# MasterVVK/qwen3-tts-axera-russian

Hardware: AMD Instinct MI355X
Metric: 12Hz codec-tokens/s (codec frames/s, 16 codes each) + RTF, Qwen3-TTS-0.6B (higher is better)
Workload: dtype f16 weights/KV, f32 accumulate (talker+CP); vocoder exact fp32 (f32 MFMA); 1 GPU; configs[2]/[3]: batch=32 mixed ru/en prompts per GPU, 64 frames/utterance/step (prefill + hipGraph decode loop), utterance-sharded DP over 1 GPU(s); batch_per_gpu=32

## Files before the change

### qwen3_tts_axera_russian_amd/csrc/q3_cp_api.hip

```cpp
#include "../../include/qwen3tts_cp.h"
#include "q3_cp.h"

namespace q3 {

static bool two_row_enabled() {
    static const bool on = !(getenv("Q3_CP_TWO_ROW") && atoi(getenv("Q3_CP_TWO_ROW")) == 0);
    return on;
}

int cp_seed_row0(const Work& w, int R, int row0, int R_total) {
    if (R_total <= 0) R_total = R;
    const int R16 = (R + 15) / 16 * 16;
    const bool two = two_row_enabled() && row0 == 0 && R_total == R && 2 * R16 <= w.max_rows;
    return two ? R16 : 0;
}

int cp_frame(hipStream_t s, const Model& m, Work& w, KVCache& kv, int R, const CpFrameIO& io, int row0, int R_total) {
    const ModelCfg& c = m.cfg;
    if (R_total <= 0) R_total = R;
    const int H = c.hidden, G = c.cp_groups;
    const int seed0 = cp_seed_row0(w, R, row0, R_total);
    RowMap rm;
    rm.slot_base = 0;
    rm.slot_stride = 1;
    rm.pos_stride = 0;
    if (seed0 > 0) {
        const int R16 = seed0;
        if (w.map_R16 != R16) {
            std::vector<int> slot(2 * R16), pos(2 * R16);
            for (int i = 0; i < 2 * R16; i++) {
                slot[i] = i % R16;
                pos[i] = i < R16 ? 1 : 0;
            }
            Q3_HIP(hipMemcpyAsync(w.map_slot, slot.data(), sizeof(int) * 2 * R16, hipMemcpyHostToDevice, s), -1);
            Q3_HIP(hipMemcpyAsync(w.map_pos, pos.data(), sizeof(int) * 2 * R16, hipMemcpyHostToDevice, s), -1);
            Q3_HIP(hipStreamSynchronize(s), -1);
            w.map_R16 = R16;
        }
        if (launch_gather_embed(s, m.talker_emb, c.talker_vocab, H, io.codes, 0, io.n_frames, io.frame_cap, 0, w.h, w.ssq, R,
                                row0, R_total, io.forced, w.xh, m.cp.L[0].in_ln))
            return -1;
        RowMap r2;
        r2.slot = w.map_slot;
        r2.pos = w.map_pos;
        r2.same_slot_rows = true;
        r2.valid_mod = R16;
        r2.valid_n = R;
        if (run_stack(s, m, m.cp, w, kv, R16 + R, r2, 256, 0)) return -1;
    } else {
        rm.pos_base = 0;
        if (run_stack(s, m, m.cp, w, kv, R, rm, 256, row0)) return -1;
        if (launch_gather_embed(s, m.talker_emb, c.talker_vocab, H, io.codes, 0, io.n_frames, io.frame_cap, 0, w.h, w.ssq, R,
                                row0, R_total, io.forced, w.xh, m.cp.L[0].in_ln))
            return -1;
        rm.pos_base = 1;
        if (run_stack(s, m, m.cp, w, kv, R, rm, 256, row0)) return -1;
    }
    const bool qkv_tab = m.cp_qkv_serves(R);
    for (int g = 0; g < G; g++) {
        if (g > 0) {
            rm.pos_base = g + 1;
            rm.skip_qkv0 = qkv_tab;
            if (run_stack(s, m, m.cp, w, kv, R, rm, 256, row0)) return -1;
        }
        LinArgs a;
        a.wp = m.cp_head[g].wp;
        a.N = c.cp_vocab;
        a.K = H;
        a.M = row0 + R;
        a.m_begin = row0;
        a.nt = 0;
        a.x16 = w.xh;
        a.ssq = w.ssq;
        a.ssq_parts = H / 16;
        a.eps = c.eps;
        a.y = w.logits;
        a.ldy = c.cp_vocab;
        if (launch_linear(s, a, PRO_NORM, EPI_STORE)) return -1;
        CpArgmaxArgs x;
        x.logits = w.logits;
        x.V = c.cp_vocab;
        x.R = R;
        x.row0 = row0;
        x.R_total = R_total;
        x.H = H;
        x.group = g;
        x.codes = io.codes;
        x.n_frames = io.n_frames;
        x.frame_cap = io.frame_cap;
        x.temperature = io.temperature;
        x.top_k = io.top_k;
        x.seed = io.seed;
        x.seed_ptr = io.seed_ptr;
        x.forced = io.forced;
        x.slots = io.slots;
        if (g + 1 < G) {
            x.next_table = m.cp_emb[g];
            x.h_out = w.h;
            x.ssq_out = w.ssq;
            x.xh_out = w.xh;
            x.gamma_next = m.cp.L[0].in_ln;
            if (qkv_tab) {
                x.next_qkv = m.cp_qkv_rows(g);
                x.qkv_out = w.qkv;
                x.qkv_ld = (c.n_heads + 2 * c.n_kv) * c.head_dim;
            }
        } else if (io.fb_h) {
            x.talker_emb = m.talker_emb;
            x.talker_vocab = c.talker_vocab;
            x.cp_tables = m.d_cp_emb_ptrs;
            x.pad_embed = io.pad_embed;
            x.n_groups = G;
            x.h_out = io.fb_h;
            x.ssq_out = io.fb_ssq;
            x.xh_out = io.fb_xh;
            x.gamma_next = io.fb_gamma;
        }
        if (launch_cp_argmax(s, x)) return -1;
    }
    return 0;
}

}

using namespace q3;

namespace {

struct CpHandle {
    Model* m = nullptr;
    int max_batch = 1;
    KVCache kv;
    Work w;
    hipStream_t s = nullptr;
    int *d_codes = nullptr, *d_nframes = nullptr;
    std::vector<int> h_codes;
    GraphExec graph;
    int graph_rows = 0;
    int step_next_pos = 0;
};

}

extern "C" {

void* cp_load(const char* weights, const char* embeddings_dir, int max_batch) {
    if (!weights) return nullptr;
    if (max_batch <= 0) max_batch = 1;
    Model* m = model_load(weights, false, true, embeddings_dir);
    if (!m) return nullptr;
    CpHandle* h = new CpHandle();
    h->m = m;
    h->max_batch = max_batch;
    const ModelCfg& c = m->cfg;
    bool ok = hipStreamCreate(&h->s) == hipSuccess;
    ok = ok && kv_alloc(h->kv, c.cp_layers, max_batch, c.n_kv, c.cp_groups + 1) == 0;
    ok = ok && work_alloc(h->w, c, 2 * ((max_batch + 15) / 16 * 16), c.cp_ffn, c.cp_vocab) == 0;
    ok = ok && hipMalloc((void**)&h->d_codes, sizeof(int) * 16 * max_batch) == hipSuccess;
    ok = ok && hipMalloc((void**)&h->d_nframes, sizeof(int) * max_batch) == hipSuccess;
    if (ok) {
        std::vector<int> ones(max_batch, 1);
        ok = hipMemcpy(h->d_nframes, ones.data(), sizeof(int) * max_batch, hipMemcpyHostToDevice) == hipSuccess;
    }
    if (!ok) {
        Q3_LOG("cp_load: allocation failed");
        cp_free(h);
        return nullptr;
    }
    h->h_codes.resize((size_t)16 * max_batch);
    return h;
}

void cp_free(void* hh) {
    CpHandle* h = (CpHandle*)hh;
    if (!h) return;
    if (h->s) hipStreamSynchronize(h->s);
    h->graph.reset();
    kv_free(h->kv);
    work_free(h->w);
    if (h->d_codes) hipFree(h->d_codes);
    if (h->d_nframes) hipFree(h->d_nframes);
    if (h->s) hipStreamDestroy(h->s);
    model_free(h->m);
    delete h;
}

int cp_hidden_size(void* hh) {
    CpHandle* h = (CpHandle*)hh;
    return h ? h->m->cfg.hidden : 0;
}

int cp_predict_batch(void* hh, const float* hidden, const int32_t* code_0, int n_rows, float temperature, int top_k,
                     uint64_t seed, int32_t* out_codes) {
    CpHandle* h = (CpHandle*)hh;
    if (!h || !hidden || !code_0 || !out_codes || n_rows <= 0 || n_rows > h->max_batch) return -1;
    const bool stochastic = temperature > 1e-6f;
    const Model& m = *h->m;
    const int H = m.cfg.hidden, G = m.cfg.cp_groups, R = n_rows;
    for (int r = 0; r < R; r++) {
        h->h_codes[(size_t)r * 16] = code_0[r];
        for (int j = 1; j < 16; j++) h->h_codes[(size_t)r * 16 + j] = -1;
    }
    Q3_HIP(hipMemcpyAsync(h->d_codes, h->h_codes.data(), sizeof(int) * 16 * R, hipMemcpyHostToDevice, h->s), -1);
    Q3_HIP(hipMemcpyAsync(h->w.rows_in, hidden, sizeof(float) * (size_t)R * H, hipMemcpyHostToDevice, h->s), -1);
    CpFrameIO io;
    io.codes = h->d_codes;
    io.n_frames = h->d_nframes;
    io.frame_cap = 1;
    io.temperature = temperature;
    io.top_k = top_k;
    io.seed = seed;
    auto body = [&]() -> int {
        if (launch_ssq_rows(h->s, h->w.rows_in, h->w.h, h->w.ssq, R, H, h->w.xh, m.cp.L[0].in_ln,
                            cp_seed_row0(h->w, R)))
            return -1;
        return cp_frame(h->s, m, h->w, h->kv, R, io);
    };
    if (stochastic) {
        if (body()) return -1;
    } else if (!h->graph.e || h->graph_rows != R) {
        if (body()) return -1;
        Q3_HIP(hipStreamSynchronize(h->s), -1);
        h->graph.reset();
        Q3_HIP(hipStreamBeginCapture(h->s, hipStreamCaptureModeThreadLocal), -1);
        int rc = body();
        hipError_t e = hipStreamEndCapture(h->s, &h->graph.g);
        if (rc || e != hipSuccess) {
            Q3_LOG("cp_predict: graph capture failed");
            return -1;
        }
        Q3_HIP(hipGraphInstantiate(&h->graph.e, h->graph.g, nullptr, nullptr, 0), -1);
        h->graph_rows = R;
    } else {
        Q3_HIP(hipGraphLaunch(h->graph.e, h->s), -1);
    }
    Q3_HIP(hipMemcpyAsync(h->h_codes.data(), h->d_codes, sizeof(int) * 16 * R, hipMemcpyDeviceToHost, h->s), -1);
    Q3_HIP(hipStreamSynchronize(h->s), -1);
    for (int r = 0; r < R; r++)
        for (int g = 0; g < G; g++) out_codes[(size_t)r * G + g] = h->h_codes[(size_t)r * 16 + 1 + g];
    return 0;
}

int cp_predict(void* hh, const float* hidden, int32_t code_0, float temperature, int top_k, uint64_t seed,
               int32_t* out_codes) {
    return cp_predict_batch(hh, hidden, &code_0, 1, temperature, top_k, seed, out_codes);
// ... 53 lines not shown
```

### qwen3_tts_axera_russian_amd/csrc/q3_engine.hip

```cpp
#include "../../include/qwen3tts_engine.h"
#include "q3_cp.h"

#include <algorithm>
#include <chrono>
#include <cmath>

using namespace q3;

namespace {

struct Engine {
    Model* m = nullptr;
    int max_batch = 0, n_ctx = 0, max_frames = 0;
    hipStream_t s = nullptr;
    KVCache kv_t, kv_c;
    Work wt, wc;
    int prefill_rows = 0;
    int *d_slot = nullptr, *d_pos = nullptr;
    int* d_tiles = nullptr;
    int *d_iota = nullptr;
    int *d_past = nullptr, *d_npast = nullptr, *d_ntext = nullptr, *d_done = nullptr, *d_nframes = nullptr;
    int *d_pos0 = nullptr, *d_posdec = nullptr, *d_lastrow = nullptr;
    int* d_codes = nullptr;
    int* d_forced = nullptr;
    bool forced_on = false;
    unsigned long long* d_seed = nullptr;
    unsigned long long n_requests = 0, req_seed = 0, n_refills = 0;
    float* d_pad = nullptr;
    int B = 0, ignore_eos = 0, cap_frames = 0, frames_run = 0;
    int frames_hi = 0;
    GraphExec graph[8];
    int graph_B = 0, graph_ignore = -1, graph_cap = -1, graph_chains = 0;
    hipEvent_t ev0 = nullptr, ev1 = nullptr;
    float last_run_ms = 0.f, last_prefill_ms = 0.f, last_host_launch_ms = 0.f;
    int* h_done = nullptr;
    float t_temp = 0.f, t_top_p = 0.95f, c_temp = 0.f;
    int t_top_k = 50, c_top_k = 50;
    unsigned long long seed = 0;
    int n_chains = 1;
    hipStream_t cs[8] = {nullptr};
    hipEvent_t ev_fork = nullptr, ev_join[8] = {nullptr};
    bool slot_mode = false;
    int graph_slots = -1;
    SlotParams* d_slots = nullptr;
    std::vector<int> h_budget, h_age;
    std::vector<char> h_live;
};

unsigned long long mix_seed(unsigned long long seed, unsigned long long k, unsigned long long golden) {
    unsigned long long z = seed + golden * k;
    z = (z ^ (z >> 30)) * 0xBF58476D1CE4E5B9ull;
    z = (z ^ (z >> 27)) * 0x94D049BB133111EBull;
    return z ^ (z >> 31);
}

int talker_tail(Engine* e, hipStream_t st, int row0, int R) {
    const Model& m = *e->m;
    const int H = m.cfg.hidden;
    FinalNormArgs f;
    f.h = e->wt.h;
    f.ssq = e->wt.ssq;
    f.ssq_parts = H / 16;
    f.gamma = m.talker.final_norm;
    f.eps = m.cfg.eps;
    f.R = R;
    f.row0 = row0;
    f.H = H;
    f.out_f32 = e->wt.hidden_f32;
    f.out_f16 = e->wt.hidden_f16;
    f.out_copy = e->wc.h;
    f.out_copy_ssq = e->wc.ssq;
    f.out_copy_xh = e->wc.xh;
    f.out_copy_gamma = m.cp.L[0].in_ln;
    f.out_copy_row_off = cp_seed_row0(e->wc, R, row0, e->B);
    if (launch_final_norm(st, f)) return -1;
    LinArgs a;
    a.wp = m.talker_head.wp;
    a.N = m.cfg.talker_vocab;
    a.K = H;
    a.M = row0 + R;
    a.m_begin = row0;
    a.nt = 1;
    a.x16 = e->wt.hidden_f16;
    a.y = e->wt.logits;
    a.ldy = m.cfg.talker_vocab;
    return launch_linear(st, a, PRO_F16, EPI_STORE);
}

int frame_chain(Engine* e, hipStream_t st, int row0, int R) {
    const Model& m = *e->m;
    TalkerSampleArgs sa;
    sa.logits = e->wt.logits;
    sa.V = m.cfg.talker_vocab;
    sa.R = R;
    sa.row0 = row0;
    sa.R_total = e->B;
    sa.audio_vocab = m.cfg.cp_vocab;
    sa.eos = m.cfg.codec_eos;
    sa.past = e->d_past;
    sa.n_past = e->d_npast;
    sa.n_text = e->d_ntext;
    sa.done = e->d_done;
    sa.codes = e->d_codes;
    sa.n_frames = e->d_nframes;
    sa.frame_cap = e->max_frames;
    sa.pos0 = e->d_pos0;
    sa.pos = e->d_posdec;
    sa.ignore_eos = e->ignore_eos;
    sa.max_frames = e->cap_frames;
    sa.temperature = e->t_temp;
    sa.top_k = e->t_top_k;
    sa.top_p = e->t_top_p;
    sa.seed = e->seed;
    sa.seed_ptr = e->d_seed;
    sa.forced = e->forced_on ? e->d_forced : nullptr;
    sa.slots = e->slot_mode ? e->d_slots : nullptr;
    if (launch_talker_sample(st, sa)) return -1;
    CpFrameIO io;
    io.codes = e->d_codes;
    io.n_frames = e->d_nframes;
    io.frame_cap = e->max_frames;
    io.fb_h = e->wt.h;
    io.fb_ssq = e->wt.ssq;
    io.fb_xh = e->wt.xh;
    io.fb_gamma = m.talker.L[0].in_ln;
    io.pad_embed = e->d_pad;
    io.temperature = e->c_temp;
    io.top_k = e->c_top_k;
    io.seed = e->seed ^ 0x5851F42D4C957F2Dull;
    io.seed_ptr = e->d_seed;
    io.forced = e->forced_on ? e->d_forced : nullptr;
    io.slots = e->slot_mode ? e->d_slots : nullptr;
    if (cp_frame(st, m, e->wc, e->kv_c, R, io, row0, e->B)) return -1;
    RowMap rm;
    rm.slot_base = 0;
    rm.slot_stride = 1;
    rm.pos = e->d_posdec;
    if (run_stack(st, m, m.talker, e->wt, e->kv_t, R, rm, 1024, row0)) return -1;
    return talker_tail(e, st, row0, R);
}

int n_chains_eff(const Engine* e) {
    const int nc = e->n_chains < 1 ? 1 : e->n_chains;
    return (nc > 1 && e->B % (16 * nc) == 0) ? nc : 1;
}

void chain_rows(const Engine* e, int c, int& row0, int& R) {
    const int nc = n_chains_eff(e);
    row0 = 0;
    for (int i = 0; i < c; i++) row0 += e->B / nc + (i < e->B % nc ? 1 : 0);
    R = e->B / nc + (c < e->B % nc ? 1 : 0);
}

int frame_eager(Engine* e) {
    const int nc = n_chains_eff(e);
    for (int c = 0; c < nc; c++) {
        int row0, R;
        chain_rows(e, c, row0, R);
        if (frame_chain(e, e->cs[c], row0, R)) return -1;
    }
    return 0;
}

int fork_chains(Engine* e) {
    Q3_HIP(hipEventRecord(e->ev_fork, e->s), -1);
    for (int c = 0; c < n_chains_eff(e); c++) Q3_HIP(hipStreamWaitEvent(e->cs[c], e->ev_fork, 0), -1);
    return 0;
}
int join_chains(Engine* e) {
    for (int c = 0; c < n_chains_eff(e); c++) {
        Q3_HIP(hipEventRecord(e->ev_join[c], e->cs[c]), -1);
        Q3_HIP(hipStreamWaitEvent(e->s, e->ev_join[c], 0), -1);
    }
    return 0;
}

}

extern "C" {

void q3e_free(void* ee) {
    Engine* e = (Engine*)ee;
    if (!e) return;
    if (e->s) hipStreamSynchronize(e->s);
    for (auto& g : e->graph) g.reset();
    kv_free(e->kv_t);
    kv_free(e->kv_c);
    work_free(e->wt);
    work_free(e->wc);
    void* ps[] = {e->d_tiles, e->d_slot, e->d_pos,  e->d_iota,   e->d_past,    e->d_npast, e->d_ntext, e->d_done,
                  e->d_nframes, e->d_pos0, e->d_posdec, e->d_lastrow, e->d_codes, e->d_pad, e->d_forced, e->d_seed, e->d_slots};
    for (void* p : ps)
        if (p) hipFree(p);
    if (e->h_done) hipHostFree(e->h_done);
    for (int c = 0; c < 8; c++) {
        if (e->cs[c]) hipStreamDestroy(e->cs[c]);
        if (e->ev_join[c]) hipEventDestroy(e->ev_join[c]);
    }
    if (e->ev_fork) hipEventDestroy(e->ev_fork);
    if (e->ev0) hipEventDestroy(e->ev0);
    if (e->ev1) hipEventDestroy(e->ev1);
    if (e->s) hipStreamDestroy(e->s);
    if (e->m) model_free(e->m);
    delete e;
}

void* q3e_create(const char* weights, int max_batch, int n_ctx, int max_frames) {
    if (!weights || max_batch <= 0 || n_ctx <= 0 || max_frames <= 0) return nullptr;
    Model* m = model_load(weights, true, true);
    if (!m) return nullptr;
    if (n_ctx > m->max_pos) {
        Q3_LOG("q3e_create: n_ctx=%d exceeds the RoPE table (%d)", n_ctx, m->max_pos);
        model_free(m);
        return nullptr;
    }
    Engine* e = new Engine();
    e->m = m;
    e->max_batch = max_batch;
    e->n_ctx = n_ctx;
    e->max_frames = max_frames;
    const ModelCfg& c = m->cfg;
    e->prefill_rows = max_batch > 2048 ? max_batch : 2048;
    int prio_lo = 0, prio_hi = 0;
    const bool use_prio = !(getenv("Q3_STREAM_PRIO") && atoi(getenv("Q3_STREAM_PRIO")) == 0) &&
                          hipDeviceGetStreamPriorityRange(&prio_lo, &prio_hi) == hipSuccess && prio_lo != prio_hi;
    auto mkstream = [&](hipStream_t* st) {
        return (use_prio ? hipStreamCreateWithPriority(st, hipStreamNonBlocking, prio_hi)
                         : hipStreamCreateWithFlags(st, hipStreamNonBlocking)) == hipSuccess;
    };
    bool ok = mkstream(&e->s);
    ok = ok && hipEventCreate(&e->ev0) == hipSuccess && hipEventCreate(&e->ev1) == hipSuccess;
    ok = ok && hipEventCreateWithFlags(&e->ev_fork, hipEventDisableTiming) == hipSuccess;
    for (int c = 0; c < 8 && ok; c++)
        ok = mkstream(&e->cs[c]) &&
             hipEventCreateWithFlags(&e->ev_join[c], hipEventDisableTiming) == hipSuccess;
    if (const char* nc = getenv("Q3_CHAINS")) e->n_chains = atoi(nc) < 1 ? 1 : atoi(nc) > 8 ? 8 : atoi(nc);
    else e->n_chains = 1;
    ok = ok && kv_alloc(e->kv_t, c.talker_layers, max_batch, c.n_kv, n_ctx) == 0;
    ok = ok && kv_alloc(e->kv_c, c.cp_layers, max_batch, c.n_kv, c.cp_groups + 1) == 0;
    ok = ok && work_alloc(e->wt, c, e->prefill_rows, c.talker_ffn, c.talker_vocab) == 0;
    ok = ok && work_alloc(e->wc, c, 2 * ((max_batch + 15) / 16 * 16), c.cp_ffn, c.cp_vocab) == 0;
    auto ialloc = [&](int** p, size_t n) { return hipMalloc((void**)p, sizeof(int) * n) == hipSuccess; };
    ok = ok && ialloc(&e->d_slot, e->prefill_rows) && ialloc(&e->d_pos, e->prefill_rows);
    ok = ok && ialloc(&e->d_tiles, (size_t)4 * e->prefill_rows);
    ok = ok && ialloc(&e->d_iota, max_batch) && ialloc(&e->d_past, (size_t)max_batch * 32);
    ok = ok && ialloc(&e->d_npast, max_batch) && ialloc(&e->d_ntext, max_batch) && ialloc(&e->d_done, max_batch);
    ok = ok && ialloc(&e->d_nframes, max_batch) && ialloc(&e->d_pos0, max_batch) && ialloc(&e->d_posdec, max_batch);
    ok = ok && ialloc(&e->d_lastrow, max_batch);
    ok = ok && ialloc(&e->d_codes, (size_t)max_frames * max_batch * 16);
    ok = ok && hipMalloc((void**)&e->d_pad, sizeof(float) * c.hidden) == hipSuccess;
    ok = ok && hipMalloc((void**)&e->d_seed, sizeof(unsigned long long) * max_batch) == hipSuccess;
    ok = ok && hipMemset(e->d_seed, 0, sizeof(unsigned long long) * max_batch) == hipSuccess;
    ok = ok && hipHostMalloc((void**)&e->h_done, sizeof(int) * max_batch, 0) == hipSuccess;
    if (ok) {
        std::vector<int> iota(max_batch);
        for (int i = 0; i < max_batch; i++) iota[i] = i;
        ok = hipMemcpy(e->d_iota, iota.data(), sizeof(int) * max_batch, hipMemcpyHostToDevice) == hipSuccess;
        ok = ok && hipMemset(e->d_pad, 0, sizeof(float) * c.hidden) == hipSuccess;
    }
    if (!ok) {
        Q3_LOG("q3e_create: allocation failed");
        q3e_free(e);
        return nullptr;
    }
    return e;
}

int q3e_set_sampling(void* ee, float talker_temperature, int talker_top_k, float talker_top_p, float cp_temperature,
                     int cp_top_k, uint64_t seed) {
    Engine* e = (Engine*)ee;
    if (!e) return -1;
    e->t_temp = talker_temperature;
    e->t_top_k = talker_top_k;
    e->t_top_p = talker_top_p;
    e->c_temp = cp_temperature;
    e->c_top_k = cp_top_k;
    e->seed = seed;
    e->n_requests = 0;
    for (auto& g : e->graph) g.reset();
    return 0;
}

int q3e_set_forced_codes(void* ee, const int32_t* forced, int n_frames) {
    Engine* e = (Engine*)ee;
    if (!e) return -1;
    const bool on = forced != nullptr && n_frames > 0;
    if (on && e->slot_mode) {
        Q3_LOG("q3e_set_forced_codes: not for a per-slot batch (q3e_open)");
        return -1;
    }
    if (on) {
        if (e->B <= 0 || n_frames > e->max_frames) return -1;
        const size_t total = (size_t)e->max_frames * e->max_batch * 16;
        if (!e->d_forced) Q3_HIP(hipMalloc((void**)&e->d_forced, sizeof(int) * total), -1);
        Q3_HIP(hipMemset(e->d_forced, 0xff, sizeof(int) * total), -1);
        Q3_HIP(hipMemcpy(e->d_forced, forced, sizeof(int) * 16 * (size_t)e->B * n_frames, hipMemcpyHostToDevice), -1);
    }
    if (on != e->forced_on) {
        e->forced_on = on;
        for (auto& g : e->graph) g.reset();
    }
    return 0;
}

int q3e_set_chains(void* ee, int n) {
    Engine* e = (Engine*)ee;
    if (!e || n < 1 || n > 8) return -1;
    if (n != e->n_chains) {
        e->n_chains = n;
        for (auto& g : e->graph) g.reset();
    }
    return 0;
}

int q3e_set_pad_embed(void* ee, const float* pad) {
    Engine* e = (Engine*)ee;
    if (!e || !pad) return -1;
    Q3_HIP(hipMemcpy(e->d_pad, pad, sizeof(float) * e->m->cfg.hidden, hipMemcpyHostToDevice), -1);
    return 0;
}

static int prefill_ids(Engine* e, int n, const int* ids, const float* prefix, const int32_t* n_rows, int B_total) {
    const Model& m = *e->m;
    const int H = m.cfg.hidden;
    size_t row_off = 0;
    int u0 = 0;
    std::vector<int> slot, pos, tiles, last(n);
    while (u0 < n) {
        int u1 = u0, rows = 0;
        while (u1 < n && rows + n_rows[u1] <= e->prefill_rows) rows += n_rows[u1++];
        slot.resize(rows);
        pos.resize(rows);
        int r = 0;
        tiles.clear();
        bool contiguous = true;
        for (int u = u0; u < u1; u++) {
            const int b = ids[u];
            if (u > u0 && b != ids[u - 1] + 1) contiguous = false;
            for (int i = 0; i < n_rows[u]; i += 16) {
                const int nn = n_rows[u] - i < 16 ? n_rows[u] - i : 16;
                const int t4[4] = {r + i, nn, b, i};
                tiles.insert(tiles.end(), t4, t4 + 4);
            }
            for (int i = 0; i < n_rows[u]; i++, r++) {
                slot[r] = b;
                pos[r] = i;
            }
            last[u] = r - 1;
        }
        Q3_HIP(hipMemcpyAsync(e->wt.rows_in, prefix + row_off * H, sizeof(float) * (size_t)rows * H, hipMemcpyHostToDevice, e->s), -1);
        Q3_HIP(hipMemcpyAsync(e->d_slot, slot.data(), sizeof(int) * rows, hipMemcpyHostToDevice, e->s), -1);
        Q3_HIP(hipMemcpyAsync(e->d_pos, pos.data(), sizeof(int) * rows, hipMemcpyHostToDevice, e->s), -1);
        Q3_HIP(hipMemcpyAsync(e->d_tiles, tiles.data(), sizeof(int) * tiles.size(), hipMemcpyHostToDevice, e->s), -1);
        if (contiguous) {
            Q3_HIP(hipMemcpyAsync(e->d_lastrow + ids[u0], last.data() + u0, sizeof(int) * (u1 - u0), hipMemcpyHostToDevice, e->s), -1);
        } else {
            for (int u = u0; u < u1; u++)
                Q3_HIP(hipMemcpyAsync(e->d_lastrow + ids[u], last.data() + u, sizeof(int), hipMemcpyHostToDevice, e->s), -1);
        }
        if (launch_ssq_rows(e->s, e->wt.rows_in, e->wt.h, e->wt.ssq, rows, H, e->wt.xh, m.talker.L[0].in_ln)) return -1;
        RowMap rm;
        rm.slot = e->d_slot;
        rm.pos = e->d_pos;
        rm.same_slot_rows = true;
        rm.tiles = e->d_tiles;
        rm.n_tiles = (int)(tiles.size() / 4);
        if (run_stack(e->s, m, m.talker, e->wt, e->kv_t, rows, rm, 1024)) return -1;
        for (int u = u0; u < u1; u += contiguous ? (u1 - u0) : 1) {
            FinalNormArgs f;
            f.h = e->wt.h;
            f.ssq = e->wt.ssq;
            f.ssq_parts = H / 16;
            f.gamma = m.talker.final_norm;
            f.eps = m.cfg.eps;
            f.R = contiguous ? u1 - u0 : 1;
            f.row0 = ids[u];
            f.H = H;
            f.row_map = e->d_lastrow;
            f.out_f32 = e->wt.hidden_f32;
            f.out_f16 = e->wt.hidden_f16;
            f.out_copy = e->wc.h;
            f.out_copy_ssq = e->wc.ssq;
            f.out_copy_xh = e->wc.xh;
            f.out_copy_gamma = m.cp.L[0].in_ln;
            f.out_copy_row_off = n_chains_eff(e) == 1 ? cp_seed_row0(e->wc, B_total, 0, B_total) : 0;
            if (launch_final_norm(e->s, f)) return -1;
        }
        Q3_HIP(hipStreamSynchronize(e->s), -1);
        row_off += rows;
        u0 = u1;
    }
    return 0;
}

static int clear_slot(Engine* e, int b, const int32_t* n_rows, const int32_t* n_text) {
    Q3_HIP(hipMemsetAsync(e->d_npast + b, 0, sizeof(int), e->s), -1);
    Q3_HIP(hipMemsetAsync(e->d_done + b, 0, sizeof(int), e->s), -1);
    Q3_HIP(hipMemsetAsync(e->d_nframes + b, 0, sizeof(int), e->s), -1);
    Q3_HIP(hipMemsetAsync(e->d_past + 32 * b, 0, sizeof(int) * 32, e->s), -1);
    Q3_HIP(hipMemset2DAsync(e->d_codes + 16 * (size_t)b, sizeof(int) * 16 * (size_t)e->B, 0xff, sizeof(int) * 16, e->max_frames, e->s), -1);
    Q3_HIP(hipMemcpyAsync(e->d_ntext + b, n_text, sizeof(int), hipMemcpyHostToDevice, e->s), -1);
    Q3_HIP(hipMemcpyAsync(e->d_pos0 + b, n_rows, sizeof(int), hipMemcpyHostToDevice, e->s), -1);
    Q3_HIP(hipMemcpyAsync(e->d_posdec + b, n_rows, sizeof(int), hipMemcpyHostToDevice, e->s), -1);
    return 0;
}

static int head_all_rows(Engine* e) {
    const Model& m = *e->m;
    LinArgs a;
    a.wp = m.talker_head.wp;
    a.N = m.cfg.talker_vocab;
    a.K = m.cfg.hidden;
    a.M = e->B;
    a.nt = 1;
    a.x16 = e->wt.hidden_f16;
    a.y = e->wt.logits;
    a.ldy = m.cfg.talker_vocab;
    return launch_linear(e->s, a, PRO_F16, EPI_STORE);
}

int q3e_start(void* ee, int B, const float* prefix, const int32_t* n_rows, const int32_t* n_text, int ignore_eos,
              int max_frames) {
    Engine* e = (Engine*)ee;
    if (!e || !prefix || !n_rows || !n_text || B <= 0 || B > e->max_batch) return -1;
    const Model& m = *e->m;
    const int H = m.cfg.hidden;
    if (max_frames <= 0 || max_frames > e->max_frames) max_frames = e->max_frames;
    std::vector<int> pos0(B);
    for (int b = 0; b < B; b++) {
        if (n_rows[b] <= 0 || n_rows[b] > e->prefill_rows || n_rows[b] + max_frames > e->n_ctx) {
            Q3_LOG("q3e_start: utterance %d: %d prefix rows + %d frames do not fit n_ctx=%d", b, n_rows[b], max_frames,
                   e->n_ctx);
            return -1;
        }
        pos0[b] = n_rows[b];
    }
    e->B = B;
    e->ignore_eos = ignore_eos ? 1 : 0;
    e->cap_frames = max_frames;
    e->frames_run = 0;
    e->frames_hi = 0;
    e->slot_mode = false;
    Q3_HIP(hipMemsetAsync(e->d_npast, 0, sizeof(int) * B, e->s), -1);
    Q3_HIP(hipMemsetAsync(e->d_done, 0, sizeof(int) * B, e->s), -1);
    Q3_HIP(hipMemsetAsync(e->d_nframes, 0, sizeof(int) * B, e->s), -1);
    Q3_HIP(hipMemsetAsync(e->d_past, 0, sizeof(int) * 32 * B, e->s), -1);
    Q3_HIP(hipMemsetAsync(e->d_codes, 0xff, sizeof(int) * 16 * (size_t)B * e->max_frames, e->s), -1);
    {
        unsigned long long z = e->seed + 0x9E3779B97F4A7C15ull * e->n_requests++;
        z = (z ^ (z >> 30)) * 0xBF58476D1CE4E5B9ull;
        z = (z ^ (z >> 27)) * 0x94D049BB133111EBull;
        e->req_seed = e->n_requests == 1 ? e->seed : (z ^ (z >> 31));
        e->n_refills = 0;
        std::vector<unsigned long long> seeds(B, e->req_seed);
        Q3_HIP(hipMemcpy(e->d_seed, seeds.data(), sizeof(unsigned long long) * B, hipMemcpyHostToDevice), -1);
    }
    if (e->forced_on) {
        e->forced_on = false;
        for (auto& g : e->graph) g.reset();
    }
    Q3_HIP(hipMemcpyAsync(e->d_ntext, n_text, sizeof(int) * B, hipMemcpyHostToDevice, e->s), -1);
    Q3_HIP(hipMemcpyAsync(e->d_pos0, pos0.data(), sizeof(int) * B, hipMemcpyHostToDevice, e->s), -1);
    Q3_HIP(hipMemcpyAsync(e->d_posdec, pos0.data(), sizeof(int) * B, hipMemcpyHostToDevice, e->s), -1);
    Q3_HIP(hipStreamSynchronize(e->s), -1);
    Q3_HIP(hipEventRecord(e->ev0, e->s), -1);
    {
        std::vector<int> ids(B);
        for (int b = 0; b < B; b++) ids[b] = b;
        if (prefill_ids(e, B, ids.data(), prefix, n_rows, B)) return -1;
    }
    if (head_all_rows(e)) return -1;
    Q3_HIP(hipEventRecord(e->ev1, e->s), -1);
    Q3_HIP(hipStreamSynchronize(e->s), -1);
    hipEventElapsedTime(&e->last_prefill_ms, e->ev0, e->ev1);
    return 0;
}

int q3e_run(void* ee, int n_frames) {
    Engine* e = (Engine*)ee;
    if (!e || e->B <= 0 || n_frames <= 0) return -1;
    int room = (e->cap_frames < e->max_frames ? e->cap_frames : e->max_frames) - e->frames_run;
    if (e->slot_mode) {
        room = 0;
        for (int b = 0; b < e->B; b++)
            if (e->h_live[b]) room = std::max(room, e->h_budget[b] - e->h_age[b]);
    }
    if (room <= 0) return 0;
    if (n_frames > room) n_frames = room;
    int done_frames = 0;
    const int nc = n_chains_eff(e);
    Q3_HIP(hipEventRecord(e->ev0, e->s), -1);
    if (fork_chains(e)) return -1;
    static const bool no_graph = getenv("Q3_NO_GRAPH") && atoi(getenv("Q3_NO_GRAPH")) != 0;
    const bool need_capture = !e->graph[0].e || e->graph_B != e->B || e->graph_ignore != e->ignore_eos ||
                              e->graph_cap != e->cap_frames || e->graph_chains != nc ||
                              e->graph_slots != (int)e->slot_mode;
    if (no_graph) {
        for (; done_frames < n_frames; done_frames++)
            if (frame_eager(e)) return -1;
    } else if (need_capture) {
        if (frame_eager(e)) return -1;
        done_frames++;
        for (int c = 0; c < nc; c++) Q3_HIP(hipStreamSynchronize(e->cs[c]), -1);
        for (int c = 0; c < nc; c++) {
            int row0, R;
            chain_rows(e, c, row0, R);
            e->graph[c].reset();
            Q3_HIP(hipStreamBeginCapture(e->cs[c], hipStreamCaptureModeRelaxed), -1);
            int rc = frame_chain(e, e->cs[c], row0, R);
            hipError_t er = hipStreamEndCapture(e->cs[c], &e->graph[c].g);
            if (rc || er != hipSuccess) {
                Q3_LOG("q3e_run: graph capture failed");
                return -1;
            }
            Q3_HIP(hipGraphInstantiate(&e->graph[c].e, e->graph[c].g, nullptr, nullptr, 0), -1);
        }
        e->graph_B = e->B;
        e->graph_ignore = e->ignore_eos;
        e->graph_cap = e->cap_frames;
        e->graph_chains = nc;
        e->graph_slots = (int)e->slot_mode;
    }
    const int check_every = 16;
    const auto th0 = std::chrono::steady_clock::now();
    while (!no_graph && done_frames < n_frames) {
        int chunk = n_frames - done_frames;
        if (!e->ignore_eos && chunk > check_every) chunk = check_every;
        for (int i = 0; i < chunk; i++)
            for (int c = 0; c < nc; c++) Q3_HIP(hipGraphLaunch(e->graph[c].e, e->cs[c]), -1);
        done_frames += chunk;
        if (!e->ignore_eos && done_frames < n_frames) {
            if (join_chains(e)) return -1;
            Q3_HIP(hipMemcpyAsync(e->h_done, e->d_done, sizeof(int) * e->B, hipMemcpyDeviceToHost, e->s), -1);
            Q3_HIP(hipStreamSynchronize(e->s), -1);
            bool all = true;
            for (int b = 0; b < e->B; b++) all = all && e->h_done[b];
            if (all) break;
            if (fork_chains(e)) return -1;
        }
    }
    e->last_host_launch_ms = (float)std::chrono::duration<double, std::milli>(std::chrono::steady_clock::now() - th0).count();
    if (join_chains(e)) return -1;
    Q3_HIP(hipEventRecord(e->ev1, e->s), -1);
    Q3_HIP(hipStreamSynchronize(e->s), -1);
    hipEventElapsedTime(&e->last_run_ms, e->ev0, e->ev1);
    if (e->slot_mode) {
        for (int b = 0; b < e->B; b++)
            if (e->h_age[b] >= 0) e->h_age[b] = std::min(e->h_age[b] + done_frames, e->max_frames);
        return done_frames;
    }
    e->frames_run += done_frames;
    e->frames_hi += done_frames;
    return done_frames;
}

float q3e_last_run_ms(void* ee) { return ee ? ((Engine*)ee)->last_run_ms : -1.f; }
float q3e_last_host_launch_ms(void* ee) { return ee ? ((Engine*)ee)->last_host_launch_ms : -1.f; }
float q3e_last_prefill_ms(void* ee) { return ee ? ((Engine*)ee)->last_prefill_ms : -1.f; }

int q3e_get_codes(void* ee, int32_t* out, int max_out_frames, int32_t* n_frames_per_utt) {
    Engine* e = (Engine*)ee;
    if (!e || !out || e->B <= 0) return -1;
    int nf = e->frames_hi < e->max_frames ? e->frames_hi : e->max_frames;
    if (e->slot_mode) {
        int hi = 0;
        for (int b = 0; b < e->B; b++)
            hi = std::max(hi, e->h_age[b]);
        nf = std::min(hi, e->max_frames);
    }
    if (nf > max_out_frames) nf = max_out_frames;
    Q3_HIP(hipMemcpy(out, e->d_codes, sizeof(int) * 16 * (size_t)e->B * nf, hipMemcpyDeviceToHost), -1);
    if (n_frames_per_utt) {
        Q3_HIP(hipMemcpy(n_frames_per_utt, e->d_npast, sizeof(int) * e->B, hipMemcpyDeviceToHost), -1);
    }
    return nf;
}

int q3e_get_done(void* ee, int32_t* done, int32_t* frames) {
    Engine* e = (Engine*)ee;
    if (!e || !done || e->B <= 0) return -1;
    Q3_HIP(hipMemcpy(done, e->d_done, sizeof(int) * e->B, hipMemcpyDeviceToHost), -1);
    std::vector<int> np(e->B);
    Q3_HIP(hipMemcpy(np.data(), e->d_npast, sizeof(int) * e->B, hipMemcpyDeviceToHost), -1);
    for (int b = 0; b < e->B; b++)
        if (np[b] >= (e->slot_mode ? e->h_budget[b] : e->cap_frames)) done[b] = 1;
    if (e->slot_mode)
        for (int b = 0; b < e->B; b++)
            if (done[b]) e->h_live[b] = 0;
    if (frames) memcpy(frames, np.data(), sizeof(int) * e->B);
    return 0;
}

int q3e_refill(void* ee, int n, const int32_t* slots, const float* prefix, const int32_t* n_rows, const int32_t* n_text) {
    Engine* e = (Engine*)ee;
    if (!e || e->B <= 0 || n <= 0 || n > e->B || !slots || !prefix || !n_rows || !n_text) return -1;
    if (e->forced_on) {
        Q3_LOG("q3e_refill: a teacher-forced batch cannot be refilled");
        return -1;
    }
    if (e->slot_mode) {
        Q3_LOG("q3e_refill: a per-slot batch (q3e_open) takes new utterances with q3e_admit");
        return -1;
    }
    std::vector<int> ids(slots, slots + n), seen(e->B, 0);
    for (int u = 0; u < n; u++) {
        const int b = ids[u];
        if (b < 0 || b >= e->B || seen[b]++) {
            Q3_LOG("q3e_refill: slot %d is out of range or listed twice (batch of %d)", b, e->B);
            return -1;
        }
        if (n_rows[u] <= 0 || n_rows[u] > e->prefill_rows || n_rows[u] + e->cap_frames > e->n_ctx) {
            Q3_LOG("q3e_refill: utterance %d: %d prefix rows + %d frames do not fit n_ctx=%d", u, n_rows[u], e->cap_frames, e->n_ctx);
            return -1;
        }
    }
    Q3_HIP(hipStreamSynchronize(e->s), -1);
    Q3_HIP(hipEventRecord(e->ev0, e->s), -1);
    for (int u = 0; u < n; u++) {
        const int b = ids[u];
        if (clear_slot(e, b, n_rows + u, n_text + u)) return -1;
        unsigned long long z = e->req_seed + 0xD1B54A32D192ED03ull * ++e->n_refills;
        z = (z ^ (z >> 30)) * 0xBF58476D1CE4E5B9ull;
        z = (z ^ (z >> 27)) * 0x94D049BB133111EBull;
        z ^= z >> 31;
        Q3_HIP(hipMemcpyAsync(e->d_seed + b, &z, sizeof(z), hipMemcpyHostToDevice, e->s), -1);
        Q3_HIP(hipStreamSynchronize(e->s), -1);
    }
    Q3_HIP(hipStreamSynchronize(e->s), -1);
    if (prefill_ids(e, n, ids.data(), prefix, n_rows, e->B)) return -1;
    if (head_all_rows(e)) return -1;
    Q3_HIP(hipEventRecord(e->ev1, e->s), -1);
    Q3_HIP(hipStreamSynchronize(e->s), -1);
    hipEventElapsedTime(&e->last_prefill_ms, e->ev0, e->ev1);
    e->frames_run = 0;
    return 0;
}

int q3e_open(void* ee, int B, int ignore_eos) {
    Engine* e = (Engine*)ee;
    if (!e || B <= 0 || B > e->max_batch) return -1;
    const Model& m = *e->m;
    const ModelCfg& c = m.cfg;
    if (c.talker_vocab > 4096 || c.cp_vocab > 4096) {
        Q3_LOG("q3e_open: vocabularies of %d / %d are beyond the per-slot sampler", c.talker_vocab, c.cp_vocab);
        return -1;
    }
    Q3_HIP(hipStreamSynchronize(e->s), -1);
    if (!e->d_slots) Q3_HIP(hipMalloc((void**)&e->d_slots, sizeof(SlotParams) * e->max_batch), -1);
    e->B = B;
    e->ignore_eos = ignore_eos ? 1 : 0;
    e->cap_frames = e->max_frames;
    e->frames_run = 0;
    e->frames_hi = 0;
    e->slot_mode = true;
    e->h_budget.assign(B, 0);
    e->h_age.assign(B, -1);
    e->h_live.assign(B, 0);
    if (e->forced_on) {
        e->forced_on = false;
        for (auto& g : e->graph) g.reset();
    }
    Q3_HIP(hipMemsetAsync(e->d_npast, 0, sizeof(int) * B, e->s), -1);
    Q3_HIP(hipMemsetD32Async((hipDeviceptr_t)e->d_done, 1, B, e->s), -1);
    Q3_HIP(hipMemsetD32Async((hipDeviceptr_t)e->d_nframes, e->max_frames, B, e->s), -1);
    Q3_HIP(hipMemsetAsync(e->d_past, 0, sizeof(int) * 32 * B, e->s), -1);
    Q3_HIP(hipMemsetAsync(e->d_ntext, 0, sizeof(int) * B, e->s), -1);
// ... 10 lines not shown

int q3e_admit(void* ee, int n, const int32_t* slots, const float* prefix, const int32_t* n_rows, const int32_t* n_text,
              const q3e_slot_params* params) {
    Engine* e = (Engine*)ee;
    if (!e || !e->slot_mode || n <= 0 || n > e->B || !slots || !prefix || !n_rows || !n_text || !params) {
        if (e && !e->slot_mode) Q3_LOG("q3e_admit: the batch was not opened with q3e_open");
        return -1;
    }
    std::vector<int> ids(slots, slots + n), seen(e->B, 0);
    std::vector<SlotParams> sp(n);
    for (int u = 0; u < n; u++) {
        const int b = ids[u];
        const q3e_slot_params& p = params[u];
        if (b < 0 || b >= e->B || seen[b]++) {
            Q3_LOG("q3e_admit: slot %d is out of range or listed twice (batch of %d)", b, e->B);
            return -1;
        }
        if (p.max_frames <= 0 || p.max_frames > e->max_frames) {
            Q3_LOG("q3e_admit: utterance %d: a budget of %d frames is outside 1..%d", u, p.max_frames, e->max_frames);
            return -1;
        }
        if (n_rows[u] <= 0 || n_rows[u] > e->prefill_rows || n_rows[u] + p.max_frames > e->n_ctx) {
            Q3_LOG("q3e_admit: utterance %d: %d prefix rows + %d frames do not fit n_ctx=%d", u, n_rows[u], p.max_frames, e->n_ctx);
            return -1;
        }
        if (!(std::isfinite(p.temperature) && p.temperature >= 0.f) || !(std::isfinite(p.cp_temperature) && p.cp_temperature >= 0.f) ||
            !(p.top_p > 0.f && p.top_p <= 1.f)) {
            Q3_LOG("q3e_admit: utterance %d: temperatures must be finite and >= 0, top_p in (0, 1]", u);
            return -1;
        }
        sp[u].max_frames = p.max_frames;
        sp[u].t_temp = p.temperature;
        sp[u].t_top_k = p.top_k;
        sp[u].t_top_p = p.top_p;
        sp[u].c_temp = p.cp_temperature;
        sp[u].c_top_k = p.cp_top_k;
        sp[u].seed = mix_seed(p.seed, (unsigned long long)(uint32_t)p.utt + 1ull, 0x9E3779B97F4A7C15ull);
        sp[u].no_row = 1;
    }
    Q3_HIP(hipStreamSynchronize(e->s), -1);
    Q3_HIP(hipEventRecord(e->ev0, e->s), -1);
    for (int u = 0; u < n; u++) {
        if (clear_slot(e, ids[u], n_rows + u, n_text + u)) return -1;
        Q3_HIP(hipMemcpyAsync(e->d_slots + ids[u], &sp[u], sizeof(SlotParams), hipMemcpyHostToDevice, e->s), -1);
    }
    Q3_HIP(hipStreamSynchronize(e->s), -1);
    const int H = e->m->cfg.hidden;
    size_t row_off = 0;
    for (int u = 0; u < n; u++) {
        if (prefill_ids(e, 1, &ids[u], prefix + row_off * H, n_rows + u, e->B)) return -1;
        row_off += n_rows[u];
    }
    if (head_all_rows(e)) return -1;
    Q3_HIP(hipEventRecord(e->ev1, e->s), -1);
    Q3_HIP(hipStreamSynchronize(e->s), -1);
    hipEventElapsedTime(&e->last_prefill_ms, e->ev0, e->ev1);
    for (int u = 0; u < n; u++) {
        e->h_budget[ids[u]] = sp[u].max_frames;
        e->h_age[ids[u]] = 0;
        e->h_live[ids[u]] = 1;
    }
    return 0;
}

int q3e_release(void* ee, int n, const int32_t* slots) {
    Engine* e = (Engine*)ee;
    if (!e || !e->slot_mode || n < 0 || (n > 0 && !slots)) return -1;
    for (int u = 0; u < n; u++)
        if (slots[u] < 0 || slots[u] >= e->B) {
            Q3_LOG("q3e_release: slot %d is out of range (batch of %d)", slots[u], e->B);
            return -1;
        }
    for (int u = 0; u < n; u++) {
        Q3_HIP(hipMemsetD32Async((hipDeviceptr_t)(e->d_done + slots[u]), 1, 1, e->s), -1);
        e->h_live[slots[u]] = 0;
    }
    Q3_HIP(hipStreamSynchronize(e->s), -1);
    return 0;
}

int q3e_get_hidden(void* ee, float* out) {
    Engine* e = (Engine*)ee;
    if (!e || !out || e->B <= 0) return -1;
    Q3_HIP(hipMemcpy(out, e->wt.hidden_f32, sizeof(float) * (size_t)e->B * e->m->cfg.hidden, hipMemcpyDeviceToHost), -1);
    return 0;
}

double q3e_step_weight_bytes(void* ee) {
    Engine* e = (Engine*)ee;
    if (!e) return 0.0;
    const ModelCfg& c = e->m->cfg;
    const double head = 2.0 * c.hidden;
    double bytes = (double)e->m->talker.weight_bytes + head * c.talker_vocab +
                   (double)(c.cp_groups + 1) * (double)e->m->cp.weight_bytes + head * c.cp_vocab * c.cp_groups;
    int row0 = 0, R = e->B;
    if (e->B > 0) chain_rows(e, 0, row0, R);
    if (R > 0 && e->m->cp_qkv_serves(R)) {
        const double qkv_ld = (double)(c.n_heads + 2 * c.n_kv) * c.head_dim;
        bytes -= (double)(c.cp_groups - 1) * (qkv_ld * c.hidden * 2.0 - 4.0 * qkv_ld * e->B);
    }
    return bytes;
}

}
```

### qwen3_tts_axera_russian_amd/csrc/q3_model.h

```cpp
#pragma once
#include "q3_kernels.h"

namespace q3 {

struct DevLinear {
    half_t* wp = nullptr;
    int N = 0, K = 0;
};

struct DevLayer {
    DevLinear qkv, o, gu, down;
    float *in_ln = nullptr, *post_ln = nullptr, *q_norm = nullptr, *k_norm = nullptr;
};

struct DevStack {
    std::vector<DevLayer> L;
    float* final_norm = nullptr;
    const float* tail_gamma = nullptr;
    int ffn = 0;
    int nt = 0;
    size_t weight_bytes = 0;
};

struct Model {
    ModelCfg cfg;
    int device = 0;
    bool has_talker = false, has_cp = false;
    DevStack talker, cp;
    float* talker_emb = nullptr;
    DevLinear talker_head;
    std::vector<float*> cp_emb;
    std::vector<DevLinear> cp_head;
    const float** d_cp_emb_ptrs = nullptr;
    float* cp_qkv_tab = nullptr;
    int cp_qkv_kbw = 0;
    const float* cp_qkv_rows(int group) const {
        return cp_qkv_tab + (size_t)group * cfg.cp_vocab * ((cfg.n_heads + 2 * cfg.n_kv) * cfg.head_dim);
    }
    bool cp_qkv_serves(int rows) const {
        return cp_qkv_tab && linear_decode_kbw(cfg.hidden, (cfg.n_heads + 2 * cfg.n_kv) * cfg.head_dim, rows) == cp_qkv_kbw;
    }
    float *rope_cos = nullptr, *rope_sin = nullptr;
    int max_pos = 0;
    std::vector<void*> allocs;
    size_t device_bytes = 0;
};

Model* model_load(const char* path, bool want_talker, bool want_cp, const char* aux_dir = nullptr);
void model_free(Model* m);

struct KVCache {
    half_t *k = nullptr, *v = nullptr;
    int n_layers = 0, n_slots = 0, n_kv = 0, n_ctx = 0, head_dim = 128;
    size_t layer_stride() const { return (size_t)n_slots * n_kv * n_ctx * head_dim; }
    size_t bytes() const { return layer_stride() * n_layers * sizeof(half_t) * 2; }
};
int kv_alloc(KVCache& kv, int n_layers, int n_slots, int n_kv, int n_ctx);
void kv_free(KVCache& kv);
int kv_zero(hipStream_t s, KVCache& kv);

inline size_t frag_idx_host(int m, int k, int K) {
    return ((((size_t)(m >> 4) * (K >> 5) + (k >> 5)) * 64 + (m & 15) + 16 * ((k >> 3) & 3)) << 3) + (k & 7);
}

struct Work {
    int max_rows = 0, hidden = 0;
    float* rows_in = nullptr;
    float *h = nullptr, *ssq = nullptr, *qkv = nullptr;
    half_t* xh = nullptr;
    half_t *attn = nullptr, *act = nullptr;
    float* hidden_f32 = nullptr;
    half_t* hidden_f16 = nullptr;
    float* logits = nullptr;
    int *map_slot = nullptr, *map_pos = nullptr;
    int map_R16 = 0;
};
int work_alloc(Work& w, const ModelCfg& c, int max_rows, int ffn, int max_vocab);
void work_free(Work& w);
int work_zero(hipStream_t s, Work& w, const ModelCfg& c, int ffn, int max_vocab);

struct RowMap {
    const int* slot = nullptr;
    const int* pos = nullptr;
    int slot_base = 0, slot_stride = 0, pos_base = 0, pos_stride = 0;
    bool same_slot_rows = false;
    int valid_mod = 0, valid_n = 0;
    const int* tiles = nullptr;
    int n_tiles = 0;
    bool skip_qkv0 = false;
};

int run_stack(hipStream_t s, const Model& m, const DevStack& st, Work& w, KVCache& kv, int R,
              const RowMap& rm, int attn_threads, int row0 = 0);

struct GraphExec {
    hipGraph_t g = nullptr;
    hipGraphExec_t e = nullptr;
    void reset();
};

}
```

### qwen3_tts_axera_russian_amd/csrc/q3_model.hip

```cpp
#include "q3_model.h"

#include <cmath>

namespace q3 {

namespace {

struct Loader {
    Model* m;
    const Pack& p;
    hipStream_t s = nullptr;
    half_t* stage = nullptr;
    size_t stage_elems = 0;
    std::vector<uint16_t> host16;
    bool ok = true;

    void* dalloc(size_t bytes) {
        void* d = nullptr;
        if (hipMalloc(&d, bytes) != hipSuccess) {
            Q3_LOG("hipMalloc(%zu) failed", bytes);
            ok = false;
            return nullptr;
        }
        m->allocs.push_back(d);
        m->device_bytes += bytes;
        return d;
    }
    const PackTensor* need(const std::string& n, uint32_t ndim, uint64_t d0, uint64_t d1 = 0) {
        const PackTensor* t = p.find(n);
        if (!t) {
            Q3_LOG("weight file lacks tensor %s", n.c_str());
            ok = false;
            return nullptr;
        }
        if (t->ndim != ndim || t->shape[0] != d0 || (ndim > 1 && t->shape[1] != d1) ||
            (t->dtype != F32 && t->dtype != F16 && t->dtype != BF16)) {
            Q3_LOG("tensor %s: unexpected shape/dtype", n.c_str());
            ok = false;
            return nullptr;
        }
        return t;
    }
    float* up_f32(const std::string& n, uint32_t ndim, uint64_t d0, uint64_t d1 = 0) {
        const PackTensor* t = need(n, ndim, d0, d1);
        if (!t) return nullptr;
        size_t ne = t->numel();
        float* d = (float*)dalloc(ne * 4);
        if (!d) return nullptr;
        if (t->dtype == F32) {
            if (hipMemcpy(d, t->data, ne * 4, hipMemcpyHostToDevice) != hipSuccess) ok = false;
        } else {
            std::vector<float> tmp(ne);
            const uint16_t* src = (const uint16_t*)t->data;
            if (t->dtype == BF16)
                for (size_t i = 0; i < ne; i++) tmp[i] = bf16_to_f32(src[i]);
            else
                for (size_t i = 0; i < ne; i++) tmp[i] = h2f(src[i]);
            if (hipMemcpy(d, tmp.data(), ne * 4, hipMemcpyHostToDevice) != hipSuccess) ok = false;
        }
        return d;
    }
    bool pack_into(const std::string& n, int N, int K, half_t* dst, int tile_off, int tile_stride) {
        const PackTensor* t = need(n, 2, (uint64_t)N, (uint64_t)K);
        if (!t) return false;
        size_t ne = (size_t)N * K;
        if (ne > stage_elems) {
            if (stage) hipFree(stage);
            stage = nullptr;
            if (hipMalloc((void**)&stage, ne * 2) != hipSuccess) {
                ok = false;
                return false;
            }
            stage_elems = ne;
        }
        const void* src = t->data;
        if (t->dtype == F32) {
            host16.resize(ne);
            const float* f = (const float*)t->data;
            for (size_t i = 0; i < ne; i++) host16[i] = f2h_sat(f[i]);
            src = host16.data();
        } else if (t->dtype == BF16) {
            host16.resize(ne);
            const uint16_t* b = (const uint16_t*)t->data;
            for (size_t i = 0; i < ne; i++) host16[i] = f2h_sat(bf16_to_f32(b[i]));
            src = host16.data();
        }
        if (hipMemcpy(stage, src, ne * 2, hipMemcpyHostToDevice) != hipSuccess) {
            ok = false;
            return false;
        }
        if (launch_pack_linear(s, stage, N, K, dst, tile_off, tile_stride) != 0) {
            ok = false;
            return false;
        }
        if (hipStreamSynchronize(s) != hipSuccess) {
            ok = false;
            return false;
        }
        return true;
    }
    DevLinear lin_alloc(int N, int K) {
        DevLinear l;
        l.N = N;
        l.K = K;
        l.wp = (half_t*)dalloc((size_t)N * K * 2);
        return l;
    }
    bool load_stack(DevStack& st, const char* prefix, int n_layers, int ffn) {
        const ModelCfg& c = m->cfg;
        const int H = c.hidden, D = c.head_dim, NQ = c.n_heads * D, NKV = c.n_kv * D;
        st.ffn = ffn;
        st.L.resize(n_layers);
        for (int i = 0; i < n_layers && ok; i++) {
            DevLayer& L = st.L[i];
            std::string b = std::string(prefix) + ".layers." + std::to_string(i) + ".";
            L.in_ln = up_f32(b + "input_ln", 1, H);
            L.post_ln = up_f32(b + "post_ln", 1, H);
            L.q_norm = up_f32(b + "q_norm", 1, D);
            L.k_norm = up_f32(b + "k_norm", 1, D);
            L.qkv = lin_alloc(NQ + 2 * NKV, H);
            L.o = lin_alloc(H, NQ);
            L.gu = lin_alloc(2 * ffn, H);
            L.down = lin_alloc(H, ffn);
            if (!ok) break;
            pack_into(b + "q_proj", NQ, H, L.qkv.wp, 0, 1);
            pack_into(b + "k_proj", NKV, H, L.qkv.wp, NQ / 16, 1);
            pack_into(b + "v_proj", NKV, H, L.qkv.wp, (NQ + NKV) / 16, 1);
            pack_into(b + "o_proj", H, NQ, L.o.wp, 0, 1);
            pack_into(b + "gate_proj", ffn, H, L.gu.wp, 0, 2);
            pack_into(b + "up_proj", ffn, H, L.gu.wp, 1, 2);
            pack_into(b + "down_proj", H, ffn, L.down.wp, 0, 1);
            st.weight_bytes += ((size_t)(NQ + 2 * NKV) * H + (size_t)H * NQ + (size_t)3 * ffn * H) * 2;
        }
        st.final_norm = up_f32(std::string(prefix) + ".norm", 1, H);
        return ok;
    }
    bool build_cp_qkv_table() {
        static const bool on = !(getenv("Q3_CP_QKV_TABLE") && atoi(getenv("Q3_CP_QKV_TABLE")) == 0);
        const ModelCfg& c = m->cfg;
        const int H = c.hidden, V = c.cp_vocab, G = c.cp_groups, ld = (c.n_heads + 2 * c.n_kv) * c.head_dim;
        if (!on || G < 2) return true;
        int pass = 64;
        while (pass >= 16 && !linear_decode_kbw(H, ld, pass)) pass /= 2;
        if (pass < 16) {
            Q3_LOG("code predictor: no q|k|v table (launch_linear has no weight-streaming kernel for K=%d)", H);
            return true;
        }
        const size_t Vp = ((size_t)V + 63) / 64 * 64, bytes = (size_t)(G - 1) * V * ld * sizeof(float);
        float* tab = (float*)dalloc(bytes);
        int* ids = nullptr;
        float *h = nullptr, *ssq = nullptr;
        half_t* xh = nullptr;
        bool good = tab && hipMalloc((void**)&ids, Vp * 4) == hipSuccess && hipMalloc((void**)&h, Vp * H * 4) == hipSuccess &&
                    hipMalloc((void**)&ssq, Vp * (H / 16) * 4) == hipSuccess && hipMalloc((void**)&xh, Vp * H * 2) == hipSuccess;
        if (good) {
            std::vector<int> iota(Vp, -1);
            for (int t = 0; t < V; t++) iota[t] = t;
            good = hipMemcpy(ids, iota.data(), Vp * 4, hipMemcpyHostToDevice) == hipSuccess;
        }
        for (int g = 0; g + 1 < G && good; g++) {
            good = launch_gather_embed(s, m->cp_emb[g], V, H, ids, 1, nullptr, 0, 0, h, ssq, (int)Vp, 0, 0, nullptr, xh,
                                       m->cp.L[0].in_ln) == 0;
            for (int r0 = 0; r0 < V && good; r0 += pass) {
                LinArgs a;
                a.wp = m->cp.L[0].qkv.wp;
                a.N = m->cp.L[0].qkv.N;
                a.K = H;
                a.M = r0 + pass < V ? r0 + pass : V;
                a.m_begin = r0;
                a.nt = m->cp.nt;
                a.x16 = xh;
                a.ssq = ssq;
                a.ssq_parts = H / 16;
                a.eps = c.eps;
                a.y = tab + (size_t)g * V * ld;
                a.ldy = ld;
                good = launch_linear(s, a, PRO_NORM, EPI_STORE) == 0;
            }
        }
        good = good && hipStreamSynchronize(s) == hipSuccess;
        for (void* d : {(void*)ids, (void*)h, (void*)ssq, (void*)xh})
            if (d) hipFree(d);
        if (!good) {
            Q3_LOG("code predictor: building the q|k|v table failed");
            ok = false;
            return false;
        }
        m->cp_qkv_tab = tab;
        m->cp_qkv_kbw = linear_decode_kbw(H, ld, pass);
        Q3_LOG("code predictor: layer-0 q|k|v table, %d groups x %d tokens x %d columns f32 = %zu bytes", G - 1, V, ld, bytes);
        return true;
    }
};

}

Model* model_load(const char* path, bool want_talker, bool want_cp, const char* aux_dir) {
    int ndev = 0;
    if (hipGetDeviceCount(&ndev) != hipSuccess || ndev <= 0) {
        Q3_LOG("no HIP device available -- this library has no CPU path");
        return nullptr;
    }
    Pack p;
    if (!p.open_auto(path, aux_dir)) return nullptr;
    Model* m = new Model();
    m->cfg.from_pack(p);
    const ModelCfg& c = m->cfg;
    if (c.head_dim != 128 || c.hidden != 1024 || c.n_heads != 2 * c.n_kv) {
        Q3_LOG("unsupported geometry: hidden=%d head_dim=%d heads=%d/%d (kernels are built for 1024/128, GQA 2)",
               c.hidden, c.head_dim, c.n_heads, c.n_kv);
        delete m;
        return nullptr;
    }
    hipGetDevice(&m->device);
    Loader L{m, p};
    if (hipStreamCreate(&L.s) != hipSuccess) {
        delete m;
        return nullptr;
    }
    const int H = c.hidden;
    if (p.find("talker.codec_embedding")) m->talker_emb = L.up_f32("talker.codec_embedding", 2, c.talker_vocab, H);
    if (want_talker) {
        m->talker.nt = 1;
        L.load_stack(m->talker, "talker", c.talker_layers, c.talker_ffn);
        m->talker_head = L.lin_alloc(c.talker_vocab, H);
        if (L.ok) L.pack_into("talker.codec_head", c.talker_vocab, H, m->talker_head.wp, 0, 1);
        if (!m->talker_emb) {
            Q3_LOG("weight file lacks talker.codec_embedding");
            L.ok = false;
        }
        m->has_talker = L.ok;
    }
    if (want_cp && L.ok) {
        m->cp.nt = 0;
        L.load_stack(m->cp, "cp", c.cp_layers, c.cp_ffn);
        m->cp.tail_gamma = m->cp.final_norm;
        m->cp_emb.resize(c.cp_groups);
        m->cp_head.resize(c.cp_groups);
        for (int g = 0; g < c.cp_groups && L.ok; g++) {
            m->cp_emb[g] = L.up_f32("cp.codec_emb." + std::to_string(g), 2, c.cp_vocab, H);
            m->cp_head[g] = L.lin_alloc(c.cp_vocab, H);
            if (L.ok) L.pack_into("cp.lm_head." + std::to_string(g), c.cp_vocab, H, m->cp_head[g].wp, 0, 1);
        }
        if (L.ok) {
            m->d_cp_emb_ptrs = (const float**)L.dalloc(sizeof(float*) * c.cp_groups);
            if (m->d_cp_emb_ptrs &&
                hipMemcpy((void*)m->d_cp_emb_ptrs, m->cp_emb.data(), sizeof(float*) * c.cp_groups,
                          hipMemcpyHostToDevice) != hipSuccess)
                L.ok = false;
        }
        if (!m->talker_emb) {
            Q3_LOG("weight file lacks talker.codec_embedding (code_0 embedding of the code predictor)");
            L.ok = false;
        }
        if (L.ok) L.build_cp_qkv_table();
        m->has_cp = L.ok;
    }
    if (L.ok) {
        m->max_pos = 8192;
        const int half = c.head_dim / 2;
        std::vector<float> cs((size_t)m->max_pos * half), sn((size_t)m->max_pos * half);
        for (int i = 0; i < half; i++) {
            const float inv_freq = 1.0f / powf((float)c.rope_theta, (float)(2 * i) / (float)c.head_dim);
            for (int pos = 0; pos < m->max_pos; pos++) {
                const float ang = (float)pos * inv_freq;
                cs[(size_t)pos * half + i] = cosf(ang);
                sn[(size_t)pos * half + i] = sinf(ang);
            }
        }
        m->rope_cos = (float*)L.dalloc(cs.size() * 4);
        m->rope_sin = (float*)L.dalloc(sn.size() * 4);
        if (L.ok) {
            if (hipMemcpy(m->rope_cos, cs.data(), cs.size() * 4, hipMemcpyHostToDevice) != hipSuccess) L.ok = false;
            if (hipMemcpy(m->rope_sin, sn.data(), sn.size() * 4, hipMemcpyHostToDevice) != hipSuccess) L.ok = false;
        }
    }
    if (L.stage) hipFree(L.stage);
    hipStreamDestroy(L.s);
    if (!L.ok) {
        model_free(m);
        return nullptr;
    }
    return m;
}

void model_free(Model* m) {
    if (!m) return;
    for (void* d : m->allocs) hipFree(d);
    delete m;
}

int kv_alloc(KVCache& kv, int n_layers, int n_slots, int n_kv, int n_ctx) {
    kv.n_layers = n_layers;
    kv.n_slots = n_slots;
    kv.n_kv = n_kv;
    kv.n_ctx = n_ctx;
    const size_t bytes = kv.layer_stride() * n_layers * sizeof(half_t);
    Q3_HIP(hipMalloc((void**)&kv.k, bytes), -1);
    Q3_HIP(hipMalloc((void**)&kv.v, bytes), -1);
    Q3_HIP(hipMemset(kv.k, 0, bytes), -1);
    Q3_HIP(hipMemset(kv.v, 0, bytes), -1);
    return 0;
}
void kv_free(KVCache& kv) {
    if (kv.k) hipFree(kv.k);
    if (kv.v) hipFree(kv.v);
    kv.k = kv.v = nullptr;
}

int kv_zero(hipStream_t s, KVCache& kv) {
    const size_t bytes = kv.layer_stride() * kv.n_layers * sizeof(half_t);
    Q3_HIP(hipMemsetAsync(kv.k, 0, bytes, s), -1);
    Q3_HIP(hipMemsetAsync(kv.v, 0, bytes, s), -1);
    return 0;
}

int work_zero(hipStream_t s, Work& w, const ModelCfg& c, int ffn, int max_vocab) {
    const size_t R = (size_t)w.max_rows;
    const int qkv_ld = (c.n_heads + 2 * c.n_kv) * c.head_dim;
    Q3_HIP(hipMemsetAsync(w.rows_in, 0, R * c.hidden * 4, s), -1);
    Q3_HIP(hipMemsetAsync(w.h, 0, R * c.hidden * 4, s), -1);
    Q3_HIP(hipMemsetAsync(w.ssq, 0, R * (c.hidden / 16) * 4, s), -1);
    Q3_HIP(hipMemsetAsync(w.xh, 0, R * c.hidden * 2, s), -1);
    Q3_HIP(hipMemsetAsync(w.qkv, 0, R * qkv_ld * 4, s), -1);
    Q3_HIP(hipMemsetAsync(w.attn, 0, R * c.n_heads * c.head_dim * 2, s), -1);
    Q3_HIP(hipMemsetAsync(w.act, 0, R * ffn * 2, s), -1);
    Q3_HIP(hipMemsetAsync(w.hidden_f32, 0, R * c.hidden * 4, s), -1);
    Q3_HIP(hipMemsetAsync(w.hidden_f16, 0, R * c.hidden * 2, s), -1);
    Q3_HIP(hipMemsetAsync(w.logits, 0, R * max_vocab * 4, s), -1);
    return 0;
}

int work_alloc(Work& w, const ModelCfg& c, int max_rows, int ffn, int max_vocab) {
    max_rows = (max_rows + 127) / 128 * 128;
    w.max_rows = max_rows;
    w.hidden = c.hidden;
    const size_t R = (size_t)max_rows;
    const int qkv_ld = (c.n_heads + 2 * c.n_kv) * c.head_dim;
    Q3_HIP(hipMalloc((void**)&w.rows_in, R * c.hidden * 4), -1);
    Q3_HIP(hipMalloc((void**)&w.h, R * c.hidden * 4), -1);
    Q3_HIP(hipMemset(w.h, 0, R * c.hidden * 4), -1);
    Q3_HIP(hipMalloc((void**)&w.ssq, R * (c.hidden / 16) * 4), -1);
    Q3_HIP(hipMalloc((void**)&w.xh, R * c.hidden * 2), -1);
    Q3_HIP(hipMemset(w.xh, 0, R * c.hidden * 2), -1);
    Q3_HIP(hipMalloc((void**)&w.qkv, R * qkv_ld * 4), -1);
    Q3_HIP(hipMalloc((void**)&w.attn, R * c.n_heads * c.head_dim * 2), -1);
    Q3_HIP(hipMemset(w.attn, 0, R * c.n_heads * c.head_dim * 2), -1);
    Q3_HIP(hipMalloc((void**)&w.act, R * ffn * 2), -1);
    Q3_HIP(hipMemset(w.act, 0, R * ffn * 2), -1);
    Q3_HIP(hipMalloc((void**)&w.hidden_f32, R * c.hidden * 4), -1);
    Q3_HIP(hipMalloc((void**)&w.hidden_f16, R * c.hidden * 2), -1);
    Q3_HIP(hipMemset(w.hidden_f16, 0, R * c.hidden * 2), -1);
    Q3_HIP(hipMalloc((void**)&w.logits, R * max_vocab * 4), -1);
    Q3_HIP(hipMalloc((void**)&w.map_slot, R * 4), -1);
    Q3_HIP(hipMalloc((void**)&w.map_pos, R * 4), -1);
    w.map_R16 = 0;
    return 0;
}
void work_free(Work& w) {
    void* ps[] = {w.rows_in, w.h, w.ssq, w.xh, w.qkv, w.attn, w.act, w.hidden_f32, w.hidden_f16, w.logits, w.map_slot, w.map_pos};
    for (void* p : ps)
        if (p) hipFree(p);
    w = Work();
}

int run_stack(hipStream_t s, const Model& m, const DevStack& st, Work& w, KVCache& kv, int R, const RowMap& rm,
              int attn_threads, int row0) {
    const ModelCfg& c = m.cfg;
    const int H = c.hidden, D = c.head_dim;
    const int qkv_ld = (c.n_heads + 2 * c.n_kv) * D;
    if (row0 % 16) {
        Q3_LOG("run_stack: row0=%d must be a multiple of 16 (fragment-ordered activations)", row0);
        return -1;
    }
    if (row0 + R > w.max_rows) {
        Q3_LOG("run_stack: %d rows > workspace %d", R, w.max_rows);
        return -1;
    }
    for (size_t li = 0; li < st.L.size(); li++) {
        const DevLayer& L = st.L[li];
        LinArgs a;
        a = LinArgs();
        a.wp = L.qkv.wp;
        a.N = L.qkv.N;
        a.K = H;
        a.M = row0 + R;
        a.m_begin = row0;
        a.nt = st.nt;
        a.x16 = w.xh;
        a.ssq = w.ssq;
        a.ssq_parts = H / 16;
        a.eps = c.eps;
        a.y = w.qkv;
        a.ldy = qkv_ld;
        if (!(li == 0 && rm.skip_qkv0) && launch_linear(s, a, PRO_NORM, EPI_STORE)) return -1;
        AttnArgs t;
        t.qkv = w.qkv;
        t.ld = qkv_ld;
        t.R = R;
        t.row0 = row0;
        t.q_norm = L.q_norm;
        t.k_norm = L.k_norm;
        t.eps = c.eps;
        t.rope_cos = m.rope_cos;
        t.rope_sin = m.rope_sin;
        t.slot = rm.slot;
        t.pos = rm.pos;
        t.slot_base = rm.slot_base;
        t.slot_stride = rm.slot_stride;
        t.pos_base = rm.pos_base;
        t.pos_stride = rm.pos_stride;
        t.kc = kv.k + li * kv.layer_stride();
        t.vc = kv.v + li * kv.layer_stride();
        t.n_ctx = kv.n_ctx;
        t.n_kv = c.n_kv;
        t.n_heads = c.n_heads;
        t.out = w.attn;
        t.scale = 1.0f / sqrtf((float)D);
        t.threads = attn_threads;
        t.valid_mod = rm.valid_mod;
        t.valid_n = rm.valid_n;
        if (rm.same_slot_rows && R > 1) {
            if (launch_attn(s, t, ATTN_PREP)) return -1;
            if (rm.tiles && rm.n_tiles > 0) {
                t.tiles = rm.tiles;
                t.n_tiles = rm.n_tiles;
            } else if (!rm.slot && !rm.pos && rm.slot_stride == 0 && rm.pos_stride == 1 && rm.valid_mod == 0) {
                t.tiles = nullptr;
                t.n_tiles = (R + 15) / 16;
            }
            if (launch_attn(s, t, ATTN_ATTEND)) return -1;
        } else {
            if (launch_attn(s, t, ATTN_FUSED)) return -1;
        }
        a = LinArgs();
        a.wp = L.o.wp;
        a.N = H;
        a.K = L.o.K;
        a.M = row0 + R;
        a.m_begin = row0;
        a.nt = st.nt;
        a.x16 = w.attn;
        a.h_out = w.h;
        a.ssq_out = w.ssq;
        a.xh_out = w.xh;
        a.gamma = L.post_ln;
        if (launch_linear(s, a, PRO_F16, EPI_RESID)) return -1;
        a = LinArgs();
        a.wp = L.gu.wp;
        a.N = L.gu.N;
        a.K = H;
        a.M = row0 + R;
        a.m_begin = row0;
        a.nt = st.nt;
        a.x16 = w.xh;
        a.ssq = w.ssq;
        a.ssq_parts = H / 16;
        a.eps = c.eps;
        a.act = w.act;
        if (launch_linear(s, a, PRO_NORM, EPI_SWIGLU)) return -1;
        a = LinArgs();
        a.wp = L.down.wp;
        a.N = H;
        a.K = L.down.K;
        a.M = row0 + R;
        a.m_begin = row0;
        a.nt = st.nt;
        a.x16 = w.act;
        a.h_out = w.h;
        a.ssq_out = w.ssq;
        a.gamma = li + 1 < st.L.size() ? st.L[li + 1].in_ln : st.tail_gamma;
        a.xh_out = a.gamma ? w.xh : nullptr;
        if (launch_linear(s, a, PRO_F16, EPI_RESID)) return -1;
    }
    return 0;
}

void GraphExec::reset() {
    if (e) hipGraphExecDestroy(e);
    if (g) hipGraphDestroy(g);
    e = nullptr;
    g = nullptr;
}

}
```

### qwen3_tts_axera_russian_amd/csrc/q3_talker_api.hip

```cpp
#include "../../include/qwen3tts_talker.h"
#include "q3_model.h"

using namespace q3;

namespace {

struct TalkerModel {
    Model* m = nullptr;
};

struct TalkerCtx {
    TalkerModel* tm = nullptr;
    int n_ctx = 0, n_batch = 0, n_slots = 1;
    KVCache kv;
    Work w;
    hipStream_t s = nullptr;
    int *d_slot = nullptr, *d_pos = nullptr;
    std::vector<int> n_used;
    GraphExec g1;
    int g1_rows = 0;
    float* h_pinned = nullptr;
    int* i_pinned = nullptr;
};

const int kStateMagic = 0x564b3351;

int attn_threads_for(int n_ctx) { return n_ctx <= 64 ? 256 : 1024; }

int forward_rows(TalkerCtx* c, int R, const RowMap& rm) {
    const Model& m = *c->tm->m;
    if (launch_ssq_rows(c->s, c->w.rows_in, c->w.h, c->w.ssq, R, m.cfg.hidden, c->w.xh, m.talker.L[0].in_ln)) return -1;
    if (run_stack(c->s, m, m.talker, c->w, c->kv, R, rm, attn_threads_for(c->n_ctx))) return -1;
    return 0;
}

int final_hidden(TalkerCtx* c, int first_row, int R) {
    const Model& m = *c->tm->m;
    const int H = m.cfg.hidden;
    FinalNormArgs f;
    f.h = c->w.h;
    f.ssq = c->w.ssq;
    f.src_off = first_row;
    f.ssq_parts = H / 16;
    f.gamma = m.talker.final_norm;
    f.eps = m.cfg.eps;
    f.R = R;
    f.H = H;
    f.out_f32 = c->w.hidden_f32;
    f.out_f16 = c->w.hidden_f16;
    return launch_final_norm(c->s, f);
}

}

extern "C" {

void wrapper_backend_init(void) {
    int n = 0;
    if (hipGetDeviceCount(&n) != hipSuccess || n <= 0)
        Q3_LOG("wrapper_backend_init: no HIP device visible; model loading will fail (no CPU path)");
}

void wrapper_backend_free(void) {}

void* wrapper_load_model(const char* path, int n_gpu_layers) {
    (void)n_gpu_layers;
    if (!path) return nullptr;
    Model* m = model_load(path, true, false);
    if (!m) return nullptr;
    TalkerModel* tm = new TalkerModel();
    tm->m = m;
    return tm;
}

void wrapper_free_model(void* model) {
    TalkerModel* tm = (TalkerModel*)model;
    if (!tm) return;
    model_free(tm->m);
    delete tm;
}

int wrapper_model_n_embd(const void* model) {
    const TalkerModel* tm = (const TalkerModel*)model;
    return tm && tm->m ? tm->m->cfg.hidden : 0;
}

void* wrapper_create_context_slots(void* model, int n_ctx, int n_batch, int n_slots) {
    TalkerModel* tm = (TalkerModel*)model;
    if (!tm || !tm->m || n_ctx <= 0 || n_slots <= 0) return nullptr;
    if (n_batch <= 0) n_batch = n_ctx;
    if (n_ctx > tm->m->max_pos) {
        Q3_LOG("wrapper_create_context: n_ctx=%d exceeds the RoPE table (%d)", n_ctx, tm->m->max_pos);
        return nullptr;
    }
    TalkerCtx* c = new TalkerCtx();
    c->tm = tm;
    c->n_ctx = n_ctx;
    c->n_batch = n_batch > n_slots ? n_batch : n_slots;
    c->n_slots = n_slots;
    c->n_used.assign(n_slots, 0);
    const ModelCfg& cfg = tm->m->cfg;
    bool ok = hipStreamCreate(&c->s) == hipSuccess;
    ok = ok && kv_alloc(c->kv, cfg.talker_layers, n_slots, cfg.n_kv, n_ctx) == 0;
    ok = ok && work_alloc(c->w, cfg, c->n_batch, cfg.talker_ffn, cfg.talker_vocab) == 0;
    ok = ok && hipMalloc((void**)&c->d_slot, sizeof(int) * c->n_batch) == hipSuccess;
    ok = ok && hipMalloc((void**)&c->d_pos, sizeof(int) * c->n_batch) == hipSuccess;
    ok = ok && hipHostMalloc((void**)&c->h_pinned, sizeof(float) * cfg.hidden * 2, 0) == hipSuccess;
    ok = ok && hipHostMalloc((void**)&c->i_pinned, sizeof(int) * 2, 0) == hipSuccess;
    if (!ok) {
        Q3_LOG("wrapper_create_context: allocation failed");
        wrapper_free_context(c);
        return nullptr;
    }
    return c;
}

void* wrapper_create_context(void* model, int n_ctx, int n_batch, int n_threads, int embeddings) {
    (void)n_threads;
    if (!embeddings) {
        Q3_LOG("wrapper_create_context: only embeddings mode exists in this library");
        return nullptr;
    }
    return wrapper_create_context_slots(model, n_ctx, n_batch, 1);
}

void wrapper_free_context(void* ctx) {
    TalkerCtx* c = (TalkerCtx*)ctx;
    if (!c) return;
    if (c->s) hipStreamSynchronize(c->s);
    c->g1.reset();
    kv_free(c->kv);
    work_free(c->w);
    if (c->d_slot) hipFree(c->d_slot);
    if (c->d_pos) hipFree(c->d_pos);
    if (c->h_pinned) hipHostFree(c->h_pinned);
    if (c->i_pinned) hipHostFree(c->i_pinned);
    if (c->s) hipStreamDestroy(c->s);
    delete c;
}

int wrapper_ctx_n_slots(void* ctx) {
    TalkerCtx* c = (TalkerCtx*)ctx;
    return c ? c->n_slots : 0;
}

void wrapper_kv_clear(void* ctx) {
    TalkerCtx* c = (TalkerCtx*)ctx;
    if (!c) return;
    c->n_used.assign(c->n_slots, 0);
}

int wrapper_decode_embd_slot(void* ctx, int slot, const float* embd, int n_tokens, int n_embd, int pos_start,
                             float* out_hidden) {
    TalkerCtx* c = (TalkerCtx*)ctx;
    if (!c || !embd || !out_hidden) return -1;
    const Model& m = *c->tm->m;
    const int H = m.cfg.hidden;
    if (n_embd != H || n_tokens <= 0 || n_tokens > c->n_batch || slot < 0 || slot >= c->n_slots || pos_start < 0 ||
        pos_start + n_tokens > c->n_ctx) {
        Q3_LOG("wrapper_decode_embd: bad arguments (n_tokens=%d n_embd=%d pos_start=%d slot=%d; n_ctx=%d n_batch=%d)",
               n_tokens, n_embd, pos_start, slot, c->n_ctx, c->n_batch);
        return -1;
    }
    Q3_HIP(hipMemcpyAsync(c->w.rows_in, embd, sizeof(float) * (size_t)n_tokens * H, hipMemcpyHostToDevice, c->s), -1);
    if (n_tokens == 1) {
        c->i_pinned[0] = slot;
        c->i_pinned[1] = pos_start;
        Q3_HIP(hipMemcpyAsync(c->d_slot, &c->i_pinned[0], sizeof(int), hipMemcpyHostToDevice, c->s), -1);
        Q3_HIP(hipMemcpyAsync(c->d_pos, &c->i_pinned[1], sizeof(int), hipMemcpyHostToDevice, c->s), -1);
        RowMap rm;
        rm.slot = c->d_slot;
        rm.pos = c->d_pos;
        if (!c->g1.e || c->g1_rows != 1) {
            if (forward_rows(c, 1, rm) || final_hidden(c, 0, 1)) return -1;
            Q3_HIP(hipStreamSynchronize(c->s), -1);
            c->g1.reset();
            Q3_HIP(hipStreamBeginCapture(c->s, hipStreamCaptureModeThreadLocal), -1);
            int rc = forward_rows(c, 1, rm) || final_hidden(c, 0, 1);
            hipError_t e = hipStreamEndCapture(c->s, &c->g1.g);
            if (rc || e != hipSuccess) {
                Q3_LOG("wrapper_decode_embd: graph capture failed");
                return -1;
            }
            Q3_HIP(hipGraphInstantiate(&c->g1.e, c->g1.g, nullptr, nullptr, 0), -1);
            c->g1_rows = 1;
        } else {
            Q3_HIP(hipGraphLaunch(c->g1.e, c->s), -1);
// ... 16 lines not shown
}

int wrapper_decode_embd(void* ctx, const float* embd, int n_tokens, int n_embd, int pos_start, float* out_hidden) {
    return wrapper_decode_embd_slot(ctx, 0, embd, n_tokens, n_embd, pos_start, out_hidden);
}

int wrapper_decode_embd_batch(void* ctx, const float* embd, int n_rows, int n_embd, const int32_t* slot_ids,
                              const int32_t* pos, float* out_hidden) {
    TalkerCtx* c = (TalkerCtx*)ctx;
    if (!c || !embd || !out_hidden || !slot_ids || !pos) return -1;
    const Model& m = *c->tm->m;
    const int H = m.cfg.hidden;
    if (n_embd != H || n_rows <= 0 || n_rows > c->n_batch || n_rows > c->n_slots) return -1;
    for (int r = 0; r < n_rows; r++) {
        if (slot_ids[r] < 0 || slot_ids[r] >= c->n_slots || pos[r] < 0 || pos[r] >= c->n_ctx) return -1;
        for (int q = 0; q < r; q++)
            if (slot_ids[q] == slot_ids[r]) return -1;
    }
    Q3_HIP(hipMemcpyAsync(c->w.rows_in, embd, sizeof(float) * (size_t)n_rows * H, hipMemcpyHostToDevice, c->s), -1);
    Q3_HIP(hipMemcpyAsync(c->d_slot, slot_ids, sizeof(int) * n_rows, hipMemcpyHostToDevice, c->s), -1);
    Q3_HIP(hipMemcpyAsync(c->d_pos, pos, sizeof(int) * n_rows, hipMemcpyHostToDevice, c->s), -1);
    RowMap rm;
    rm.slot = c->d_slot;
    rm.pos = c->d_pos;
    if (forward_rows(c, n_rows, rm) || final_hidden(c, 0, n_rows)) return -1;
    Q3_HIP(hipMemcpyAsync(out_hidden, c->w.hidden_f32, sizeof(float) * (size_t)n_rows * H, hipMemcpyDeviceToHost, c->s),
           -1);
    Q3_HIP(hipStreamSynchronize(c->s), -1);
    for (int r = 0; r < n_rows; r++)
        if (pos[r] + 1 > c->n_used[slot_ids[r]]) c->n_used[slot_ids[r]] = pos[r] + 1;
    return 0;
}

int wrapper_codec_head(void* ctx, const float* hidden, int n_rows, float* logits_out) {
    TalkerCtx* c = (TalkerCtx*)ctx;
    if (!c || !hidden || !logits_out || n_rows <= 0 || n_rows > c->n_batch) return -1;
    const Model& m = *c->tm->m;
    const int H = m.cfg.hidden, V = m.cfg.talker_vocab;
    std::vector<uint16_t> h16((size_t)((n_rows + 15) / 16 * 16) * H, 0);
    for (int r = 0; r < n_rows; r++)
        for (int k = 0; k < H; k++) h16[frag_idx_host(r, k, H)] = f2h_sat(hidden[(size_t)r * H + k]);
    Q3_HIP(hipMemcpyAsync(c->w.hidden_f16, h16.data(), h16.size() * 2, hipMemcpyHostToDevice, c->s), -1);
    LinArgs a;
    a.wp = m.talker_head.wp;
    a.N = V;
    a.K = H;
    a.M = n_rows;
    a.nt = 1;
    a.x16 = c->w.hidden_f16;
    a.y = c->w.logits;
    a.ldy = V;
    if (launch_linear(c->s, a, PRO_F16, EPI_STORE)) return -1;
    Q3_HIP(hipMemcpyAsync(logits_out, c->w.logits, sizeof(float) * (size_t)n_rows * V, hipMemcpyDeviceToHost, c->s), -1);
    Q3_HIP(hipStreamSynchronize(c->s), -1);
    return V;
}

size_t wrapper_state_get_size(void* ctx) {
    TalkerCtx* c = (TalkerCtx*)ctx;
    if (!c) return 0;
    const size_t per = (size_t)c->kv.n_kv * c->n_used[0] * c->kv.head_dim * sizeof(half_t);
    return 6 * sizeof(int32_t) + 2 * per * c->kv.n_layers;
}

int wrapper_state_save_file(void* ctx, const char* path) {
    TalkerCtx* c = (TalkerCtx*)ctx;
    if (!c || !path) return -1;
    FILE* f = fopen(path, "wb");
    if (!f) {
        Q3_LOG("wrapper_state_save_file: failed to save to %s", path);
        return -1;
    }
    const int n_pos = c->n_used[0], D = c->kv.head_dim;
    int32_t hdr[6] = {kStateMagic, 1, c->kv.n_layers, c->kv.n_kv, D, n_pos};
    bool ok = fwrite(hdr, sizeof(hdr), 1, f) == 1;
    std::vector<uint16_t> buf((size_t)n_pos * D);
    hipStreamSynchronize(c->s);
    for (int l = 0; l < c->kv.n_layers && ok; l++)
        for (int kvsel = 0; kvsel < 2 && ok; kvsel++)
            for (int g = 0; g < c->kv.n_kv && ok; g++) {
                const half_t* base = (kvsel ? c->kv.v : c->kv.k) + l * c->kv.layer_stride() +
                                     ((size_t)0 * c->kv.n_kv + g) * (size_t)c->kv.n_ctx * D;
                if (n_pos > 0) {
                    ok = hipMemcpy(buf.data(), base, buf.size() * 2, hipMemcpyDeviceToHost) == hipSuccess;
                    ok = ok && fwrite(buf.data(), 2, buf.size(), f) == buf.size();
                }
            }
    ok = (fclose(f) == 0) && ok;
    if (!ok) {
        Q3_LOG("wrapper_state_save_file: failed to save to %s", path);
        return -1;
    }
    return 0;
}

int wrapper_state_load_file(void* ctx, const char* path) {
    TalkerCtx* c = (TalkerCtx*)ctx;
    if (!c || !path) return -1;
    FILE* f = fopen(path, "rb");
    if (!f) {
        Q3_LOG("wrapper_state_load_file: failed to load from %s", path);
        return -1;
    }
    int32_t hdr[6];
    bool ok = fread(hdr, sizeof(hdr), 1, f) == 1;
    const int D = c->kv.head_dim;
    ok = ok && hdr[0] == kStateMagic && hdr[1] == 1 && hdr[2] == c->kv.n_layers && hdr[3] == c->kv.n_kv &&
         hdr[4] == D && hdr[5] >= 0 && hdr[5] <= c->n_ctx;
    if (!ok) {
        fclose(f);
        Q3_LOG("wrapper_state_load_file: %s does not match this context", path);
        return -1;
    }
    const int n_pos = hdr[5];
    std::vector<uint16_t> buf((size_t)n_pos * D);
    hipStreamSynchronize(c->s);
    for (int l = 0; l < c->kv.n_layers && ok; l++)
        for (int kvsel = 0; kvsel < 2 && ok; kvsel++)
            for (int g = 0; g < c->kv.n_kv && ok; g++) {
                half_t* base = (kvsel ? c->kv.v : c->kv.k) + l * c->kv.layer_stride() +
                               ((size_t)0 * c->kv.n_kv + g) * (size_t)c->kv.n_ctx * D;
                if (n_pos > 0) {
                    ok = fread(buf.data(), 2, buf.size(), f) == buf.size();
                    ok = ok && hipMemcpy(base, buf.data(), buf.size() * 2, hipMemcpyHostToDevice) == hipSuccess;
                }
            }
    fclose(f);
    if (!ok) {
        Q3_LOG("wrapper_state_load_file: failed to load from %s", path);
        return -1;
    }
    c->n_used[0] = n_pos;
    fprintf(stderr, "wrapper_state_load_file: loaded from %s, n_tokens=%d\n", path, n_pos);
    return 0;
}

}
```

### qwen3_tts_axera_russian_amd/csrc/q3_text_api.hip

```cpp
#include "../../include/qwen3tts_text.h"
#include "q3_model.h"

using namespace q3;

namespace {

typedef _Float16 h8v __attribute__((ext_vector_type(8)));

__device__ __forceinline__ size_t fidx(int m, int k, int K) {
    return ((((size_t)(m >> 4) * (K >> 5) + (k >> 5)) * 64 + (m & 15) + 16 * ((k >> 3) & 3)) << 3) + (k & 7);
}

__global__ void __launch_bounds__(256) text_gather_kernel(const half_t* __restrict__ table, int V, int TD,
                                                          const int* __restrict__ ids, half_t* __restrict__ x16) {
    const int r = blockIdx.x, t = ids[r];
    for (int k8 = threadIdx.x; k8 < TD / 8; k8 += 256) {
        h8v v = {0, 0, 0, 0, 0, 0, 0, 0};
        if (t >= 0 && t < V) v = *(const h8v*)(table + (size_t)t * TD + k8 * 8);
        *(h8v*)(x16 + fidx(r, k8 * 8, TD)) = v;
    }
}
__global__ void __launch_bounds__(256) bias_rows_kernel(const float* __restrict__ bias, int N, float* __restrict__ h) {
    const int r = blockIdx.x;
    for (int n4 = threadIdx.x; n4 < N / 4; n4 += 256) *(float4*)(h + fidx(r, n4 * 4, N)) = *(const float4*)(bias + n4 * 4);
}
__global__ void __launch_bounds__(256) silu_f16_kernel(const float* __restrict__ h, half_t* __restrict__ x16, size_t n) {
    const size_t i = (size_t)blockIdx.x * 256 + threadIdx.x;
    if (i < n) {
        const float v = h[i];
        const float s = v * (1.0f / (1.0f + __expf(-v)));
        x16[i] = (half_t)fminf(fmaxf(s, -65504.f), 65504.f);
    }
}
__global__ void __launch_bounds__(256) prefix_rows_kernel(const float* __restrict__ proj, int H, const int* __restrict__ src,
                                                          const int* __restrict__ cod, const float* __restrict__ codec,
                                                          int codec_vocab, float* __restrict__ out) {
    const int j = blockIdx.x, s = src[j], c = cod[j];
    for (int k4 = threadIdx.x; k4 < H / 4; k4 += 256) {
        float4 v = *(const float4*)(proj + fidx(s, k4 * 4, H));
        if (c >= 0 && c < codec_vocab) {
            const float4 e = *(const float4*)(codec + (size_t)c * H + k4 * 4);
            v.x += e.x;
            v.y += e.y;
            v.z += e.z;
            v.w += e.w;
        }
        *(float4*)(out + (size_t)j * H + k4 * 4) = v;
    }
}

struct TextFE {
    int V = 0, TD = 0, H = 0, codec_vocab = 0, max_rows = 0;
    int special[12] = {151644, 77091, 198, 151671, 151672, 151673, 2148, 2149, 2155, 2156, 2157, 0};
    half_t* table = nullptr;
    DevLinear fc1, fc2;
    float *b1 = nullptr, *b2 = nullptr, *codec = nullptr;
    half_t *x16 = nullptr, *a16 = nullptr;
    float *h1 = nullptr, *h2 = nullptr, *ssq = nullptr, *out = nullptr;
    int *d_ids = nullptr, *d_src = nullptr, *d_cod = nullptr;
    hipStream_t s = nullptr;
    std::vector<void*> allocs;
};

void* dal(TextFE* t, size_t bytes) {
    void* p = nullptr;
    if (hipMalloc(&p, bytes ? bytes : 16) != hipSuccess) return nullptr;
    hipMemset(p, 0, bytes ? bytes : 16);
    t->allocs.push_back(p);
    return p;
}

half_t* upload_f16(TextFE* t, const PackTensor* pt) {
    const size_t ne = pt->numel();
    half_t* d = (half_t*)dal(t, ne * 2);
    if (!d) return nullptr;
    const size_t slice = (size_t)8 << 20;
    std::vector<uint16_t> buf;
    for (size_t o = 0; o < ne; o += slice) {
        const size_t n = ne - o < slice ? ne - o : slice;
        const void* src = nullptr;
        if (pt->dtype == F16) src = (const uint16_t*)pt->data + o;
        else {
            buf.resize(n);
            if (pt->dtype == F32) {
                const float* f = (const float*)pt->data + o;
                for (size_t i = 0; i < n; i++) buf[i] = f2h_sat(f[i]);
            } else if (pt->dtype == BF16) {
                const uint16_t* b = (const uint16_t*)pt->data + o;
                for (size_t i = 0; i < n; i++) buf[i] = f2h_sat(bf16_to_f32(b[i]));
            } else return nullptr;
            src = buf.data();
        }
        if (hipMemcpy(d + o, src, n * 2, hipMemcpyHostToDevice) != hipSuccess) return nullptr;
    }
    return d;
}
float* upload_f32(TextFE* t, const PackTensor* pt) {
    const size_t ne = pt->numel();
    float* d = (float*)dal(t, ne * 4);
    if (!d) return nullptr;
    std::vector<float> tmp;
    const void* src = pt->data;
    if (pt->dtype != F32) {
        tmp.resize(ne);
        const uint16_t* u = (const uint16_t*)pt->data;
        for (size_t i = 0; i < ne; i++) tmp[i] = pt->dtype == BF16 ? bf16_to_f32(u[i]) : h2f(u[i]);
        src = tmp.data();
    }
    return hipMemcpy(d, src, ne * 4, hipMemcpyHostToDevice) == hipSuccess ? d : nullptr;
}
bool pack_linear(TextFE* t, const PackTensor* pt, DevLinear& L) {
    L.N = (int)pt->shape[0];
    L.K = (int)pt->shape[1];
    half_t* rowmajor = upload_f16(t, pt);
    L.wp = (half_t*)dal(t, (size_t)L.N * L.K * 2);
    if (!rowmajor || !L.wp) return false;
    if (launch_pack_linear(t->s, rowmajor, L.N, L.K, L.wp, 0, 1)) return false;
    return hipStreamSynchronize(t->s) == hipSuccess;
}

int project(TextFE* t, int R) {
    hipLaunchKernelGGL(text_gather_kernel, dim3(R), dim3(256), 0, t->s, t->table, t->V, t->TD, t->d_ids, t->x16);
    hipLaunchKernelGGL(bias_rows_kernel, dim3(R), dim3(256), 0, t->s, t->b1, t->fc1.N, t->h1);
    LinArgs a;
    a.wp = t->fc1.wp;
    a.N = t->fc1.N;
    a.K = t->fc1.K;
    a.M = R;
    a.x16 = t->x16;
    a.h_out = t->h1;
    a.ssq_out = t->ssq;
    if (launch_linear(t->s, a, PRO_F16, EPI_RESID)) return -1;
    const int Rp = (R + 15) / 16 * 16;
    const size_t n1 = (size_t)Rp * t->fc1.N;
    hipLaunchKernelGGL(silu_f16_kernel, dim3((unsigned)((n1 + 255) / 256)), dim3(256), 0, t->s, t->h1, t->a16, n1);
    hipLaunchKernelGGL(bias_rows_kernel, dim3(R), dim3(256), 0, t->s, t->b2, t->fc2.N, t->h2);
    a = LinArgs();
    a.wp = t->fc2.wp;
    a.N = t->fc2.N;
    a.K = t->fc2.K;
    a.M = R;
    a.x16 = t->a16;
    a.h_out = t->h2;
    a.ssq_out = t->ssq;
    if (launch_linear(t->s, a, PRO_F16, EPI_RESID)) return -1;
    Q3_HIP(hipGetLastError(), -1);
    return 0;
}

int emit(TextFE* t, const std::vector<int>& ids, const std::vector<int>& src, const std::vector<int>& cod, float* out) {
    const int R = (int)ids.size(), J = (int)src.size();
    if (R > t->max_rows || J > t->max_rows) return -1;
    for (int id : ids)
        if (id < 0 || id >= t->V) {
            Q3_LOG("text front-end: token id %d outside the table of %d rows", id, t->V);
            return -1;
        }
    Q3_HIP(hipMemcpyAsync(t->d_ids, ids.data(), sizeof(int) * R, hipMemcpyHostToDevice, t->s), -1);
    Q3_HIP(hipMemcpyAsync(t->d_src, src.data(), sizeof(int) * J, hipMemcpyHostToDevice, t->s), -1);
    Q3_HIP(hipMemcpyAsync(t->d_cod, cod.data(), sizeof(int) * J, hipMemcpyHostToDevice, t->s), -1);
    if (project(t, R)) return -1;
    hipLaunchKernelGGL(prefix_rows_kernel, dim3(J), dim3(256), 0, t->s, t->h2, t->H, t->d_src, t->d_cod, t->codec, t->codec_vocab,
                       t->out);
    Q3_HIP(hipGetLastError(), -1);
    Q3_HIP(hipMemcpyAsync(out, t->out, sizeof(float) * (size_t)J * t->H, hipMemcpyDeviceToHost, t->s), -1);
    Q3_HIP(hipStreamSynchronize(t->s), -1);
    return J;
}

}

extern "C" {

void tfe_free(void* hh) {
    TextFE* t = (TextFE*)hh;
    if (!t) return;
    if (t->s) hipStreamSynchronize(t->s);
    for (void* p : t->allocs) hipFree(p);
    if (t->s) hipStreamDestroy(t->s);
    delete t;
}

void* tfe_load(const char* weights, const char* embeddings_dir, int max_tokens) {
    int ndev = 0;
    if (hipGetDeviceCount(&ndev) != hipSuccess || ndev <= 0) {
        Q3_LOG("no HIP device available -- this library has no CPU path");
        return nullptr;
    }
    if (!weights && !embeddings_dir) return nullptr;
    Pack p;
    if (!p.open_auto(weights ? weights : embeddings_dir, embeddings_dir)) return nullptr;
    const PackTensor *te = p.find("text.embedding"), *w1 = p.find("text.fc1.weight"), *c1 = p.find("text.fc1.bias"),
                     *w2 = p.find("text.fc2.weight"), *c2 = p.find("text.fc2.bias"), *ce = p.find("talker.codec_embedding");
    if (!te || !w1 || !c1 || !w2 || !c2 || !ce) {
        Q3_LOG("tfe_load: %s lacks text.embedding / text.fc{1,2}.{weight,bias} / talker.codec_embedding", weights ? weights : embeddings_dir);
        return nullptr;
    }
    TextFE* t = new TextFE();
    t->V = (int)te->shape[0];
    t->TD = (int)te->shape[1];
    t->H = (int)w2->shape[0];
    t->codec_vocab = (int)ce->shape[0];
    const int mid = (int)w1->shape[0];
    if (te->ndim != 2 || (int)w1->shape[1] != t->TD || (int)w2->shape[1] != mid || (int)ce->shape[1] != t->H ||
        (t->TD != 1024 && t->TD != 2048 && t->TD != 3072) || (mid != 1024 && mid != 2048 && mid != 3072) || t->H % 128 || mid % 128) {
        Q3_LOG("tfe_load: unsupported geometry table [%d][%d] -> %d -> %d (the GEMM kernels take K in {1024, 2048, 3072}, N %% 128 == 0)",
               t->V, t->TD, mid, t->H);
        delete t;
        return nullptr;
    }
    static const char* keys[12] = {"im_start", "assistant", "newline", "tts_pad", "tts_bos", "tts_eos", "codec_pad", "codec_bos",
                                   "codec_nothink", "codec_think_bos", "codec_think_eos", ""};
    for (int i = 0; i < 11; i++) t->special[i] = (int)p.get(keys[i], (double)t->special[i]);
    t->max_rows = (max_tokens > 0 ? max_tokens : 512) + 16;
    const size_t Rp = ((size_t)t->max_rows + 127) / 128 * 128;
    bool ok = hipStreamCreate(&t->s) == hipSuccess;
    ok = ok && (t->table = upload_f16(t, te)) && pack_linear(t, w1, t->fc1) && pack_linear(t, w2, t->fc2);
    ok = ok && (t->b1 = upload_f32(t, c1)) && (t->b2 = upload_f32(t, c2)) && (t->codec = upload_f32(t, ce));
    ok = ok && (t->x16 = (half_t*)dal(t, Rp * t->TD * 2)) && (t->a16 = (half_t*)dal(t, Rp * mid * 2));
    ok = ok && (t->h1 = (float*)dal(t, Rp * mid * 4)) && (t->h2 = (float*)dal(t, Rp * t->H * 4));
    ok = ok && (t->ssq = (float*)dal(t, Rp * (mid / 16) * 4)) && (t->out = (float*)dal(t, Rp * t->H * 4));
    ok = ok && (t->d_ids = (int*)dal(t, Rp * 4)) && (t->d_src = (int*)dal(t, Rp * 4)) && (t->d_cod = (int*)dal(t, Rp * 4));
    if (!ok) {
        Q3_LOG("tfe_load: upload failed");
        tfe_free(t);
        return nullptr;
    }
    return t;
}

int tfe_hidden_size(void* h) { return h ? ((TextFE*)h)->H : 0; }
int tfe_text_vocab(void* h) { return h ? ((TextFE*)h)->V : 0; }

int tfe_embed_text(void* hh, const int32_t* token_ids, int n, float* out) {
    TextFE* t = (TextFE*)hh;
    if (!t || !token_ids || !out || n <= 0) return -1;
    std::vector<int> ids(token_ids, token_ids + n), src(n), cod(n, -1);
    for (int i = 0; i < n; i++) src[i] = i;
    return emit(t, ids, src, cod, out) == n ? 0 : -1;
}

int tfe_build_prefix(void* hh, const int32_t* text_token_ids, int n, const int32_t* special, float* out) {
    TextFE* t = (TextFE*)hh;
    if (!t || !out || n < 0 || (n > 0 && !text_token_ids)) return -1;
    const int* sp = special ? special : t->special;
    std::vector<int> ids = {sp[0], sp[1], sp[2], sp[3], sp[4], sp[5]};
    ids.insert(ids.end(), text_token_ids, text_token_ids + n);
    std::vector<int> src, cod;
    auto row = [&](int s_, int c_) {
        src.push_back(s_);
        cod.push_back(c_);
    };
    for (int i = 0; i < 3; i++) row(i, -1);
    row(3, sp[8]);
    row(3, sp[9]);
    row(3, sp[10]);
    row(4, sp[6]);
    for (int i = 0; i < n; i++) row(6 + i, sp[6]);
    row(5, sp[6]);
    row(3, sp[7]);
    return emit(t, ids, src, cod, out);
}

int tfe_tts_pad_embed(void* hh, float* out) {
    TextFE* t = (TextFE*)hh;
    if (!t || !out) return -1;
    const int32_t id = t->special[3];
    return tfe_embed_text(t, &id, 1, out);
}

}
```

### qwen3_tts_axera_russian_amd/csrc/q3_voc.hip

```cpp
#include "../../include/qwen3tts_voc.h"
#include "q3_common.h"
#include "q3_voc_ops.h"

#include <algorithm>
#include <cmath>
#include <utility>

namespace q3 {

typedef float f16v __attribute__((ext_vector_type(16)));

enum { VOP_RVQ = 1, VOP_CONV = 2, VOP_CONVT = 3, VOP_DWCONV = 4, VOP_NORM = 5, VOP_ATTN = 6, VOP_GLU = 7, VOP_EMBMEAN = 8 };
enum { VF_SNAKE = 1, VF_RES_ADD = 2, VF_RES_SAVE = 4, VF_CLAMP = 8, VF_GELU = 16 };

__device__ __forceinline__ float gelu_erf(float x) { return 0.5f * x * (1.0f + erff(x * 0.70710678118654752f)); }
__device__ __forceinline__ float elu1(float x) { return x > 0.f ? x : expm1f(x); }


static int g_voc_split = 1;
static int g_voc_max_wgs = 0;
constexpr int VKC = 8;
constexpr int VTN = 128;
#ifndef Q3_VOC_XPAD
#define Q3_VOC_XPAD 1
// ... 1171 lines not shown
    };
    const int t0 = pos - window + 1 > 0 ? pos - window + 1 : 0;
    float q0, q1;
    rope(x + ((size_t)b * 3 * HD + h * D) * x_ld, x_ld, skip + i, pos - t0, q0, q1);
    const float* kb = kv + ((size_t)b * 2 * HD + h * D) * kv_ld;
    const float* vb = kb + (size_t)HD * kv_ld;
    const float scale = 1.0f / sqrtf((float)D);
    float m = -INFINITY, lsum = 0.f, o0 = 0.f, o1 = 0.f;
    for (int t = t0; t <= pos; t++) {
        const int col = Hk + (t - p0);
        float k0, k1;
        rope(kb, kv_ld, col, t - t0, k0, k1);
        float sc = q0 * k0 + q1 * k1;
#pragma unroll
        for (int o = 32; o > 0; o >>= 1) sc += __shfl_xor(sc, o, 64);
        sc *= scale;
        const float mn = fmaxf(m, sc), corr = __expf(m - mn), p = __expf(sc - mn);
        float v0 = 0.f, v1 = 0.f;
        if (on) {
            v0 = vb[(size_t)j * kv_ld + col];
            v1 = vb[(size_t)(j + half) * kv_ld + col];
        }
        lsum = lsum * corr + p;
        o0 = o0 * corr + p * v0;
        o1 = o1 * corr + p * v1;
        m = mn;
    }
    if (on) {
        float* yb = y + ((size_t)b * HD + h * D) * x_ld + skip + i;
        yb[(size_t)j * x_ld] = o0 / lsum;
        yb[(size_t)(j + half) * x_ld] = o1 / lsum;
    }
}

template <typename T>
__global__ void __launch_bounds__(256) voc_incr_emit_kernel(const float* __restrict__ y, int ld, int skip, int n,
                                                            const long long* __restrict__ out_off, T* __restrict__ out) {
    const int b = blockIdx.y;
    const long long o = out_off[b];
    for (int i = blockIdx.x * 256 + threadIdx.x; i < n; i += gridDim.x * 256) voc_store(out, o + i, y[(size_t)b * ld + skip + i]);
}

struct VocOp {
    int op = 0, cin = 0, cout = 0, k = 0, p0 = 0, flags = 0, nq = 0, cb = 0;
    float *w = nullptr, *bias = nullptr, *alpha = nullptr, *inv_beta = nullptr;
    int kind = 0, heads = 0, head_dim = 0, window = 0;
    float eps = 0.f, theta = 10000.f;
    _Float16 *w_hi = nullptr, *w_lo = nullptr;
    int Mp128 = 0;
    float *p_sem = nullptr, *p_ac = nullptr;
    float* w1p = nullptr;
    int lt = 0, rt = 0;
};

static inline long pitch4(long L) { return (L + 31) & ~31L; }
static inline long convt_out(const VocOp& op, long L) { return (L - 1) * op.p0 + op.k - op.lt - op.rt; }
static inline long convt_cols(const VocOp& op, long L) {
    const long lc = (convt_out(op, L) + op.lt + op.p0 - 1) / op.p0;
    return lc < L ? L : lc;
}

struct Voc {
    int device = 0;
    int chunk = 64, max_batch = 1, upsample = 1;
    long chunk_samples = 0;
    std::vector<VocOp> ops;
    std::vector<void*> allocs;
    hipStream_t s = nullptr;
    hipEvent_t e0 = nullptr, e1 = nullptr;
    int64_t* d_codes = nullptr;
    int* d_ovf = nullptr;
    bool warned_ovf = false;
    float *buf[3] = {nullptr, nullptr, nullptr};
    _Float16 *plane[4] = {nullptr, nullptr, nullptr, nullptr};
    size_t buf_elems = 0;
    float last_ms = 0.f;
    double flops_per_chunk = 0.0;
    float* d_wave = nullptr;
    int16_t* d_wave16 = nullptr;
    size_t wave_cap = 0, wave16_cap = 0;
    ChunkPlace* d_place = nullptr;
    float batch_ms = 0.f;
    int batch_chunks = 0;
};

static float* voc_up(Voc* v, const PackTensor* t) {
    size_t ne = t->numel();
    std::vector<float> tmp;
    const float* src = (const float*)t->data;
    if (t->dtype == F16) {
        tmp.resize(ne);
        for (size_t i = 0; i < ne; i++) tmp[i] = h2f(((const uint16_t*)t->data)[i]);
        src = tmp.data();
    } else if (t->dtype != F32) {
        return nullptr;
    }
    float* d = nullptr;
    if (hipMalloc((void**)&d, ne * 4) != hipSuccess) return nullptr;
    v->allocs.push_back(d);
    if (hipMemcpy(d, src, ne * 4, hipMemcpyHostToDevice) != hipSuccess) return nullptr;
    return d;
}

static float* voc_up_host(Voc* v, const std::vector<float>& h) {
    float* d = nullptr;
    if (hipMalloc((void**)&d, h.size() * 4) != hipSuccess) return nullptr;
    v->allocs.push_back(d);
    if (hipMemcpy(d, h.data(), h.size() * 4, hipMemcpyHostToDevice) != hipSuccess) return nullptr;
    return d;
}

static void voc_destroy(Voc* v) {
    if (!v) return;
    if (v->s) hipStreamSynchronize(v->s);
    for (void* p : v->allocs) hipFree(p);
    for (float* b : v->buf)
        if (b) hipFree(b);
    for (_Float16* b : v->plane)
        if (b) hipFree(b);
    if (v->d_codes) hipFree(v->d_codes);
    if (v->d_wave) hipFree(v->d_wave);
    if (v->d_wave16) hipFree(v->d_wave16);
    if (v->d_place) hipFree(v->d_place);
    if (v->d_ovf) hipFree(v->d_ovf);
    if (v->e0) hipEventDestroy(v->e0);
    if (v->e1) hipEventDestroy(v->e1);
    if (v->s) hipStreamDestroy(v->s);
    delete v;
}

}

using namespace q3;

static inline void voc_bind(const Voc* v) {
    int d = -1;
    if (v && (hipGetDevice(&d) != hipSuccess || d != v->device)) hipSetDevice(v->device);
}

extern "C" {

void voc_free(void* vv) {
    voc_bind((Voc*)vv);
    voc_destroy((Voc*)vv);
}

void* voc_load(const char* weights, int chunk_tokens, int max_batch) {
    int ndev = 0;
    if (hipGetDeviceCount(&ndev) != hipSuccess || ndev <= 0) {
        Q3_LOG("no HIP device available -- this library has no CPU path");
        return nullptr;
    }
    if (!weights) return nullptr;
    Pack p;
    if (!p.open(weights)) return nullptr;
    const PackTensor* prog = p.find("voc.program");
    if (!prog || prog->dtype != I32 || prog->ndim != 2 || prog->shape[1] != 8) {
        Q3_LOG("%s holds no vocoder program (tensor voc.program int32 [n][8])", weights);
        return nullptr;
    }
    if (const char* ex = getenv("Q3_VOC_EXACT")) g_voc_split = atoi(ex) ? 0 : 1;
    Voc* v = new Voc();
    hipGetDevice(&v->device);
    v->chunk = chunk_tokens > 0 ? chunk_tokens : 64;
    v->max_batch = max_batch > 0 ? max_batch : 1;
    bool ok = true;
    {
        int lo = 0, hi = 0;
        const bool prio = !(getenv("Q3_STREAM_PRIO") && atoi(getenv("Q3_STREAM_PRIO")) == 0);
        if (prio && hipDeviceGetStreamPriorityRange(&lo, &hi) == hipSuccess && lo != hi)
            ok = hipStreamCreateWithPriority(&v->s, hipStreamNonBlocking, lo) == hipSuccess;
        else
            ok = hipStreamCreateWithFlags(&v->s, hipStreamNonBlocking) == hipSuccess;
    }
    ok = ok && hipEventCreate(&v->e0) == hipSuccess && hipEventCreate(&v->e1) == hipSuccess;
    const int32_t* pr = (const int32_t*)prog->data;
    const int n_ops = (int)prog->shape[0];
    int C = 0;
    long L = v->chunk;
    size_t max_elems = 0;
    double flops = 0.0;
    for (int i = 0; i < n_ops && ok; i++) {
        const int32_t* r = pr + i * 8;
        VocOp op;
        op.op = r[0];
        const std::string base = "voc.op" + std::to_string(i) + ".";
        auto need = [&](const char* n) -> const PackTensor* {
            const PackTensor* t = p.find(base + n);
            if (!t) {
                Q3_LOG("vocoder program op %d needs tensor %s%s", i, base.c_str(), n);
                ok = false;
            }
            return t;
        };
        if (op.op == VOP_EMBMEAN) {
            op.nq = r[1];
            op.cb = r[2];
            op.cout = r[3];
            const PackTensor* tb = need("embedding");
            if (!ok) break;
            if (op.nq < 1 || op.nq > 16 || tb->numel() != (uint64_t)op.nq * op.cb * op.cout) {
                Q3_LOG("vocoder op %d: embedding table size does not match the program (1..16 quantisers)", i);
                ok = false;
                break;
            }
            op.w = voc_up(v, tb);
            ok = op.w != nullptr;
            C = op.cout;
        } else if (op.op == VOP_RVQ) {
            op.nq = r[1];
            op.cb = r[2];
            op.cin = r[3];
            op.cout = r[4];
            const PackTensor *cb = need("codebook"), *ps = need("proj_sem"), *pa = need("proj_ac");
            if (!ok) break;
            if (op.nq < 1 || op.nq > 16) {
                Q3_LOG("vocoder op %d: %d quantisers (a request carries 16 ids per frame)", i, op.nq);
                ok = false;
                break;
            }
            if (cb->numel() != (uint64_t)op.nq * op.cb * op.cin || ps->numel() != (uint64_t)op.cout * op.cin ||
                pa->numel() != (uint64_t)op.cout * op.cin) {
                Q3_LOG("vocoder op %d: RVQ tensor sizes do not match the program", i);
                ok = false;
                break;
            }
            op.w = voc_up(v, cb);
            op.p_sem = voc_up(v, ps);
            op.p_ac = voc_up(v, pa);
            ok = op.w && op.p_sem && op.p_ac;
            C = op.cout;
            flops += 2.0 * 2 * op.cin * op.cout * L;
        } else if (op.op == VOP_CONV || op.op == VOP_CONVT) {
            op.cin = r[1];
            op.cout = r[2];
            op.k = r[3];
            op.p0 = r[4];
            op.flags = r[5];
            if (op.op == VOP_CONVT) {
                op.lt = r[6];
                op.rt = r[7];
                if (op.lt < 0 || op.rt < 0 || op.p0 <= 0 || op.lt + op.rt > op.k || convt_out(op, L) <= 0) {
                    Q3_LOG("vocoder op %d: transposed conv k=%d s=%d cannot be trimmed by %d + %d", i, op.k, op.p0, op.lt, op.rt);
                    ok = false;
                    break;
                }
            }
            if (op.cin != C) {
                Q3_LOG("vocoder op %d: expects %d input channels, previous op produced %d", i, op.cin, C);
                ok = false;
                break;
            }
            const PackTensor *wt = need("weight"), *bs = p.find(base + "bias");
            if (!ok) break;
            if (wt->numel() != (uint64_t)op.cin * op.cout * op.k || wt->dtype != F32) {
                Q3_LOG("vocoder op %d: weight size/dtype does not match the program", i);
                ok = false;
                break;
            }
            const float* src = (const float*)wt->data;
            std::vector<float> wk;
            if (op.op == VOP_CONV) {
                wk.resize((size_t)op.k * op.cout * op.cin);
                for (int co = 0; co < op.cout; co++)
                    for (int ci = 0; ci < op.cin; ci++)
                        for (int k = 0; k < op.k; k++)
                            wk[((size_t)k * op.cout + co) * op.cin + ci] = src[((size_t)co * op.cin + ci) * op.k + k];
            } else {
                const int s = op.p0;
                const int J = s > 0 ? op.k / s : 0;
                if (s <= 0 || J < 1 || op.k != J * s) {
                    Q3_LOG("vocoder op %d: transposed conv needs kernel = J*stride (got k=%d s=%d)", i, op.k, s);
                    ok = false;
                    break;
                }
                wk.resize((size_t)J * op.cout * s * op.cin);
                for (int j = 0; j < J; j++)
                    for (int co = 0; co < op.cout; co++)
                        for (int ph = 0; ph < s; ph++)
                            for (int ci = 0; ci < op.cin; ci++)
                                wk[((size_t)(J - 1 - j) * op.cout * s + (size_t)co * s + ph) * op.cin + ci] =
                                    src[((size_t)ci * op.cout + co) * op.k + ph + j * s];
            }
            if (op.cin % 16 == 0) {
                const int KTAPS = op.op == VOP_CONV ? op.k : op.k / op.p0;
                const int Mrows = op.op == VOP_CONV ? op.cout : op.cout * op.p0;
                const int Mp = Mrows % 96 == 0 ? Mrows : (Mrows + 127) / 128 * 128;
                std::vector<uint16_t> hi((size_t)(op.cin / 16) * KTAPS * Mp * 16, 0), lo(hi.size(), 0);
                bool in_range = true;
                for (int k = 0; k < KTAPS; k++)
                    for (int m = 0; m < Mrows; m++)
                        for (int ci = 0; ci < op.cin; ci++) {
                            const float wv = wk[((size_t)k * Mrows + m) * op.cin + ci];
                            in_range = in_range && fabsf(wv) <= 65504.f;
                            const uint16_t h = f2h_sat(wv);
                            const size_t d = ((((size_t)(ci >> 4) * KTAPS + k) * Mp) + m) * 16 + (ci & 15);
                            hi[d] = h;
                            lo[d] = f2h_sat((wv - h2f(h)) * 2048.0f);
                        }
                void *dh = nullptr, *dl = nullptr;
                if (in_range) {
                    if (hipMalloc(&dh, hi.size() * 2) != hipSuccess || hipMalloc(&dl, lo.size() * 2) != hipSuccess) {
                        ok = false;
                        break;
                    }
                    v->allocs.push_back(dh);
                    v->allocs.push_back(dl);
                    ok = hipMemcpy(dh, hi.data(), hi.size() * 2, hipMemcpyHostToDevice) == hipSuccess &&
                         hipMemcpy(dl, lo.data(), lo.size() * 2, hipMemcpyHostToDevice) == hipSuccess;
                    op.w_hi = (_Float16*)dh;
                    op.w_lo = (_Float16*)dl;
                    op.Mp128 = Mp;
                    if (!ok) break;
                }
            }
            if (op.op == VOP_CONV && op.k == 1 && op.cin == op.cout && resunit_channels(op.cin) &&
                (op.flags & VF_RES_ADD) && (op.flags & VF_SNAKE)) {
                const int Cc = op.cin;
                std::vector<float> w1((size_t)Cc * Cc);
                for (int t2 = 0; t2 < Cc / 32; t2++)
                    for (int t = 0; t < Cc / 2; t++)
                        for (int ln = 0; ln < 64; ln++) {
                            const int mt = t / 16, q = t % 16, h = ln >> 5, m = ln & 31;
                            const int c = 32 * mt + (q & 3) + 8 * (q >> 2) + 4 * h;
                            w1[((size_t)t2 * (Cc / 2) + t) * 64 + ln] = wk[(size_t)(32 * t2 + m) * Cc + c];
                        }
                op.w1p = voc_up_host(v, w1);
                if (!op.w1p) {
                    ok = false;
                    break;
                }
            }
            {
                const int KTAPS = op.op == VOP_CONV ? op.k : op.k / op.p0;
                const int Mrows = op.op == VOP_CONV ? op.cout : op.cout * op.p0;
                const int Mp = (Mrows + 3) / 4 * 4;
                std::vector<float> wp((size_t)(op.cin / 8) * KTAPS * 8 * Mp, 0.f);
                for (int k = 0; k < KTAPS; k++)
                    for (int m = 0; m < Mrows; m++)
                        for (int ci = 0; ci < op.cin; ci++)
                            wp[((((size_t)(ci >> 3) * KTAPS + k) * 8 + (ci & 7)) * Mp) + m] =
                                wk[((size_t)k * Mrows + m) * op.cin + ci];
                wk.swap(wp);
            }
            op.w = voc_up_host(v, wk);
            op.bias = bs ? voc_up(v, bs) : nullptr;
            if (op.flags & VF_SNAKE) {
                const PackTensor *al = need("alpha"), *be = need("beta");
                if (!ok) break;
                std::vector<float> ha(op.cin), hb(op.cin);
                for (int c = 0; c < op.cin; c++) {
                    const float av = al->dtype == F32 ? ((const float*)al->data)[c] : h2f(((const uint16_t*)al->data)[c]);
                    const float bv = be->dtype == F32 ? ((const float*)be->data)[c] : h2f(((const uint16_t*)be->data)[c]);
                    ha[c] = expf(av);
                    hb[c] = 1.0f / (expf(bv) + 1e-9f);
                }
                op.alpha = voc_up_host(v, ha);
                op.inv_beta = voc_up_host(v, hb);
            }
            if (op.cin % 8) {
                Q3_LOG("vocoder op %d: Cin=%d is not a multiple of 8", i, op.cin);
                ok = false;
                break;
            }
            ok = ok && op.w;
            flops += 2.0 * op.cin * op.cout * op.k * L;
            C = op.cout;
            if (op.op == VOP_CONVT) L = convt_out(op, L);
        } else if (op.op == VOP_DWCONV || op.op == VOP_NORM || op.op == VOP_ATTN || op.op == VOP_GLU) {
            op.cin = r[1];
            op.cout = r[2];
            op.flags = r[5];
            if (op.cin != C) {
                Q3_LOG("vocoder op %d: expects %d input channels, previous op produced %d", i, op.cin, C);
                ok = false;
                break;
            }
            auto vec = [&](const char* n, uint64_t ne, bool required) -> float* {
                const PackTensor* t = p.find(base + n);
                if (!t) {
                    if (required) {
                        Q3_LOG("vocoder program op %d needs tensor %s%s", i, base.c_str(), n);
                        ok = false;
                    }
                    return nullptr;
                }
                if (t->numel() != ne) {
                    Q3_LOG("vocoder op %d: tensor %s has %llu elements, the program needs %llu", i, n,
                           (unsigned long long)t->numel(), (unsigned long long)ne);
                    ok = false;
                    return nullptr;
                }
                float* d = voc_up(v, t);
                if (!d) ok = false;
                return d;
            };
            if (op.op == VOP_DWCONV) {
                op.k = r[3];
                if (op.cout != op.cin || op.k < 1 || op.k > 64) ok = false;
                op.w = vec("weight", (uint64_t)op.cin * op.k, true);
                op.bias = vec("bias", (uint64_t)op.cin, false);
                flops += 2.0 * op.cin * op.k * L;
            } else if (op.op == VOP_NORM) {
                op.kind = r[3];
                op.eps = (float)((double)r[4] * 1e-9);
                if (op.cout != op.cin || (op.kind != 0 && op.kind != 1)) ok = false;
                op.w = vec("weight", (uint64_t)op.cin, true);
                op.bias = vec("bias", (uint64_t)op.cin, false);
            } else if (op.op == VOP_ATTN) {
                op.heads = r[3];
                op.head_dim = r[4];
                op.window = r[6];
                op.theta = (float)r[7];
                if (op.heads <= 0 || op.head_dim <= 0 || op.head_dim > 128 || (op.head_dim & 1) || op.window <= 0 ||
                    op.cin != 3 * op.heads * op.head_dim || op.cout != op.heads * op.head_dim)
                    ok = false;
                flops += 4.0 * op.heads * op.head_dim * (double)(op.window < L ? op.window : L) * L;
            } else {
                op.kind = r[3];
                if (op.cin != 2 * op.cout || (op.kind != 0 && op.kind != 1)) ok = false;
            }
            if (!ok) {
                Q3_LOG("vocoder op %d: malformed program row / tensors", i);
                break;
            }
            C = op.cout;
            if ((size_t)op.cin * pitch4(L) > max_elems) max_elems = (size_t)op.cin * pitch4(L);
        } else {
            Q3_LOG("vocoder program op %d: unknown opcode %d", i, op.op);
            ok = false;
            break;
        }
        if ((size_t)C * pitch4(L) > max_elems) max_elems = (size_t)C * pitch4(L);
        v->ops.push_back(op);
    }
    if (ok && C != 1) {
        Q3_LOG("vocoder program must end with 1 channel (got %d)", C);
        ok = false;
    }
    if (ok) {
        long up = 1;
        for (const VocOp& o : v->ops)
            if (o.op == VOP_CONVT) up *= o.p0;
        v->upsample = (int)up;
        v->chunk_samples = L;
        if (L > (long)v->chunk * up) {
            Q3_LOG("vocoder program yields %ld samples for %d frames, more than %ld per frame", L, v->chunk, up);
            ok = false;
        }
    }
    if (ok) {
        v->flops_per_chunk = flops;
        v->buf_elems = max_elems * v->max_batch;
        for (int i = 0; i < 3 && ok; i++)
            ok = hipMalloc((void**)&v->buf[i], v->buf_elems * 4) == hipSuccess && hipMemset(v->buf[i], 0, v->buf_elems * 4) == hipSuccess;
        for (int i = 0; i < 4 && ok; i++) ok = hipMalloc((void**)&v->plane[i], v->buf_elems * 2) == hipSuccess;
        ok = ok && hipMalloc((void**)&v->d_codes, sizeof(int64_t) * 16 * v->chunk * v->max_batch) == hipSuccess;
        ok = ok && hipMalloc((void**)&v->d_ovf, 16) == hipSuccess && hipMemset(v->d_ovf, 0, 16) == hipSuccess;
        ok = ok && hipMalloc((void**)&v->d_place, sizeof(ChunkPlace) * v->max_batch) == hipSuccess;
    }
    if (!ok) {
        Q3_LOG("voc_load failed");
        voc_destroy(v);
        return nullptr;
    }
    return v;
}

int voc_set_exact_fp32(int on) {
    g_voc_split = on ? 0 : 1;
    return 0;
}

int voc_set_narrow_k1(int on) {
    g_voc_narrow_k1 = on ? 1 : 0;
    return 0;
}

int voc_set_fused_units(int on) {
    g_voc_fuse = on ? 1 : 0;
    return 0;
}

int voc_set_max_workgroups(int n) {
    if (n < 0) {
        int dev = 0;
        hipDeviceProp_t p;
        n = (hipGetDevice(&dev) == hipSuccess && hipGetDeviceProperties(&p, dev) == hipSuccess) ? p.multiProcessorCount : 0;
    }
    g_voc_max_wgs = n;
    return n;
}

int voc_chunk_tokens(void* vv) { return vv ? ((Voc*)vv)->chunk : 0; }
int voc_samples_per_token(void* vv) { return vv ? ((Voc*)vv)->upsample : 0; }
int voc_chunk_samples(void* vv) { return vv ? (int)((Voc*)vv)->chunk_samples : 0; }
float voc_last_decode_ms(void* vv) { return vv ? ((Voc*)vv)->last_ms : -1.f; }
double voc_decode_flops(void* vv, int B) { return vv ? ((Voc*)vv)->flops_per_chunk * B : 0.0; }

struct SplitState {
    int f32_idx = 0;
    bool f32_cur = true;
    int planes = -1;
    float* res = nullptr;
};

static bool split_capable(const VocOp& op) { return (op.op == VOP_CONV || op.op == VOP_CONVT) && op.w_hi != nullptr; }

static int voc_conv_split(Voc* v, const VocOp& op, const VocOp* next, bool last, int B, int C, long L, SplitState& st) {
    const int KT = op.op == VOP_CONV ? op.k : op.k / op.p0;
    int in_set = st.planes;
    if (in_set < 0) {
        if (!st.f32_cur) return -1;
        in_set = 0;
        hipLaunchKernelGGL(snake_split_kernel, dim3((unsigned)((L + 255) / 256), op.cin / 8, B), dim3(256), 0, v->s,
                           v->buf[st.f32_idx], op.alpha, op.inv_beta, v->plane[0], v->plane[1], op.cin, (int)L, (int)pitch4(L),
                           (op.flags & VF_GELU) ? 1 : 0, v->d_ovf);
        Q3_HIP(hipGetLastError(), -1);
    }
    if (op.flags & VF_RES_SAVE) {
        if (!st.f32_cur) return -1;
        st.res = v->buf[st.f32_idx];
    }
    const bool want_planes = next && split_capable(*next) && op.op == VOP_CONV && op.cout % 16 == 0 && !(next->flags & VF_GELU);
    const bool want_f32 = !want_planes || last || (next->flags & VF_RES_SAVE);
    SplitArgs sa;
    sa.xh = v->plane[2 * in_set];
    sa.xl = v->plane[2 * in_set + 1];
    sa.w_hi = op.w_hi;
    sa.w_lo = op.w_lo;
    sa.bias = op.bias;
    sa.ovf = v->d_ovf;
    sa.res = (op.flags & VF_RES_ADD) ? st.res : nullptr;
    sa.Cin = op.cin;
    sa.Cout = op.cout;
    sa.Mp = op.Mp128;
    sa.Lin = (int)L;
    sa.clamp = (op.flags & VF_CLAMP) ? 1 : 0;
    if (op.op == VOP_CONV) {
        sa.dil = op.p0;
        sa.stride = 1;
        sa.M = op.cout;
// ... 125 lines not shown
            st.f32_idx = cur;
            st.f32_cur = true;
            st.planes = -1;
            if (op_ms) {
                hipEventRecord(v->e1, v->s);
                hipStreamSynchronize(v->s);
                hipEventElapsedTime(&op_ms[i], v->e0, v->e1);
                op_ms[i + 1] = 0.f;
            }
            i++;
            continue;
        } else {
            if (!st.f32_cur) return -1;
            cur = st.f32_idx;
            in = v->buf[cur];
            out = v->buf[cur ^ 1];
            ConvArgs a;
            a.x = in;
            a.y = out;
            a.wk = op.w;
            a.bias = op.bias;
            a.alpha = op.alpha;
            a.inv_beta = op.inv_beta;
            a.Cin = op.cin;
            a.Cout = op.cout;
            a.Lin = (int)L;
            a.clamp = (op.flags & VF_CLAMP) ? 1 : 0;
            a.gelu = (op.flags & VF_GELU) ? 1 : 0;
            a.ldx = ld;
            if (op.op == VOP_CONV) {
                a.K = op.k;
                a.dil = op.p0;
                a.stride = 1;
                a.M = op.cout;
                a.Lout = a.Lc = (int)L;
                a.Lrule = (int)Lf;
            } else {
                a.K = op.k / op.p0;
                a.dil = 1;
                a.stride = op.p0;
                a.M = op.cout * op.p0;
                a.lt = op.lt;
                a.Lout = (int)convt_out(op, L);
                a.Lc = (int)convt_cols(op, L);
                a.Lrule = (int)convt_cols(op, Lf);
            }
            a.ldy = (int)pitch4(a.Lout);
            if (op.flags & VF_RES_SAVE) {
                std::swap(v->buf[2], v->buf[cur]);
                res = st.res = v->buf[2];
                a.x = res;
            }
            if (op.flags & VF_RES_ADD) a.res = res ? res : st.res;
            if (launch_conv(v->s, a, B)) return -1;
            C = op.cout;
            if (op.op == VOP_CONVT) L = convt_out(op, L), Lf = convt_out(op, Lf);
            cur ^= 1;
            st.f32_idx = cur;
            st.f32_cur = true;
            st.planes = -1;
        }
        if (op_ms) {
            hipEventRecord(v->e1, v->s);
            hipStreamSynchronize(v->s);
            hipEventElapsedTime(&op_ms[i], v->e0, v->e1);
        }
    }
    if (!st.f32_cur) return -1;
    *out_dev = v->buf[st.f32_idx];
    if (outC) *outC = C;
    if (outL) *outL = L;
    return 0;
}

int voc_decode(void* vv, const int64_t* codes, int B, float* out) {
    Voc* v = (Voc*)vv;
    voc_bind(v);
    if (!v || !codes || !out || B <= 0 || B > v->max_batch) return -1;
    Q3_HIP(hipMemcpyAsync(v->d_codes, codes, sizeof(int64_t) * 16 * (size_t)v->chunk * B, hipMemcpyHostToDevice, v->s), -1);
    Q3_HIP(hipEventRecord(v->e0, v->s), -1);
    float* res = nullptr;
    if (voc_run(v, B, &res)) return -1;
    Q3_HIP(hipEventRecord(v->e1, v->s), -1);
    int ovf = 0;
    if (g_voc_split) Q3_HIP(hipMemcpyAsync(&ovf, v->d_ovf, sizeof(int), hipMemcpyDeviceToHost, v->s), -1);
    const size_t row = sizeof(float) * (size_t)v->chunk_samples, dpitch = sizeof(float) * (size_t)pitch4(v->chunk_samples);
    Q3_HIP(hipMemcpy2DAsync(out, row, res, dpitch, row, (size_t)B, hipMemcpyDeviceToHost, v->s), -1);
    Q3_HIP(hipStreamSynchronize(v->s), -1);
    if (ovf) {
        if (!v->warned_ovf) Q3_LOG("vocoder: activation outside the fp16 range, decoding this call with the exact-fp32 path");
        v->warned_ovf = true;
        Q3_HIP(hipMemsetAsync(v->d_ovf, 0, sizeof(int), v->s), -1);
        Q3_HIP(hipEventRecord(v->e0, v->s), -1);
        if (voc_run(v, B, &res, -1, nullptr, nullptr, nullptr, true)) return -1;
        Q3_HIP(hipEventRecord(v->e1, v->s), -1);
        Q3_HIP(hipMemcpy2DAsync(out, row, res, dpitch, row, (size_t)B, hipMemcpyDeviceToHost, v->s), -1);
        Q3_HIP(hipStreamSynchronize(v->s), -1);
    }
    hipEventElapsedTime(&v->last_ms, v->e0, v->e1);
    return 0;
}

int voc_debug_profile(void* vv, int B, float* op_ms, int max_ops) {
    Voc* v = (Voc*)vv;
    voc_bind(v);
    if (!v || B <= 0 || B > v->max_batch || (int)v->ops.size() > max_ops) return -1;
    float* res = nullptr;
    if (voc_run(v, B, &res, -1, nullptr, nullptr, op_ms)) return -1;
    return (int)v->ops.size();
}

int voc_debug_run(void* vv, const int64_t* codes, int B, int n_ops, float* out, int* C, int* L) {
    Voc* v = (Voc*)vv;
    voc_bind(v);
    if (!v || B <= 0 || B > v->max_batch) return -1;
    Q3_HIP(hipMemcpyAsync(v->d_codes, codes, sizeof(int64_t) * 16 * (size_t)v->chunk * B, hipMemcpyHostToDevice, v->s), -1);
    float* res = nullptr;
    long LL = 0;
    if (voc_run(v, B, &res, n_ops, C, &LL)) return -1;
    *L = (int)LL;
    Q3_HIP(hipMemcpy2DAsync(out, sizeof(float) * (size_t)LL, res, sizeof(float) * (size_t)pitch4(LL), sizeof(float) * (size_t)LL,
                            (size_t)B * (*C), hipMemcpyDeviceToHost, v->s), -1);
    Q3_HIP(hipStreamSynchronize(v->s), -1);
    return 0;
}

static int voc_decode_frames(const Voc* v, int len) {
    static const int full = getenv("Q3_VOC_FULL_CHUNKS") ? atoi(getenv("Q3_VOC_FULL_CHUNKS")) : 0;
    static const int rnd = getenv("Q3_VOC_FRAME_ROUND") ? atoi(getenv("Q3_VOC_FRAME_ROUND")) : 8;
    if (full || g_voc_split || len >= v->chunk) return v->chunk;
    const int r = rnd > 0 ? rnd : 1;
    const int t = (len + 1 + r - 1) / r * r;
    return t < v->chunk ? t : v->chunk;
}

int voc_synthesize_max_samples(void* vv, int n) {
    Voc* v = (Voc*)vv;
    if (!v || n <= 0) return 0;
    return (n + v->chunk) * v->upsample;
}

namespace {
struct WalkChunk { int utt, start, len; size_t cl; int head; long long dst; };

long long plan_walk(const Voc* v, int u, int n, long long base, std::vector<WalkChunk>& out) {
    const int CH = v->chunk, SPT = v->upsample;
    const size_t CS = (size_t)v->chunk_samples, OV = (size_t)16 * SPT;
    if (n > CH && CH <= 32) {
        Q3_LOG("vocoder chunk walk: chunk_tokens=%d is too short for the 16-frame overlap walk (need > 32)", CH);
        return -1;
    }
    auto sliced = [&](int len) -> size_t { return (size_t)len * SPT < CS ? (size_t)len * SPT : CS; };
    if (n <= CH) {
        out.push_back({u, 0, n, sliced(n), 0, base});
        return (long long)sliced(n);
    }
    size_t have = 0;
    for (int start = 0; start < n; start += CH - 16) {
        const int len = (start + CH <= n) ? CH : n - start;
        const size_t cl = sliced(len);
        if (start == 0) {
            out.push_back({u, start, len, cl, 0, base});
            have = cl;
        } else if (have >= OV && cl >= OV) {
            out.push_back({u, start, len, cl, (int)OV, base + (long long)(have - OV)});
            have += cl - OV;
        } else {
            out.push_back({u, start, len, cl, 0, base + (long long)have});
            have += cl;
        }
    }
    return (long long)have;
}

extern "C++" {
template <class ChunkCodes, class Restore>
int decode_walk(Voc* v, const std::vector<WalkChunk>& walk, ChunkCodes chunk_codes, float* wave, Restore restore, int* n_calls) {
    const int CH = v->chunk, OV = 16 * v->upsample;
    std::vector<int> order(walk.size()), frames(walk.size());
    for (size_t i = 0; i < walk.size(); i++) order[i] = (int)i, frames[i] = voc_decode_frames(v, walk[i].len);
    std::stable_sort(order.begin(), order.end(), [&](int x, int y) { return frames[x] > frames[y]; });
    std::vector<int64_t> padded((size_t)v->max_batch * CH * 16);
    std::vector<ChunkPlace> place(v->max_batch);
    bool redo_exact = false;
    for (int attempt = 0; attempt < 2; attempt++) {
        Q3_HIP(hipEventRecord(v->e0, v->s), -1);
        if (restore()) return -1;
        int calls = 0;
        for (size_t c0 = 0; c0 < walk.size();) {
            const int T = frames[order[c0]];
            int B = 0;
            while (c0 + B < walk.size() && B < v->max_batch && frames[order[c0 + B]] == T) B++;
            std::fill(padded.begin(), padded.begin() + (size_t)B * T * 16, 0);
            for (int b = 0; b < B; b++) {
                const WalkChunk& w = walk[order[c0 + b]];
                memcpy(padded.data() + (size_t)b * T * 16, chunk_codes(order[c0 + b]), sizeof(int64_t) * 16 * w.len);
                place[b] = {b, (int)w.cl, w.head, w.dst};
            }
            Q3_HIP(hipMemcpyAsync(v->d_codes, padded.data(), sizeof(int64_t) * 16 * (size_t)T * B, hipMemcpyHostToDevice, v->s), -1);
            Q3_HIP(hipMemcpyAsync(v->d_place, place.data(), sizeof(ChunkPlace) * B, hipMemcpyHostToDevice, v->s), -1);
            float* res = nullptr;
            long LL = 0;
            if (voc_run(v, B, &res, -1, nullptr, &LL, nullptr, redo_exact, T)) return -1;
            for (int b = 0; b < B; b++)
                if ((long)place[b].len > LL) {
                    Q3_LOG("vocoder chunk walk: a decode of %d frames yields %ld samples, fewer than the %d kept", T, LL, place[b].len);
                    return -1;
                }
            const int pitch = (int)pitch4(LL);
            hipLaunchKernelGGL(voc_place_copy_kernel, dim3(64, B), dim3(256), 0, v->s, res, pitch, v->d_place, wave);
            hipLaunchKernelGGL(voc_place_blend_kernel, dim3(32, B), dim3(256), 0, v->s, res, pitch, v->d_place, wave, OV);
            Q3_HIP(hipGetLastError(), -1);
            Q3_HIP(hipStreamSynchronize(v->s), -1);
            c0 += B;
            calls++;
        }
        Q3_HIP(hipEventRecord(v->e1, v->s), -1);
        int ovf = 0;
        if (g_voc_split && !redo_exact) Q3_HIP(hipMemcpyAsync(&ovf, v->d_ovf, sizeof(int), hipMemcpyDeviceToHost, v->s), -1);
        Q3_HIP(hipStreamSynchronize(v->s), -1);
        *n_calls = calls;
        if (!ovf) break;
        if (!v->warned_ovf) Q3_LOG("vocoder: activation outside the fp16 range, decoding this request with the exact-fp32 path");
        v->warned_ovf = true;
        Q3_HIP(hipMemsetAsync(v->d_ovf, 0, sizeof(int), v->s), -1);
        redo_exact = true;
    }
    return 0;
}

template <typename T>
int grow(T** p, size_t* cap, size_t n) {
    if (n <= *cap) return 0;
    if (*p) hipFree(*p);
    *p = nullptr;
    *cap = 0;
    Q3_HIP(hipMalloc((void**)p, sizeof(T) * n), -1);
    *cap = n;
    return 0;
}

}

int synth_batch(Voc* v, const int64_t* codes, const int32_t* n_tokens, int U, int64_t* offsets, bool want16, void* out, int64_t cap) {
    voc_bind(v);
    if (!v || !codes || !n_tokens || !offsets || !out || U <= 0) return -1;
    std::vector<WalkChunk> walk;
    std::vector<size_t> code_off(U);
    long long total = 0;
    size_t coff = 0;
    for (int u = 0; u < U; u++) {
        if (n_tokens[u] <= 0) {
            Q3_LOG("voc_synthesize_batch: utterance %d has %d frames", u, n_tokens[u]);
            return -1;
        }
        const long long len = plan_walk(v, u, n_tokens[u], total, walk);
        if (len < 0) return -1;
        offsets[u] = total;
        code_off[u] = coff;
        coff += (size_t)n_tokens[u] * 16;
        total += len;
    }
    offsets[U] = total;
    if (total > cap) {
        Q3_LOG("voc_synthesize_batch: %lld samples do not fit the caller's buffer of %lld", total, (long long)cap);
        return -1;
    }
    if (grow(&v->d_wave, &v->wave_cap, (size_t)total)) return -1;
    int calls = 0;
    if (decode_walk(v, walk, [&](int c) { return codes + code_off[walk[c].utt] + (size_t)walk[c].start * 16; }, v->d_wave,
                    [] { return 0; }, &calls))
        return -1;
    hipEventElapsedTime(&v->batch_ms, v->e0, v->e1);
    v->batch_chunks = (int)walk.size();
    if (!want16) {
        Q3_HIP(hipMemcpyAsync(out, v->d_wave, sizeof(float) * (size_t)total, hipMemcpyDeviceToHost, v->s), -1);
    } else {
        if (grow(&v->d_wave16, &v->wave16_cap, (size_t)total)) return -1;
        hipLaunchKernelGGL(voc_to_int16_kernel, dim3((unsigned)((total + 255) / 256)), dim3(256), 0, v->s, v->d_wave, v->d_wave16, total);
        Q3_HIP(hipGetLastError(), -1);
        Q3_HIP(hipMemcpyAsync(out, v->d_wave16, sizeof(int16_t) * (size_t)total, hipMemcpyDeviceToHost, v->s), -1);
    }
    Q3_HIP(hipStreamSynchronize(v->s), -1);
    return 0;
}

struct StreamState {
    int n_frames = 0;
    int n_chunks = 0;
    long long have = 0;
    long long emitted = 0;
    bool finished = false;
    int frame_base = 0;
    std::vector<int64_t> frames;
};

struct VocStream {
    Voc* v = nullptr;
    int max_streams = 0;
    std::vector<StreamState> st;
    float* d_tail = nullptr;
    float* d_work = nullptr;
    size_t work_cap = 0;
    float* d_out = nullptr;
    int16_t* d_out16 = nullptr;
    size_t out_cap = 0, out16_cap = 0;
    StreamWin* d_win = nullptr;
    int last_calls = 0, last_chunks = 0;
    float last_ms = 0.f;
};

struct PushPlan {
    std::vector<WalkChunk> walk;
    std::vector<long long> have, n_out;
    std::vector<int> n_chunks;
};

int plan_push(const VocStream* s, int n, const int32_t* streams, const int32_t* n_new, const int32_t* finish, PushPlan& p) {
    const Voc* v = s->v;
    const int CH = v->chunk;
    const long long OV = 16LL * v->upsample;
    if (n < 0 || (n > 0 && (!streams || !n_new))) return -1;
    p.walk.clear();
    p.have.assign(n, 0);
    p.n_out.assign(n, 0);
    p.n_chunks.assign(n, 0);
    std::vector<char> seen(s->max_streams, 0);
    std::vector<WalkChunk> full;
    for (int i = 0; i < n; i++) {
        const int k = streams[i];
        if (k < 0 || k >= s->max_streams || seen[k] || n_new[i] < 0) {
            Q3_LOG("voc_stream_push: entry %d: bad stream %d (or named twice) or %d new frames", i, k, n_new[i]);
            return -1;
        }
        seen[k] = 1;
        const StreamState& t = s->st[k];
        if (t.finished) {
            Q3_LOG("voc_stream_push: stream %d has finished (voc_stream_reset starts the next utterance)", k);
            return -1;
        }
        const bool fin = finish && finish[i];
        const int N = t.n_frames + n_new[i];
        p.have[i] = t.have;
        p.n_chunks[i] = t.n_chunks;
        if (N > 0) {
            full.clear();
            const long long total = plan_walk(v, i, N, 0, full);
            if (total < 0) return -1;
            int c = t.n_chunks;
            for (; c < (int)full.size() && (fin || full[c].start + CH <= N); c++) {
                p.walk.push_back(full[c]);
                p.have[i] = full[c].dst + (long long)full[c].cl;
            }
            p.n_chunks[i] = c;
            if (fin && p.have[i] != total) return -1;
        }
        p.n_out[i] = fin ? p.have[i] - t.emitted : std::max(0LL, p.have[i] - OV - t.emitted);
    }
    return 0;
}

int stream_push(VocStream* s, int n, const int32_t* streams, const int64_t* codes, const int32_t* n_new, const int32_t* finish,
                bool want16, void* out, int64_t cap, int64_t* offsets) {
    if (!s || !offsets) return -1;
    Voc* v = s->v;
    voc_bind(v);
    const int CH = v->chunk, OV = 16 * v->upsample;
    PushPlan p;
    if (plan_push(s, n, streams, n_new, finish, p)) return -1;
    long long total = 0;
    for (int i = 0; i < n; i++) offsets[i] = total, total += p.n_out[i];
    offsets[n] = total;
    if (total > cap || (total > 0 && !out)) {
        Q3_LOG("voc_stream_push: %lld samples do not fit the caller's buffer of %lld", total, (long long)cap);
        return -1;
    }
    std::vector<StreamWin> win;
    std::vector<long long> win_of(n, -1);
    long long work = 0;
    for (int i = 0; i < n; i++) {
        const StreamState& t = s->st[streams[i]];
        const bool fin = finish && finish[i];
        if (p.n_chunks[i] == t.n_chunks && p.n_out[i] == 0) continue;
        const long long size = p.have[i] - t.emitted;
        win_of[i] = work;
        win.push_back({work, offsets[i], p.n_out[i], streams[i], (int)(t.have - t.emitted), fin ? 0 : OV});
        if (!fin && size - p.n_out[i] != OV) return -1;
        work += size;
    }
    for (WalkChunk& c : p.walk) {
        const StreamState& t = s->st[streams[c.utt]];
        if (c.dst < t.emitted || c.dst + (long long)c.cl > p.have[c.utt]) return -1;
        c.dst = win_of[c.utt] + (c.dst - t.emitted);
    }
    size_t need = 0;
    for (int i = 0; i < n; i++) need += (size_t)n_new[i];
    if (need > 0 && !codes) return -1;
    size_t coff = 0;
    for (int i = 0; i < n; i++) {
        StreamState& t = s->st[streams[i]];
        t.frames.insert(t.frames.end(), codes + coff, codes + coff + (size_t)n_new[i] * 16);
        t.n_frames += n_new[i];
        coff += (size_t)n_new[i] * 16;
    }
    s->last_calls = 0;
    s->last_chunks = (int)p.walk.size();
    s->last_ms = 0.f;
    if (!win.empty()) {
        if (grow(&s->d_work, &s->work_cap, (size_t)work)) return -1;
        Q3_HIP(hipMemcpyAsync(s->d_win, win.data(), sizeof(StreamWin) * win.size(), hipMemcpyHostToDevice, v->s), -1);
        const dim3 grid(64, (unsigned)win.size());
        auto load = [&]() -> int {
            hipLaunchKernelGGL(voc_stream_load_kernel, grid, dim3(256), 0, v->s, s->d_tail, OV, s->d_win, s->d_work);
            Q3_HIP(hipGetLastError(), -1);
            return 0;
        };
        if (p.walk.empty()) {
            if (load()) return -1;
        } else {
            auto chunk_codes = [&](int c) {
                const WalkChunk& w = p.walk[c];
                const StreamState& t = s->st[streams[w.utt]];
                return t.frames.data() + (size_t)(w.start - t.frame_base) * 16;
            };
            if (decode_walk(v, p.walk, chunk_codes, s->d_work, load, &s->last_calls)) return -1;
            hipEventElapsedTime(&s->last_ms, v->e0, v->e1);
        }
        if (total > 0 && want16) {
            if (grow(&s->d_out16, &s->out16_cap, (size_t)total)) return -1;
            hipLaunchKernelGGL(voc_stream_emit_kernel<int16_t>, grid, dim3(256), 0, v->s, s->d_work, s->d_win, s->d_tail, OV, s->d_out16);
        } else if (total > 0) {
            if (grow(&s->d_out, &s->out_cap, (size_t)total)) return -1;
            hipLaunchKernelGGL(voc_stream_emit_kernel<float>, grid, dim3(256), 0, v->s, s->d_work, s->d_win, s->d_tail, OV, s->d_out);
        } else {
            hipLaunchKernelGGL(voc_stream_emit_kernel<float>, grid, dim3(256), 0, v->s, s->d_work, s->d_win, s->d_tail, OV, (float*)nullptr);
        }
        Q3_HIP(hipGetLastError(), -1);
        if (total > 0)
            Q3_HIP(hipMemcpyAsync(out, want16 ? (void*)s->d_out16 : (void*)s->d_out, (want16 ? sizeof(int16_t) : sizeof(float)) * (size_t)total,
                                  hipMemcpyDeviceToHost, v->s), -1);
        Q3_HIP(hipStreamSynchronize(v->s), -1);
    }
    for (int i = 0; i < n; i++) {
        StreamState& t = s->st[streams[i]];
        t.have = p.have[i];
        t.emitted += p.n_out[i];
        t.n_chunks = p.n_chunks[i];
        if (finish && finish[i]) {
            t.finished = true;
            std::vector<int64_t>().swap(t.frames);
            continue;
        }
        const int keep_from = t.n_chunks * (CH - 16);
        if (keep_from > t.frame_base) {
            t.frames.erase(t.frames.begin(), t.frames.begin() + (size_t)(keep_from - t.frame_base) * 16);
            t.frame_base = keep_from;
        }
    }
    return 0;
}
}

int64_t voc_synthesize_batch_max_samples(void* vv, const int32_t* n_tokens, int U) {
    Voc* v = (Voc*)vv;
    if (!v || !n_tokens || U <= 0) return 0;
    int64_t t = 0;
    for (int u = 0; u < U; u++) t += n_tokens[u] > 0 ? (int64_t)voc_synthesize_max_samples(v, n_tokens[u]) : 0;
    return t;
}

int voc_synthesize_batch_f32(void* vv, const int64_t* codes, const int32_t* n_tokens, int U, float* out, int64_t out_capacity,
                             int64_t* offsets) {
    return synth_batch((Voc*)vv, codes, n_tokens, U, offsets, false, out, out_capacity);
}

int voc_synthesize_batch(void* vv, const int64_t* codes, const int32_t* n_tokens, int U, int16_t* out, int64_t out_capacity,
                         int64_t* offsets) {
    return synth_batch((Voc*)vv, codes, n_tokens, U, offsets, true, out, out_capacity);
}

int voc_synthesize_f32(void* vv, const int64_t* codes, int n, float* out, int32_t* n_samples) {
    int64_t offsets[2];
    if (!n_samples || synth_batch((Voc*)vv, codes, &n, 1, offsets, false, out, voc_synthesize_max_samples(vv, n))) return -1;
    *n_samples = (int32_t)offsets[1];
    return 0;
}

int voc_synthesize(void* vv, const int64_t* codes, int n, int16_t* out, int32_t* n_samples) {
    int64_t offsets[2];
    if (!n_samples || synth_batch((Voc*)vv, codes, &n, 1, offsets, true, out, voc_synthesize_max_samples(vv, n))) return -1;
    *n_samples = (int32_t)offsets[1];
    return 0;
}

void* voc_stream_create(void* vv, int max_streams) {
    Voc* v = (Voc*)vv;
    if (!v || max_streams <= 0) return nullptr;
    voc_bind(v);
    VocStream* s = new VocStream;
    s->v = v;
    s->max_streams = max_streams;
    s->st.resize(max_streams);
    const size_t OV = (size_t)16 * v->upsample;
    if (hipMalloc((void**)&s->d_tail, sizeof(float) * OV * max_streams) != hipSuccess ||
        hipMalloc((void**)&s->d_win, sizeof(StreamWin) * max_streams) != hipSuccess) {
        Q3_LOG("voc_stream_create: device allocation failed");
        voc_stream_free(s);
        return nullptr;
    }
    return s;
}

void voc_stream_free(void* ss) {
    VocStream* s = (VocStream*)ss;
    if (!s) return;
    voc_bind(s->v);
    hipStreamSynchronize(s->v->s);
    for (void* p : {(void*)s->d_tail, (void*)s->d_work, (void*)s->d_out, (void*)s->d_out16, (void*)s->d_win})
        if (p) hipFree(p);
    delete s;
}

int voc_stream_reset(void* ss, int stream) {
// ... 312 lines not shown
        }
        if (n_new[i] == 0) continue;
        if (s->n_frames[k] + n_new[i] > 0x7fffffffLL) {
            Q3_LOG("voc_incr_push: stream %d is beyond 2^31 frames", k);
            return -1;
        }
        incr_key(v, s->n_frames[k], s->n_frames[k] + n_new[i], key);
        p.n_out[i] = key[nops];
        size_t g = 0;
        while (g < p.keys.size() && (p.keys[g] != key || (int)p.members[g].size() >= v->max_batch)) g++;
        if (g == p.keys.size()) {
            p.keys.push_back(key);
            p.members.emplace_back();
        }
        p.members[g].push_back(i);
    }
    (void)finish;
    return 0;
}

int incr_push(VocIncr* s, int n, const int32_t* streams, const int64_t* codes, const int32_t* n_new, const int32_t* finish,
              bool want16, void* out, int64_t cap, int64_t* offsets) {
    if (!s || !offsets) return -1;
    Voc* v = s->v;
    voc_bind(v);
    IncrPlan p;
    if (incr_plan(s, n, streams, n_new, finish, p)) return -1;
    long long total = 0;
    size_t frames = 0;
    std::vector<size_t> coff(n, 0);
    for (int i = 0; i < n; i++) {
        offsets[i] = total;
        total += p.n_out[i];
        coff[i] = frames * 16;
        frames += (size_t)n_new[i];
    }
    offsets[n] = total;
    if (total > cap || (total > 0 && !out) || (frames > 0 && !codes) || (size_t)total > s->out_cap) {
        Q3_LOG("voc_incr_push: %lld samples do not fit the caller's buffer of %lld (or no codes given)", total, (long long)cap);
        return -1;
    }
    const size_t nops = v->ops.size();
    const int mb = v->max_batch;
    std::vector<int64_t> hcodes;
    std::vector<int> meta((1 + nops) * mb);
    std::vector<long long> off(mb), before;
    s->last_launches = 0;
    s->last_ms = 0.f;
    if (!p.keys.empty()) Q3_HIP(hipEventRecord(v->e0, v->s), -1);
    for (size_t g = 0; g < p.keys.size(); g++) {
        const std::vector<int>& mem = p.members[g];
        const int B = (int)mem.size(), T = n_new[mem[0]];
        hcodes.resize((size_t)B * T * 16);
        std::fill(meta.begin(), meta.end(), 0);
        for (int b = 0; b < B; b++) {
            const int e = mem[b], k = streams[e];
            memcpy(hcodes.data() + (size_t)b * T * 16, codes + coff[e], sizeof(int64_t) * 16 * T);
            incr_chain(v, s->n_frames[k], before);
            meta[b] = k;
            for (size_t i = 0; i < nops; i++) meta[(1 + i) * mb + b] = (int)before[i];
            off[b] = offsets[e];
        }
        Q3_HIP(hipMemcpyAsync(s->d_codes, hcodes.data(), sizeof(int64_t) * hcodes.size(), hipMemcpyHostToDevice, v->s), -1);
        Q3_HIP(hipMemcpyAsync(s->d_meta, meta.data(), sizeof(int) * meta.size(), hipMemcpyHostToDevice, v->s), -1);
        Q3_HIP(hipMemcpyAsync(s->d_off, off.data(), sizeof(long long) * B, hipMemcpyHostToDevice, v->s), -1);
        float* y = nullptr;
        int ld = 0, skip = 0;
        if (incr_walk(s, p.keys[g], B, false, nullptr, nullptr, &s->last_launches, &y, &ld, &skip)) return -1;
        const long long ns = p.keys[g][nops];
        if (ns > 0) {
            const dim3 grid((unsigned)std::min<long long>(64, (ns + 255) / 256), B);
            if (want16)
                hipLaunchKernelGGL(voc_incr_emit_kernel<int16_t>, grid, dim3(256), 0, v->s, y, ld, skip, (int)ns, s->d_off, s->d_out16);
            else
                hipLaunchKernelGGL(voc_incr_emit_kernel<float>, grid, dim3(256), 0, v->s, y, ld, skip, (int)ns, s->d_off, s->d_out);
            Q3_HIP(hipGetLastError(), -1);
            s->last_launches++;
        }
        Q3_HIP(hipStreamSynchronize(v->s), -1);
    }
    if (!p.keys.empty()) {
        Q3_HIP(hipEventRecord(v->e1, v->s), -1);
        if (total > 0)
            Q3_HIP(hipMemcpyAsync(out, want16 ? (void*)s->d_out16 : (void*)s->d_out, (want16 ? sizeof(int16_t) : sizeof(float)) * (size_t)total,
                                  hipMemcpyDeviceToHost, v->s), -1);
        Q3_HIP(hipStreamSynchronize(v->s), -1);
        hipEventElapsedTime(&s->last_ms, v->e0, v->e1);
    }
    for (int i = 0; i < n; i++) {
        s->n_frames[streams[i]] += n_new[i];
        if (finish && finish[i]) s->finished[streams[i]] = 1;
    }
    return 0;
}

void incr_destroy(VocIncr* s) {
    if (!s) return;
    for (void* p : {(void*)s->d_hist, (void*)s->buf[0], (void*)s->buf[1], (void*)s->buf[2], (void*)s->d_kv, (void*)s->d_codes,
                    (void*)s->d_meta, (void*)s->d_off, (void*)s->d_out, (void*)s->d_out16})
        if (p) hipFree(p);
    delete s;
}
}

extern "C" {

int64_t voc_incr_samples(void* vv, int64_t n_frames) {
    const Voc* v = (const Voc*)vv;
    if (!v || n_frames < 0) return -1;
    std::vector<long long> in;
    incr_chain(v, n_frames, in);
    return in.back();
}

void voc_incr_free(void* ss) {
    VocIncr* s = (VocIncr*)ss;
    if (!s) return;
    voc_bind(s->v);
    hipStreamSynchronize(s->v->s);
    incr_destroy(s);
}

void* voc_incr_create(void* vv, int max_streams) {
    Voc* v = (Voc*)vv;
    if (!v || max_streams <= 0) return nullptr;
    voc_bind(v);
    VocIncr* s = new VocIncr;
    s->v = v;
    s->max_streams = max_streams;
    s->n_frames.assign(max_streams, 0);
    s->finished.assign(max_streams, 0);
    const size_t nops = v->ops.size();
    s->H.assign(nops, 0);
    s->hoff.assign(nops, 0);
    for (size_t i = 0; i < nops; i++) {
        const VocOp& op = v->ops[i];
        if (op.op == VOP_CONVT && (op.rt != op.k - op.p0 || op.lt > op.p0)) {
            Q3_LOG("voc_incr_create: op %zu: a transposed conv k=%d s=%d trimmed %d + %d cannot be streamed (right trim must be k - s)", i,
                   op.k, op.p0, op.lt, op.rt);
            delete s;
            return nullptr;
        }
        s->H[i] = incr_hist_cols(op);
        if (s->H[i] > 256 || (op.op == VOP_ATTN && op.head_dim > 128)) {
            Q3_LOG("voc_incr_create: op %zu carries %d columns, more than the 256 the history kernel holds", i, s->H[i]);
            delete s;
            return nullptr;
        }
        s->hoff[i] = s->state_floats;
        s->state_floats += (size_t)s->H[i] * incr_hist_chans(op);
    }
    size_t need = 0, need_kv = 0;
    std::vector<long long> key;
    bool ok = true;
    for (long long prev : {0LL, (long long)v->chunk}) {
        int launches = 0;
        incr_key(v, prev, prev + v->chunk, key);
        ok = ok && incr_walk(s, key, v->max_batch, true, &need, &need_kv, &launches, nullptr, nullptr, nullptr) == 0;
    }
    if (!ok) {
        Q3_LOG("voc_incr_create: the vocoder program cannot be run incrementally");
        delete s;
        return nullptr;
    }
    const size_t mb = (size_t)v->max_batch;
    const size_t buf_elems = need * mb + 1024, kv_elems = need_kv * mb + 1024;
    s->out_cap = (size_t)max_streams * v->chunk * v->upsample;
    auto alloc = [&](void** p, size_t bytes, bool zero) {
        if (!ok) return;
        ok = hipMalloc(p, bytes) == hipSuccess && (!zero || hipMemset(*p, 0, bytes) == hipSuccess);
        if (ok) s->device_bytes += bytes;
    };
    alloc((void**)&s->d_hist, sizeof(float) * std::max<size_t>(1, s->state_floats * max_streams), true);
    for (int i = 0; i < 3; i++) alloc((void**)&s->buf[i], sizeof(float) * buf_elems, true);
    alloc((void**)&s->d_kv, sizeof(float) * kv_elems, true);
    alloc((void**)&s->d_codes, sizeof(int64_t) * 16 * v->chunk * mb, false);
    alloc((void**)&s->d_meta, sizeof(int) * (1 + nops) * mb, false);
    alloc((void**)&s->d_off, sizeof(long long) * mb, false);
    alloc((void**)&s->d_out, sizeof(float) * s->out_cap, false);
    alloc((void**)&s->d_out16, sizeof(int16_t) * s->out_cap, false);
    if (!ok) {
        Q3_LOG("voc_incr_create: device allocation failed");
        incr_destroy(s);
        return nullptr;
    }
    return s;
}

int voc_incr_reset(void* ss, int stream) {
    VocIncr* s = (VocIncr*)ss;
    if (!s || stream < 0 || stream >= s->max_streams) return -1;
    voc_bind(s->v);
    if (s->state_floats)
        Q3_HIP(hipMemsetAsync(s->d_hist + (size_t)stream * s->state_floats, 0, sizeof(float) * s->state_floats, s->v->s), -1);
    s->n_frames[stream] = 0;
    s->finished[stream] = 0;
    return 0;
}

int64_t voc_incr_push_max_samples(void* ss, int n, const int32_t* streams, const int32_t* n_new, const int32_t* finish) {
    VocIncr* s = (VocIncr*)ss;
    IncrPlan p;
    if (!s || incr_plan(s, n, streams, n_new, finish, p)) return -1;
    int64_t t = 0;
    for (int i = 0; i < n; i++) t += p.n_out[i];
    return t;
}

int voc_incr_push(void* s, int n, const int32_t* streams, const int64_t* codes, const int32_t* n_new, const int32_t* finish,
                  int16_t* out, int64_t out_capacity, int64_t* offsets) {
    return incr_push((VocIncr*)s, n, streams, codes, n_new, finish, true, out, out_capacity, offsets);
}

int voc_incr_push_f32(void* s, int n, const int32_t* streams, const int64_t* codes, const int32_t* n_new, const int32_t* finish,
                      float* out, int64_t out_capacity, int64_t* offsets) {
    return incr_push((VocIncr*)s, n, streams, codes, n_new, finish, false, out, out_capacity, offsets);
}

float voc_incr_last_ms(void* s) { return s ? ((VocIncr*)s)->last_ms : -1.f; }
int voc_incr_last_launches(void* s) { return s ? ((VocIncr*)s)->last_launches : -1; }
int64_t voc_incr_state_bytes(void* s) { return s ? (int64_t)(((VocIncr*)s)->state_floats * sizeof(float)) : -1; }
int64_t voc_incr_device_bytes(void* s) { return s ? (int64_t)((VocIncr*)s)->device_bytes : -1; }

}
```

Measured before the change: 9166 codec_frames/s.

## Replace blocking memcpys with stream-ordered async copies and extend two-row CP seeding to chains

```diff
diff --git a/qwen3_tts_axera_russian_amd/csrc/q3_cp_api.hip b/qwen3_tts_axera_russian_amd/csrc/q3_cp_api.hip
--- a/qwen3_tts_axera_russian_amd/csrc/q3_cp_api.hip
+++ b/qwen3_tts_axera_russian_amd/csrc/q3_cp_api.hip
@@ -9,10 +9,12 @@
 }
 
 int cp_seed_row0(const Work& w, int R, int row0, int R_total) {
+    (void)R;
+    (void)row0;
     if (R_total <= 0) R_total = R;
-    const int R16 = (R + 15) / 16 * 16;
-    const bool two = two_row_enabled() && row0 == 0 && R_total == R && 2 * R16 <= w.max_rows;
-    return two ? R16 : 0;
+    const int B16 = (R_total + 15) / 16 * 16;
+    const bool two = two_row_enabled() && 2 * B16 <= w.max_rows;
+    return two ? B16 : 0;
 }
 
 int cp_frame(hipStream_t s, const Model& m, Work& w, KVCache& kv, int R, const CpFrameIO& io, int row0, int R_total) {
@@ -24,7 +26,22 @@
     rm.slot_base = 0;
     rm.slot_stride = 1;
     rm.pos_stride = 0;
-    if (seed0 > 0) {
+    if (seed0 > 0 && (row0 != 0 || R_total != R)) {
+        RowMap r0;
+        r0.slot_base = -seed0;
+        r0.slot_stride = 1;
+        r0.pos_base = 0;
+        r0.pos_stride = 0;
+        r0.same_slot_rows = true;
+        if (run_stack(s, m, m.cp, w, kv, R, r0, 256, seed0 + row0)) return -1;
+        if (launch_gather_embed(s, m.talker_emb, c.talker_vocab, H, io.codes, 0, io.n_frames, io.frame_cap, 0, w.h, w.ssq, R,
+                                row0, R_total, io.forced, w.xh, m.cp.L[0].in_ln))
+            return -1;
+        RowMap r1 = rm;
+        r1.pos_base = 1;
+        r1.same_slot_rows = true;
+        if (run_stack(s, m, m.cp, w, kv, R, r1, 256, row0)) return -1;
+    } else if (seed0 > 0) {
         const int R16 = seed0;
         if (w.map_R16 != R16) {
             std::vector<int> slot(2 * R16), pos(2 * R16);
@@ -147,20 +164,26 @@
 void* cp_load(const char* weights, const char* embeddings_dir, int max_batch) {
     if (!weights) return nullptr;
     if (max_batch <= 0) max_batch = 1;
-    Model* m = model_load(weights, false, true, embeddings_dir);
-    if (!m) return nullptr;
+    hipStream_t s = nullptr;
+    if (hipStreamCreate(&s) != hipSuccess) return nullptr;
+    Model* m = model_load(weights, false, true, embeddings_dir, s);
+    if (!m) {
+        hipStreamDestroy(s);
+        return nullptr;
+    }
     CpHandle* h = new CpHandle();
     h->m = m;
+    h->s = s;
     h->max_batch = max_batch;
     const ModelCfg& c = m->cfg;
-    bool ok = hipStreamCreate(&h->s) == hipSuccess;
-    ok = ok && kv_alloc(h->kv, c.cp_layers, max_batch, c.n_kv, c.cp_groups + 1) == 0;
-    ok = ok && work_alloc(h->w, c, 2 * ((max_batch + 15) / 16 * 16), c.cp_ffn, c.cp_vocab) == 0;
+    bool ok = kv_alloc(h->kv, c.cp_layers, max_batch, c.n_kv, c.cp_groups + 1, h->s) == 0;
+    ok = ok && work_alloc(h->w, c, 2 * ((max_batch + 15) / 16 * 16), c.cp_ffn, c.cp_vocab, h->s) == 0;
     ok = ok && hipMalloc((void**)&h->d_codes, sizeof(int) * 16 * max_batch) == hipSuccess;
     ok = ok && hipMalloc((void**)&h->d_nframes, sizeof(int) * max_batch) == hipSuccess;
     if (ok) {
         std::vector<int> ones(max_batch, 1);
-        ok = hipMemcpy(h->d_nframes, ones.data(), sizeof(int) * max_batch, hipMemcpyHostToDevice) == hipSuccess;
+        ok = hipMemcpyAsync(h->d_nframes, ones.data(), sizeof(int) * max_batch, hipMemcpyHostToDevice, h->s) == hipSuccess &&
+             hipStreamSynchronize(h->s) == hipSuccess;
     }
     if (!ok) {
         Q3_LOG("cp_load: allocation failed");
diff --git a/qwen3_tts_axera_russian_amd/csrc/q3_engine.hip b/qwen3_tts_axera_russian_amd/csrc/q3_engine.hip
--- a/qwen3_tts_axera_russian_amd/csrc/q3_engine.hip
+++ b/qwen3_tts_axera_russian_amd/csrc/q3_engine.hip
@@ -34,10 +34,13 @@
     hipEvent_t ev0 = nullptr, ev1 = nullptr;
     float last_run_ms = 0.f, last_prefill_ms = 0.f, last_host_launch_ms = 0.f;
     int* h_done = nullptr;
+    int* h_read = nullptr;
     float t_temp = 0.f, t_top_p = 0.95f, c_temp = 0.f;
     int t_top_k = 50, c_top_k = 50;
     unsigned long long seed = 0;
     int n_chains = 1;
+    bool use_prio = false;
+    int prio_hi = 0;
     hipStream_t cs[8] = {nullptr};
     hipEvent_t ev_fork = nullptr, ev_join[8] = {nullptr};
     bool slot_mode = false;
@@ -136,6 +139,7 @@
     rm.slot_base = 0;
     rm.slot_stride = 1;
     rm.pos = e->d_posdec;
+    rm.rows_total = e->B;
     if (run_stack(st, m, m.talker, e->wt, e->kv_t, R, rm, 1024, row0)) return -1;
     return talker_tail(e, st, row0, R);
 }
@@ -152,23 +156,44 @@
     R = e->B / nc + (c < e->B % nc ? 1 : 0);
 }
 
+bool make_stream(const Engine* e, hipStream_t* st) {
+    return (e->use_prio ? hipStreamCreateWithPriority(st, hipStreamNonBlocking, e->prio_hi)
+                        : hipStreamCreateWithFlags(st, hipStreamNonBlocking)) == hipSuccess;
+}
+
+int ensure_chains(Engine* e, int n) {
+    if (n < 2) return 0;
+    if (!e->ev_fork) Q3_HIP(hipEventCreateWithFlags(&e->ev_fork, hipEventDisableTiming), -1);
+    for (int c = 0; c < n; c++) {
+        if (!e->cs[c] && !make_stream(e, &e->cs[c])) return -1;
+        if (!e->ev_join[c]) Q3_HIP(hipEventCreateWithFlags(&e->ev_join[c], hipEventDisableTiming), -1);
+    }
+    return 0;
+}
+
+hipStream_t chain_stream(const Engine* e, int c) { return n_chains_eff(e) == 1 ? e->s : e->cs[c]; }
+
 int frame_eager(Engine* e) {
     const int nc = n_chains_eff(e);
     for (int c = 0; c < nc; c++) {
         int row0, R;
         chain_rows(e, c, row0, R);
-        if (frame_chain(e, e->cs[c], row0, R)) return -1;
+        if (frame_chain(e, chain_stream(e, c), row0, R)) return -1;
     }
     return 0;
 }
 
 int fork_chains(Engine* e) {
+    const int nc = n_chains_eff(e);
+    if (nc == 1) return 0;
     Q3_HIP(hipEventRecord(e->ev_fork, e->s), -1);
-    for (int c = 0; c < n_chains_eff(e); c++) Q3_HIP(hipStreamWaitEvent(e->cs[c], e->ev_fork, 0), -1);
+    for (int c = 0; c < nc; c++) Q3_HIP(hipStreamWaitEvent(e->cs[c], e->ev_fork, 0), -1);
     return 0;
 }
 int join_chains(Engine* e) {
-    for (int c = 0; c < n_chains_eff(e); c++) {
+    const int nc = n_chains_eff(e);
+    if (nc == 1) return 0;
+    for (int c = 0; c < nc; c++) {
         Q3_HIP(hipEventRecord(e->ev_join[c], e->cs[c]), -1);
         Q3_HIP(hipStreamWaitEvent(e->s, e->ev_join[c], 0), -1);
     }
@@ -193,6 +218,7 @@
     for (void* p : ps)
         if (p) hipFree(p);
     if (e->h_done) hipHostFree(e->h_done);
+    if (e->h_read) hipHostFree(e->h_read);
     for (int c = 0; c < 8; c++) {
         if (e->cs[c]) hipStreamDestroy(e->cs[c]);
         if (e->ev_join[c]) hipEventDestroy(e->ev_join[c]);
@@ -207,39 +233,40 @@
 
 void* q3e_create(const char* weights, int max_batch, int n_ctx, int max_frames) {
     if (!weights || max_batch <= 0 || n_ctx <= 0 || max_frames <= 0) return nullptr;
-    Model* m = model_load(weights, true, true);
-    if (!m) return nullptr;
+    Engine* e = new Engine();
+    int prio_lo = 0, prio_hi = 0;
+    e->use_prio = !(getenv("Q3_STREAM_PRIO") && atoi(getenv("Q3_STREAM_PRIO")) == 0) &&
+                  hipDeviceGetStreamPriorityRange(&prio_lo, &prio_hi) == hipSuccess && prio_lo != prio_hi;
+    e->prio_hi = prio_hi;
+    if (!make_stream(e, &e->s)) {
+        Q3_LOG("q3e_create: no stream");
+        q3e_free(e);
+        return nullptr;
+    }
+    Model* m = model_load(weights, true, true, nullptr, e->s);
+    if (!m) {
+        q3e_free(e);
+        return nullptr;
+    }
+    e->m = m;
     if (n_ctx > m->max_pos) {
         Q3_LOG("q3e_create: n_ctx=%d exceeds the RoPE table (%d)", n_ctx, m->max_pos);
-        model_free(m);
+        q3e_free(e);
         return nullptr;
     }
-    Engine* e = new Engine();
-    e->m = m;
     e->max_batch = max_batch;
     e->n_ctx = n_ctx;
     e->max_frames = max_frames;
     const ModelCfg& c = m->cfg;
     e->prefill_rows = max_batch > 2048 ? max_batch : 2048;
-    int prio_lo = 0, prio_hi = 0;
-    const bool use_prio = !(getenv("Q3_STREAM_PRIO") && atoi(getenv("Q3_STREAM_PRIO")) == 0) &&
-                          hipDeviceGetStreamPriorityRange(&prio_lo, &prio_hi) == hipSuccess && prio_lo != prio_hi;
-    auto mkstream = [&](hipStream_t* st) {
-        return (use_prio ? hipStreamCreateWithPriority(st, hipStreamNonBlocking, prio_hi)
-                         : hipStreamCreateWithFlags(st, hipStreamNonBlocking)) == hipSuccess;
-    };
-    bool ok = mkstream(&e->s);
-    ok = ok && hipEventCreate(&e->ev0) == hipSuccess && hipEventCreate(&e->ev1) == hipSuccess;
-    ok = ok && hipEventCreateWithFlags(&e->ev_fork, hipEventDisableTiming) == hipSuccess;
-    for (int c = 0; c < 8 && ok; c++)
-        ok = mkstream(&e->cs[c]) &&
-             hipEventCreateWithFlags(&e->ev_join[c], hipEventDisableTiming) == hipSuccess;
+    bool ok = hipEventCreate(&e->ev0) == hipSuccess && hipEventCreate(&e->ev1) == hipSuccess;
     if (const char* nc = getenv("Q3_CHAINS")) e->n_chains = atoi(nc) < 1 ? 1 : atoi(nc) > 8 ? 8 : atoi(nc);
     else e->n_chains = 1;
-    ok = ok && kv_alloc(e->kv_t, c.talker_layers, max_batch, c.n_kv, n_ctx) == 0;
-    ok = ok && kv_alloc(e->kv_c, c.cp_layers, max_batch, c.n_kv, c.cp_groups + 1) == 0;
-    ok = ok && work_alloc(e->wt, c, e->prefill_rows, c.talker_ffn, c.talker_vocab) == 0;
-    ok = ok && work_alloc(e->wc, c, 2 * ((max_batch + 15) / 16 * 16), c.cp_ffn, c.cp_vocab) == 0;
+    ok = ok && ensure_chains(e, e->n_chains) == 0;
+    ok = ok && kv_alloc(e->kv_t, c.talker_layers, max_batch, c.n_kv, n_ctx, e->s) == 0;
+    ok = ok && kv_alloc(e->kv_c, c.cp_layers, max_batch, c.n_kv, c.cp_groups + 1, e->s) == 0;
+    ok = ok && work_alloc(e->wt, c, e->prefill_rows, c.talker_ffn, c.talker_vocab, e->s) == 0;
+    ok = ok && work_alloc(e->wc, c, 2 * ((max_batch + 15) / 16 * 16), c.cp_ffn, c.cp_vocab, e->s) == 0;
     auto ialloc = [&](int** p, size_t n) { return hipMalloc((void**)p, sizeof(int) * n) == hipSuccess; };
     ok = ok && ialloc(&e->d_slot, e->prefill_rows) && ialloc(&e->d_pos, e->prefill_rows);
     ok = ok && ialloc(&e->d_tiles, (size_t)4 * e->prefill_rows);
@@ -250,13 +277,15 @@
     ok = ok && ialloc(&e->d_codes, (size_t)max_frames * max_batch * 16);
     ok = ok && hipMalloc((void**)&e->d_pad, sizeof(float) * c.hidden) == hipSuccess;
     ok = ok && hipMalloc((void**)&e->d_seed, sizeof(unsigned long long) * max_batch) == hipSuccess;
-    ok = ok && hipMemset(e->d_seed, 0, sizeof(unsigned long long) * max_batch) == hipSuccess;
+    ok = ok && hipMemsetAsync(e->d_seed, 0, sizeof(unsigned long long) * max_batch, e->s) == hipSuccess;
     ok = ok && hipHostMalloc((void**)&e->h_done, sizeof(int) * max_batch, 0) == hipSuccess;
+    ok = ok && hipHostMalloc((void**)&e->h_read, sizeof(int) * ((size_t)max_batch + (size_t)max_frames * max_batch * 16), 0) == hipSuccess;
     if (ok) {
         std::vector<int> iota(max_batch);
         for (int i = 0; i < max_batch; i++) iota[i] = i;
-        ok = hipMemcpy(e->d_iota, iota.data(), sizeof(int) * max_batch, hipMemcpyHostToDevice) == hipSuccess;
-        ok = ok && hipMemset(e->d_pad, 0, sizeof(float) * c.hidden) == hipSuccess;
+        ok = hipMemcpyAsync(e->d_iota, iota.data(), sizeof(int) * max_batch, hipMemcpyHostToDevice, e->s) == hipSuccess;
+        ok = ok && hipMemsetAsync(e->d_pad, 0, sizeof(float) * c.hidden, e->s) == hipSuccess;
+        ok = hipStreamSynchronize(e->s) == hipSuccess && ok;
     }
     if (!ok) {
         Q3_LOG("q3e_create: allocation failed");
@@ -293,8 +322,9 @@
         if (e->B <= 0 || n_frames > e->max_frames) return -1;
         const size_t total = (size_t)e->max_frames * e->max_batch * 16;
         if (!e->d_forced) Q3_HIP(hipMalloc((void**)&e->d_forced, sizeof(int) * total), -1);
-        Q3_HIP(hipMemset(e->d_forced, 0xff, sizeof(int) * total), -1);
-        Q3_HIP(hipMemcpy(e->d_forced, forced, sizeof(int) * 16 * (size_t)e->B * n_frames, hipMemcpyHostToDevice), -1);
+        Q3_HIP(hipMemsetAsync(e->d_forced, 0xff, sizeof(int) * total, e->s), -1);
+        Q3_HIP(hipMemcpyAsync(e->d_forced, forced, sizeof(int) * 16 * (size_t)e->B * n_frames, hipMemcpyHostToDevice, e->s), -1);
+        Q3_HIP(hipStreamSynchronize(e->s), -1);
     }
     if (on != e->forced_on) {
         e->forced_on = on;
@@ -307,6 +337,7 @@
     Engine* e = (Engine*)ee;
     if (!e || n < 1 || n > 8) return -1;
     if (n != e->n_chains) {
+        if (ensure_chains(e, n)) return -1;
         e->n_chains = n;
         for (auto& g : e->graph) g.reset();
     }
@@ -316,7 +347,8 @@
 int q3e_set_pad_embed(void* ee, const float* pad) {
     Engine* e = (Engine*)ee;
     if (!e || !pad) return -1;
-    Q3_HIP(hipMemcpy(e->d_pad, pad, sizeof(float) * e->m->cfg.hidden, hipMemcpyHostToDevice), -1);
+    Q3_HIP(hipMemcpyAsync(e->d_pad, pad, sizeof(float) * e->m->cfg.hidden, hipMemcpyHostToDevice, e->s), -1);
+    Q3_HIP(hipStreamSynchronize(e->s), -1);
     return 0;
 }
 
@@ -383,7 +415,7 @@
             f.out_copy_ssq = e->wc.ssq;
             f.out_copy_xh = e->wc.xh;
             f.out_copy_gamma = m.cp.L[0].in_ln;
-            f.out_copy_row_off = n_chains_eff(e) == 1 ? cp_seed_row0(e->wc, B_total, 0, B_total) : 0;
+            f.out_copy_row_off = cp_seed_row0(e->wc, B_total, 0, B_total);
             if (launch_final_norm(e->s, f)) return -1;
         }
         Q3_HIP(hipStreamSynchronize(e->s), -1);
@@ -427,6 +459,7 @@
     const int H = m.cfg.hidden;
     if (max_frames <= 0 || max_frames > e->max_frames) max_frames = e->max_frames;
     std::vector<int> pos0(B);
+    std::vector<unsigned long long> seeds;
     for (int b = 0; b < B; b++) {
         if (n_rows[b] <= 0 || n_rows[b] > e->prefill_rows || n_rows[b] + max_frames > e->n_ctx) {
             Q3_LOG("q3e_start: utterance %d: %d prefix rows + %d frames do not fit n_ctx=%d", b, n_rows[b], max_frames,
@@ -452,8 +485,8 @@
         z = (z ^ (z >> 27)) * 0x94D049BB133111EBull;
         e->req_seed = e->n_requests == 1 ? e->seed : (z ^ (z >> 31));
         e->n_refills = 0;
-        std::vector<unsigned long long> seeds(B, e->req_seed);
-        Q3_HIP(hipMemcpy(e->d_seed, seeds.data(), sizeof(unsigned long long) * B, hipMemcpyHostToDevice), -1);
+        seeds.assign(B, e->req_seed);
+        Q3_HIP(hipMemcpyAsync(e->d_seed, seeds.data(), sizeof(unsigned long long) * B, hipMemcpyHostToDevice, e->s), -1);
     }
     if (e->forced_on) {
         e->forced_on = false;
@@ -501,14 +534,14 @@
     } else if (need_capture) {
         if (frame_eager(e)) return -1;
         done_frames++;
-        for (int c = 0; c < nc; c++) Q3_HIP(hipStreamSynchronize(e->cs[c]), -1);
+        for (int c = 0; c < nc; c++) Q3_HIP(hipStreamSynchronize(chain_stream(e, c)), -1);
         for (int c = 0; c < nc; c++) {
             int row0, R;
             chain_rows(e, c, row0, R);
             e->graph[c].reset();
-            Q3_HIP(hipStreamBeginCapture(e->cs[c], hipStreamCaptureModeRelaxed), -1);
-            int rc = frame_chain(e, e->cs[c], row0, R);
-            hipError_t er = hipStreamEndCapture(e->cs[c], &e->graph[c].g);
+            Q3_HIP(hipStreamBeginCapture(chain_stream(e, c), hipStreamCaptureModeRelaxed), -1);
+            int rc = frame_chain(e, chain_stream(e, c), row0, R);
+            hipError_t er = hipStreamEndCapture(chain_stream(e, c), &e->graph[c].g);
             if (rc || er != hipSuccess) {
                 Q3_LOG("q3e_run: graph capture failed");
                 return -1;
@@ -527,7 +560,7 @@
         int chunk = n_frames - done_frames;
         if (!e->ignore_eos && chunk > check_every) chunk = check_every;
         for (int i = 0; i < chunk; i++)
-            for (int c = 0; c < nc; c++) Q3_HIP(hipGraphLaunch(e->graph[c].e, e->cs[c]), -1);
+            for (int c = 0; c < nc; c++) Q3_HIP(hipGraphLaunch(e->graph[c].e, chain_stream(e, c)), -1);
         done_frames += chunk;
         if (!e->ignore_eos && done_frames < n_frames) {
             if (join_chains(e)) return -1;
@@ -569,19 +602,25 @@
         nf = std::min(hi, e->max_frames);
     }
     if (nf > max_out_frames) nf = max_out_frames;
-    Q3_HIP(hipMemcpy(out, e->d_codes, sizeof(int) * 16 * (size_t)e->B * nf, hipMemcpyDeviceToHost), -1);
-    if (n_frames_per_utt) {
-        Q3_HIP(hipMemcpy(n_frames_per_utt, e->d_npast, sizeof(int) * e->B, hipMemcpyDeviceToHost), -1);
-    }
+    int* h_np = e->h_read;
+    int* h_codes = e->h_read + e->max_batch;
+    const size_t n_codes = 16 * (size_t)e->B * (nf > 0 ? nf : 0);
+    if (n_codes) Q3_HIP(hipMemcpyAsync(h_codes, e->d_codes, sizeof(int) * n_codes, hipMemcpyDeviceToHost, e->s), -1);
+    if (n_frames_per_utt) Q3_HIP(hipMemcpyAsync(h_np, e->d_npast, sizeof(int) * e->B, hipMemcpyDeviceToHost, e->s), -1);
+    Q3_HIP(hipStreamSynchronize(e->s), -1);
+    if (n_codes) memcpy(out, h_codes, sizeof(int) * n_codes);
+    if (n_frames_per_utt) memcpy(n_frames_per_utt, h_np, sizeof(int) * e->B);
     return nf;
 }
 
 int q3e_get_done(void* ee, int32_t* done, int32_t* frames) {
     Engine* e = (Engine*)ee;
     if (!e || !done || e->B <= 0) return -1;
-    Q3_HIP(hipMemcpy(done, e->d_done, sizeof(int) * e->B, hipMemcpyDeviceToHost), -1);
-    std::vector<int> np(e->B);
-    Q3_HIP(hipMemcpy(np.data(), e->d_npast, sizeof(int) * e->B, hipMemcpyDeviceToHost), -1);
+    Q3_HIP(hipMemcpyAsync(e->h_done, e->d_done, sizeof(int) * e->B, hipMemcpyDeviceToHost, e->s), -1);
+    Q3_HIP(hipMemcpyAsync(e->h_read, e->d_npast, sizeof(int) * e->B, hipMemcpyDeviceToHost, e->s), -1);
+    Q3_HIP(hipStreamSynchronize(e->s), -1);
+    memcpy(done, e->h_done, sizeof(int) * e->B);
+    std::vector<int> np(e->h_read, e->h_read + e->B);
     for (int b = 0; b < e->B; b++)
         if (np[b] >= (e->slot_mode ? e->h_budget[b] : e->cap_frames)) done[b] = 1;
     if (e->slot_mode)
@@ -758,7 +797,8 @@
 int q3e_get_hidden(void* ee, float* out) {
     Engine* e = (Engine*)ee;
     if (!e || !out || e->B <= 0) return -1;
-    Q3_HIP(hipMemcpy(out, e->wt.hidden_f32, sizeof(float) * (size_t)e->B * e->m->cfg.hidden, hipMemcpyDeviceToHost), -1);
+    Q3_HIP(hipMemcpyAsync(out, e->wt.hidden_f32, sizeof(float) * (size_t)e->B * e->m->cfg.hidden, hipMemcpyDeviceToHost, e->s), -1);
+    Q3_HIP(hipStreamSynchronize(e->s), -1);
     return 0;
 }
 
diff --git a/qwen3_tts_axera_russian_amd/csrc/q3_model.h b/qwen3_tts_axera_russian_amd/csrc/q3_model.h
--- a/qwen3_tts_axera_russian_amd/csrc/q3_model.h
+++ b/qwen3_tts_axera_russian_amd/csrc/q3_model.h
@@ -46,7 +46,7 @@
     size_t device_bytes = 0;
 };
 
-Model* model_load(const char* path, bool want_talker, bool want_cp, const char* aux_dir = nullptr);
+Model* model_load(const char* path, bool want_talker, bool want_cp, const char* aux_dir = nullptr, hipStream_t s = nullptr);
 void model_free(Model* m);
 
 struct KVCache {
@@ -55,7 +55,7 @@
     size_t layer_stride() const { return (size_t)n_slots * n_kv * n_ctx * head_dim; }
     size_t bytes() const { return layer_stride() * n_layers * sizeof(half_t) * 2; }
 };
-int kv_alloc(KVCache& kv, int n_layers, int n_slots, int n_kv, int n_ctx);
+int kv_alloc(KVCache& kv, int n_layers, int n_slots, int n_kv, int n_ctx, hipStream_t s = nullptr);
 void kv_free(KVCache& kv);
 int kv_zero(hipStream_t s, KVCache& kv);
 
@@ -75,7 +75,7 @@
     int *map_slot = nullptr, *map_pos = nullptr;
     int map_R16 = 0;
 };
-int work_alloc(Work& w, const ModelCfg& c, int max_rows, int ffn, int max_vocab);
+int work_alloc(Work& w, const ModelCfg& c, int max_rows, int ffn, int max_vocab, hipStream_t s = nullptr);
 void work_free(Work& w);
 int work_zero(hipStream_t s, Work& w, const ModelCfg& c, int ffn, int max_vocab);
 
@@ -88,6 +88,7 @@
     const int* tiles = nullptr;
     int n_tiles = 0;
     bool skip_qkv0 = false;
+    int rows_total = 0;
 };
 
 int run_stack(hipStream_t s, const Model& m, const DevStack& st, Work& w, KVCache& kv, int R,
diff --git a/qwen3_tts_axera_russian_amd/csrc/q3_model.hip b/qwen3_tts_axera_russian_amd/csrc/q3_model.hip
--- a/qwen3_tts_axera_russian_amd/csrc/q3_model.hip
+++ b/qwen3_tts_axera_russian_amd/csrc/q3_model.hip
@@ -15,6 +15,9 @@
     std::vector<uint16_t> host16;
     bool ok = true;
 
+    bool up(void* d, const void* src, size_t bytes) {
+        return hipMemcpyAsync(d, src, bytes, hipMemcpyHostToDevice, s) == hipSuccess && hipStreamSynchronize(s) == hipSuccess;
+    }
     void* dalloc(size_t bytes) {
         void* d = nullptr;
         if (hipMalloc(&d, bytes) != hipSuccess) {
@@ -48,7 +51,7 @@
         float* d = (float*)dalloc(ne * 4);
         if (!d) return nullptr;
         if (t->dtype == F32) {
-            if (hipMemcpy(d, t->data, ne * 4, hipMemcpyHostToDevice) != hipSuccess) ok = false;
+            if (!up(d, t->data, ne * 4)) ok = false;
         } else {
             std::vector<float> tmp(ne);
             const uint16_t* src = (const uint16_t*)t->data;
@@ -56,7 +59,7 @@
                 for (size_t i = 0; i < ne; i++) tmp[i] = bf16_to_f32(src[i]);
             else
                 for (size_t i = 0; i < ne; i++) tmp[i] = h2f(src[i]);
-            if (hipMemcpy(d, tmp.data(), ne * 4, hipMemcpyHostToDevice) != hipSuccess) ok = false;
+            if (!up(d, tmp.data(), ne * 4)) ok = false;
         }
         return d;
     }
@@ -85,7 +88,7 @@
             for (size_t i = 0; i < ne; i++) host16[i] = f2h_sat(bf16_to_f32(b[i]));
             src = host16.data();
         }
-        if (hipMemcpy(stage, src, ne * 2, hipMemcpyHostToDevice) != hipSuccess) {
+        if (!up(stage, src, ne * 2)) {
             ok = false;
             return false;
         }
@@ -156,7 +159,7 @@
         if (good) {
             std::vector<int> iota(Vp, -1);
             for (int t = 0; t < V; t++) iota[t] = t;
-            good = hipMemcpy(ids, iota.data(), Vp * 4, hipMemcpyHostToDevice) == hipSuccess;
+            good = up(ids, iota.data(), Vp * 4);
         }
         for (int g = 0; g + 1 < G && good; g++) {
             good = launch_gather_embed(s, m->cp_emb[g], V, H, ids, 1, nullptr, 0, 0, h, ssq, (int)Vp, 0, 0, nullptr, xh,
@@ -195,7 +198,7 @@
 
 }
 
-Model* model_load(const char* path, bool want_talker, bool want_cp, const char* aux_dir) {
+Model* model_load(const char* path, bool want_talker, bool want_cp, const char* aux_dir, hipStream_t stream) {
     int ndev = 0;
     if (hipGetDeviceCount(&ndev) != hipSuccess || ndev <= 0) {
         Q3_LOG("no HIP device available -- this library has no CPU path");
@@ -214,7 +217,8 @@
     }
     hipGetDevice(&m->device);
     Loader L{m, p};
-    if (hipStreamCreate(&L.s) != hipSuccess) {
+    L.s = stream;
+    if (!stream && hipStreamCreateWithFlags(&L.s, hipStreamNonBlocking) != hipSuccess) {
         delete m;
         return nullptr;
     }
@@ -244,10 +248,7 @@
         }
         if (L.ok) {
             m->d_cp_emb_ptrs = (const float**)L.dalloc(sizeof(float*) * c.cp_groups);
-            if (m->d_cp_emb_ptrs &&
-                hipMemcpy((void*)m->d_cp_emb_ptrs, m->cp_emb.data(), sizeof(float*) * c.cp_groups,
-                          hipMemcpyHostToDevice) != hipSuccess)
-                L.ok = false;
+            if (m->d_cp_emb_ptrs && !L.up((void*)m->d_cp_emb_ptrs, m->cp_emb.data(), sizeof(float*) * c.cp_groups)) L.ok = false;
         }
         if (!m->talker_emb) {
             Q3_LOG("weight file lacks talker.codec_embedding (code_0 embedding of the code predictor)");
@@ -271,12 +272,13 @@
         m->rope_cos = (float*)L.dalloc(cs.size() * 4);
         m->rope_sin = (float*)L.dalloc(sn.size() * 4);
         if (L.ok) {
-            if (hipMemcpy(m->rope_cos, cs.data(), cs.size() * 4, hipMemcpyHostToDevice) != hipSuccess) L.ok = false;
-            if (hipMemcpy(m->rope_sin, sn.data(), sn.size() * 4, hipMemcpyHostToDevice) != hipSuccess) L.ok = false;
-        }
-    }
+            if (!L.up(m->rope_cos, cs.data(), cs.size() * 4)) L.ok = false;
+            if (!L.up(m->rope_sin, sn.data(), sn.size() * 4)) L.ok = false;
+        }
+    }
+    hipStreamSynchronize(L.s);
     if (L.stage) hipFree(L.stage);
-    hipStreamDestroy(L.s);
+    if (!stream) hipStreamDestroy(L.s);
     if (!L.ok) {
         model_free(m);
         return nullptr;
@@ -290,7 +292,7 @@
     delete m;
 }
 
-int kv_alloc(KVCache& kv, int n_layers, int n_slots, int n_kv, int n_ctx) {
+int kv_alloc(KVCache& kv, int n_layers, int n_slots, int n_kv, int n_ctx, hipStream_t s) {
     kv.n_layers = n_layers;
     kv.n_slots = n_slots;
     kv.n_kv = n_kv;
@@ -298,8 +300,9 @@
     const size_t bytes = kv.layer_stride() * n_layers * sizeof(half_t);
     Q3_HIP(hipMalloc((void**)&kv.k, bytes), -1);
     Q3_HIP(hipMalloc((void**)&kv.v, bytes), -1);
-    Q3_HIP(hipMemset(kv.k, 0, bytes), -1);
-    Q3_HIP(hipMemset(kv.v, 0, bytes), -1);
+    Q3_HIP(hipMemsetAsync(kv.k, 0, bytes, s), -1);
+    Q3_HIP(hipMemsetAsync(kv.v, 0, bytes, s), -1);
+    Q3_HIP(hipStreamSynchronize(s), -1);
     return 0;
 }
 void kv_free(KVCache& kv) {
@@ -331,7 +334,7 @@
     return 0;
 }
 
-int work_alloc(Work& w, const ModelCfg& c, int max_rows, int ffn, int max_vocab) {
+int work_alloc(Work& w, const ModelCfg& c, int max_rows, int ffn, int max_vocab, hipStream_t s) {
     max_rows = (max_rows + 127) / 128 * 128;
     w.max_rows = max_rows;
     w.hidden = c.hidden;
@@ -339,21 +342,22 @@
     const int qkv_ld = (c.n_heads + 2 * c.n_kv) * c.head_dim;
     Q3_HIP(hipMalloc((void**)&w.rows_in, R * c.hidden * 4), -1);
     Q3_HIP(hipMalloc((void**)&w.h, R * c.hidden * 4), -1);
-    Q3_HIP(hipMemset(w.h, 0, R * c.hidden * 4), -1);
+    Q3_HIP(hipMemsetAsync(w.h, 0, R * c.hidden * 4, s), -1);
     Q3_HIP(hipMalloc((void**)&w.ssq, R * (c.hidden / 16) * 4), -1);
     Q3_HIP(hipMalloc((void**)&w.xh, R * c.hidden * 2), -1);
-    Q3_HIP(hipMemset(w.xh, 0, R * c.hidden * 2), -1);
+    Q3_HIP(hipMemsetAsync(w.xh, 0, R * c.hidden * 2, s), -1);
     Q3_HIP(hipMalloc((void**)&w.qkv, R * qkv_ld * 4), -1);
     Q3_HIP(hipMalloc((void**)&w.attn, R * c.n_heads * c.head_dim * 2), -1);
-    Q3_HIP(hipMemset(w.attn, 0, R * c.n_heads * c.head_dim * 2), -1);
+    Q3_HIP(hipMemsetAsync(w.attn, 0, R * c.n_heads * c.head_dim * 2, s), -1);
     Q3_HIP(hipMalloc((void**)&w.act, R * ffn * 2), -1);
-    Q3_HIP(hipMemset(w.act, 0, R * ffn * 2), -1);
+    Q3_HIP(hipMemsetAsync(w.act, 0, R * ffn * 2, s), -1);
     Q3_HIP(hipMalloc((void**)&w.hidden_f32, R * c.hidden * 4), -1);
     Q3_HIP(hipMalloc((void**)&w.hidden_f16, R * c.hidden * 2), -1);
-    Q3_HIP(hipMemset(w.hidden_f16, 0, R * c.hidden * 2), -1);
+    Q3_HIP(hipMemsetAsync(w.hidden_f16, 0, R * c.hidden * 2, s), -1);
     Q3_HIP(hipMalloc((void**)&w.logits, R * max_vocab * 4), -1);
     Q3_HIP(hipMalloc((void**)&w.map_slot, R * 4), -1);
     Q3_HIP(hipMalloc((void**)&w.map_pos, R * 4), -1);
+    Q3_HIP(hipStreamSynchronize(s), -1);
     w.map_R16 = 0;
     return 0;
 }
@@ -418,6 +422,11 @@
         t.out = w.attn;
         t.scale = 1.0f / sqrtf((float)D);
         t.threads = attn_threads;
+        if (rm.rows_total > R) {
+            const int fit = 65536 / (rm.rows_total * c.n_kv);
+            if (t.threads > fit) t.threads = fit / 64 * 64;
+            if (t.threads < 256) t.threads = 256;
+        }
         t.valid_mod = rm.valid_mod;
         t.valid_n = rm.valid_n;
         if (rm.same_slot_rows && R > 1) {
diff --git a/qwen3_tts_axera_russian_amd/csrc/q3_talker_api.hip b/qwen3_tts_axera_russian_amd/csrc/q3_talker_api.hip
--- a/qwen3_tts_axera_russian_amd/csrc/q3_talker_api.hip
+++ b/qwen3_tts_axera_russian_amd/csrc/q3_talker_api.hip
@@ -101,8 +101,8 @@
     c->n_used.assign(n_slots, 0);
     const ModelCfg& cfg = tm->m->cfg;
     bool ok = hipStreamCreate(&c->s) == hipSuccess;
-    ok = ok && kv_alloc(c->kv, cfg.talker_layers, n_slots, cfg.n_kv, n_ctx) == 0;
-    ok = ok && work_alloc(c->w, cfg, c->n_batch, cfg.talker_ffn, cfg.talker_vocab) == 0;
+    ok = ok && kv_alloc(c->kv, cfg.talker_layers, n_slots, cfg.n_kv, n_ctx, c->s) == 0;
+    ok = ok && work_alloc(c->w, cfg, c->n_batch, cfg.talker_ffn, cfg.talker_vocab, c->s) == 0;
     ok = ok && hipMalloc((void**)&c->d_slot, sizeof(int) * c->n_batch) == hipSuccess;
     ok = ok && hipMalloc((void**)&c->d_pos, sizeof(int) * c->n_batch) == hipSuccess;
     ok = ok && hipHostMalloc((void**)&c->h_pinned, sizeof(float) * cfg.hidden * 2, 0) == hipSuccess;
@@ -285,7 +285,8 @@
                 const half_t* base = (kvsel ? c->kv.v : c->kv.k) + l * c->kv.layer_stride() +
                                      ((size_t)0 * c->kv.n_kv + g) * (size_t)c->kv.n_ctx * D;
                 if (n_pos > 0) {
-                    ok = hipMemcpy(buf.data(), base, buf.size() * 2, hipMemcpyDeviceToHost) == hipSuccess;
+                    ok = hipMemcpyAsync(buf.data(), base, buf.size() * 2, hipMemcpyDeviceToHost, c->s) == hipSuccess &&
+                         hipStreamSynchronize(c->s) == hipSuccess;
                     ok = ok && fwrite(buf.data(), 2, buf.size(), f) == buf.size();
                 }
             }
@@ -325,7 +326,8 @@
                                ((size_t)0 * c->kv.n_kv + g) * (size_t)c->kv.n_ctx * D;
                 if (n_pos > 0) {
                     ok = fread(buf.data(), 2, buf.size(), f) == buf.size();
-                    ok = ok && hipMemcpy(base, buf.data(), buf.size() * 2, hipMemcpyHostToDevice) == hipSuccess;
+                    ok = ok && hipMemcpyAsync(base, buf.data(), buf.size() * 2, hipMemcpyHostToDevice, c->s) == hipSuccess &&
+                         hipStreamSynchronize(c->s) == hipSuccess;
                 }
             }
     fclose(f);
diff --git a/qwen3_tts_axera_russian_amd/csrc/q3_text_api.hip b/qwen3_tts_axera_russian_amd/csrc/q3_text_api.hip
--- a/qwen3_tts_axera_russian_amd/csrc/q3_text_api.hip
+++ b/qwen3_tts_axera_russian_amd/csrc/q3_text_api.hip
@@ -65,7 +65,7 @@
 void* dal(TextFE* t, size_t bytes) {
     void* p = nullptr;
     if (hipMalloc(&p, bytes ? bytes : 16) != hipSuccess) return nullptr;
-    hipMemset(p, 0, bytes ? bytes : 16);
+    hipMemsetAsync(p, 0, bytes ? bytes : 16, t->s);
     t->allocs.push_back(p);
     return p;
 }
@@ -91,7 +91,8 @@
             } else return nullptr;
             src = buf.data();
         }
-        if (hipMemcpy(d + o, src, n * 2, hipMemcpyHostToDevice) != hipSuccess) return nullptr;
+        if (hipMemcpyAsync(d + o, src, n * 2, hipMemcpyHostToDevice, t->s) != hipSuccess || hipStreamSynchronize(t->s) != hipSuccess)
+            return nullptr;
     }
     return d;
 }
@@ -107,7 +108,7 @@
         for (size_t i = 0; i < ne; i++) tmp[i] = pt->dtype == BF16 ? bf16_to_f32(u[i]) : h2f(u[i]);
         src = tmp.data();
     }
-    return hipMemcpy(d, src, ne * 4, hipMemcpyHostToDevice) == hipSuccess ? d : nullptr;
+    return hipMemcpyAsync(d, src, ne * 4, hipMemcpyHostToDevice, t->s) == hipSuccess && hipStreamSynchronize(t->s) == hipSuccess ? d : nullptr;
 }
 bool pack_linear(TextFE* t, const PackTensor* pt, DevLinear& L) {
     L.N = (int)pt->shape[0];
@@ -221,6 +222,7 @@
     ok = ok && (t->h1 = (float*)dal(t, Rp * mid * 4)) && (t->h2 = (float*)dal(t, Rp * t->H * 4));
     ok = ok && (t->ssq = (float*)dal(t, Rp * (mid / 16) * 4)) && (t->out = (float*)dal(t, Rp * t->H * 4));
     ok = ok && (t->d_ids = (int*)dal(t, Rp * 4)) && (t->d_src = (int*)dal(t, Rp * 4)) && (t->d_cod = (int*)dal(t, Rp * 4));
+    ok = ok && hipStreamSynchronize(t->s) == hipSuccess;
     if (!ok) {
         Q3_LOG("tfe_load: upload failed");
         tfe_free(t);
diff --git a/qwen3_tts_axera_russian_amd/csrc/q3_voc.hip b/qwen3_tts_axera_russian_amd/csrc/q3_voc.hip
--- a/qwen3_tts_axera_russian_amd/csrc/q3_voc.hip
+++ b/qwen3_tts_axera_russian_amd/csrc/q3_voc.hip
@@ -1277,7 +1277,24 @@
     ChunkPlace* d_place = nullptr;
     float batch_ms = 0.f;
     int batch_chunks = 0;
+    char* h_stage = nullptr;
+    size_t h_stage_bytes = 0;
+    int* h_ovf = nullptr;
 };
+
+static bool voc_upload(Voc* v, void* d, const void* src, size_t bytes) {
+    return hipMemcpyAsync(d, src, bytes, hipMemcpyHostToDevice, v->s) == hipSuccess && hipStreamSynchronize(v->s) == hipSuccess;
+}
+
+static int voc_read_back(Voc* v, void* out, const void* dev, size_t bytes) {
+    for (size_t o = 0; o < bytes; o += v->h_stage_bytes) {
+        const size_t n = bytes - o < v->h_stage_bytes ? bytes - o : v->h_stage_bytes;
+        Q3_HIP(hipMemcpyAsync(v->h_stage, (const char*)dev + o, n, hipMemcpyDeviceToHost, v->s), -1);
+        Q3_HIP(hipStreamSynchronize(v->s), -1);
+        memcpy((char*)out + o, v->h_stage, n);
+    }
+    return 0;
+}
 
 static float* voc_up(Voc* v, const PackTensor* t) {
     size_t ne = t->numel();
@@ -1293,7 +1310,7 @@
     float* d = nullptr;
     if (hipMalloc((void**)&d, ne * 4) != hipSuccess) return nullptr;
     v->allocs.push_back(d);
-    if (hipMemcpy(d, src, ne * 4, hipMemcpyHostToDevice) != hipSuccess) return nullptr;
+    if (!voc_upload(v, d, src, ne * 4)) return nullptr;
     return d;
 }
 
@@ -1301,7 +1318,7 @@
     float* d = nullptr;
     if (hipMalloc((void**)&d, h.size() * 4) != hipSuccess) return nullptr;
     v->allocs.push_back(d);
-    if (hipMemcpy(d, h.data(), h.size() * 4, hipMemcpyHostToDevice) != hipSuccess) return nullptr;
+    if (!voc_upload(v, d, h.data(), h.size() * 4)) return nullptr;
     return d;
 }
 
@@ -1318,6 +1335,8 @@
     if (v->d_wave16) hipFree(v->d_wave16);
     if (v->d_place) hipFree(v->d_place);
     if (v->d_ovf) hipFree(v->d_ovf);
+    if (v->h_stage) hipHostFree(v->h_stage);
+    if (v->h_ovf) hipHostFree(v->h_ovf);
     if (v->e0) hipEventDestroy(v->e0);
     if (v->e1) hipEventDestroy(v->e1);
     if (v->s) hipStreamDestroy(v->s);
@@ -1362,7 +1381,8 @@
     bool ok = true;
     {
         int lo = 0, hi = 0;
-        const bool prio = !(getenv("Q3_STREAM_PRIO") && atoi(getenv("Q3_STREAM_PRIO")) == 0);
+        const int mode = getenv("Q3_STREAM_PRIO") ? atoi(getenv("Q3_STREAM_PRIO")) : 1;
+        const bool prio = mode != 0 && mode != 2;
         if (prio && hipDeviceGetStreamPriorityRange(&lo, &hi) == hipSuccess && lo != hi)
             ok = hipStreamCreateWithPriority(&v->s, hipStreamNonBlocking, lo) == hipSuccess;
         else
@@ -1501,8 +1521,7 @@
                     }
                     v->allocs.push_back(dh);
                     v->allocs.push_back(dl);
-                    ok = hipMemcpy(dh, hi.data(), hi.size() * 2, hipMemcpyHostToDevice) == hipSuccess &&
-                         hipMemcpy(dl, lo.data(), lo.size() * 2, hipMemcpyHostToDevice) == hipSuccess;
+                    ok = voc_upload(v, dh, hi.data(), hi.size() * 2) && voc_upload(v, dl, lo.data(), lo.size() * 2);
                     op.w_hi = (_Float16*)dh;
                     op.w_lo = (_Float16*)dl;
                     op.Mp128 = Mp;
@@ -1648,11 +1667,16 @@
         v->flops_per_chunk = flops;
         v->buf_elems = max_elems * v->max_batch;
         for (int i = 0; i < 3 && ok; i++)
-            ok = hipMalloc((void**)&v->buf[i], v->buf_elems * 4) == hipSuccess && hipMemset(v->buf[i], 0, v->buf_elems * 4) == hipSuccess;
+            ok = hipMalloc((void**)&v->buf[i], v->buf_elems * 4) == hipSuccess && hipMemsetAsync(v->buf[i], 0, v->buf_elems * 4, v->s) == hipSuccess;
         for (int i = 0; i < 4 && ok; i++) ok = hipMalloc((void**)&v->plane[i], v->buf_elems * 2) == hipSuccess;
         ok = ok && hipMalloc((void**)&v->d_codes, sizeof(int64_t) * 16 * v->chunk * v->max_batch) == hipSuccess;
-        ok = ok && hipMalloc((void**)&v->d_ovf, 16) == hipSuccess && hipMemset(v->d_ovf, 0, 16) == hipSuccess;
+        ok = ok && hipMalloc((void**)&v->d_ovf, 16) == hipSuccess && hipMemsetAsync(v->d_ovf, 0, 16, v->s) == hipSuccess;
         ok = ok && hipMalloc((void**)&v->d_place, sizeof(ChunkPlace) * v->max_batch) == hipSuccess;
+        v->h_stage_bytes = sizeof(float) * (size_t)v->chunk_samples * v->max_batch;
+        if (v->h_stage_bytes < 4096) v->h_stage_bytes = 4096;
+        ok = ok && hipHostMalloc((void**)&v->h_stage, v->h_stage_bytes, 0) == hipSuccess;
+        ok = ok && hipHostMalloc((void**)&v->h_ovf, 16, 0) == hipSuccess;
+        ok = ok && hipStreamSynchronize(v->s) == hipSuccess;
     }
     if (!ok) {
         Q3_LOG("voc_load failed");
@@ -1944,21 +1968,22 @@
     float* res = nullptr;
     if (voc_run(v, B, &res)) return -1;
     Q3_HIP(hipEventRecord(v->e1, v->s), -1);
-    int ovf = 0;
-    if (g_voc_split) Q3_HIP(hipMemcpyAsync(&ovf, v->d_ovf, sizeof(int), hipMemcpyDeviceToHost, v->s), -1);
+    *v->h_ovf = 0;
+    if (g_voc_split) Q3_HIP(hipMemcpyAsync(v->h_ovf, v->d_ovf, sizeof(int), hipMemcpyDeviceToHost, v->s), -1);
     const size_t row = sizeof(float) * (size_t)v->chunk_samples, dpitch = sizeof(float) * (size_t)pitch4(v->chunk_samples);
-    Q3_HIP(hipMemcpy2DAsync(out, row, res, dpitch, row, (size_t)B, hipMemcpyDeviceToHost, v->s), -1);
+    Q3_HIP(hipMemcpy2DAsync(v->h_stage, row, res, dpitch, row, (size_t)B, hipMemcpyDeviceToHost, v->s), -1);
     Q3_HIP(hipStreamSynchronize(v->s), -1);
-    if (ovf) {
+    if (*v->h_ovf) {
         if (!v->warned_ovf) Q3_LOG("vocoder: activation outside the fp16 range, decoding this call with the exact-fp32 path");
         v->warned_ovf = true;
         Q3_HIP(hipMemsetAsync(v->d_ovf, 0, sizeof(int), v->s), -1);
         Q3_HIP(hipEventRecord(v->e0, v->s), -1);
         if (voc_run(v, B, &res, -1, nullptr, nullptr, nullptr, true)) return -1;
         Q3_HIP(hipEventRecord(v->e1, v->s), -1);
-        Q3_HIP(hipMemcpy2DAsync(out, row, res, dpitch, row, (size_t)B, hipMemcpyDeviceToHost, v->s), -1);
+        Q3_HIP(hipMemcpy2DAsync(v->h_stage, row, res, dpitch, row, (size_t)B, hipMemcpyDeviceToHost, v->s), -1);
         Q3_HIP(hipStreamSynchronize(v->s), -1);
     }
+    memcpy(out, v->h_stage, row * (size_t)B);
     hipEventElapsedTime(&v->last_ms, v->e0, v->e1);
     return 0;
 }
@@ -2078,11 +2103,11 @@
             calls++;
         }
         Q3_HIP(hipEventRecord(v->e1, v->s), -1);
-        int ovf = 0;
-        if (g_voc_split && !redo_exact) Q3_HIP(hipMemcpyAsync(&ovf, v->d_ovf, sizeof(int), hipMemcpyDeviceToHost, v->s), -1);
+        *v->h_ovf = 0;
+        if (g_voc_split && !redo_exact) Q3_HIP(hipMemcpyAsync(v->h_ovf, v->d_ovf, sizeof(int), hipMemcpyDeviceToHost, v->s), -1);
         Q3_HIP(hipStreamSynchronize(v->s), -1);
         *n_calls = calls;
-        if (!ovf) break;
+        if (!*v->h_ovf) break;
         if (!v->warned_ovf) Q3_LOG("vocoder: activation outside the fp16 range, decoding this request with the exact-fp32 path");
         v->warned_ovf = true;
         Q3_HIP(hipMemsetAsync(v->d_ovf, 0, sizeof(int), v->s), -1);
@@ -2136,12 +2161,12 @@
     hipEventElapsedTime(&v->batch_ms, v->e0, v->e1);
     v->batch_chunks = (int)walk.size();
     if (!want16) {
-        Q3_HIP(hipMemcpyAsync(out, v->d_wave, sizeof(float) * (size_t)total, hipMemcpyDeviceToHost, v->s), -1);
+        if (voc_read_back(v, out, v->d_wave, sizeof(float) * (size_t)total)) return -1;
     } else {
         if (grow(&v->d_wave16, &v->wave16_cap, (size_t)total)) return -1;
         hipLaunchKernelGGL(voc_to_int16_kernel, dim3((unsigned)((total + 255) / 256)), dim3(256), 0, v->s, v->d_wave, v->d_wave16, total);
         Q3_HIP(hipGetLastError(), -1);
-        Q3_HIP(hipMemcpyAsync(out, v->d_wave16, sizeof(int16_t) * (size_t)total, hipMemcpyDeviceToHost, v->s), -1);
+        if (voc_read_back(v, out, v->d_wave16, sizeof(int16_t) * (size_t)total)) return -1;
     }
     Q3_HIP(hipStreamSynchronize(v->s), -1);
     return 0;
@@ -2299,8 +2324,8 @@
         }
         Q3_HIP(hipGetLastError(), -1);
         if (total > 0)
-            Q3_HIP(hipMemcpyAsync(out, want16 ? (void*)s->d_out16 : (void*)s->d_out, (want16 ? sizeof(int16_t) : sizeof(float)) * (size_t)total,
-                                  hipMemcpyDeviceToHost, v->s), -1);
+            if (voc_read_back(v, out, want16 ? (void*)s->d_out16 : (void*)s->d_out, (want16 ? sizeof(int16_t) : sizeof(float)) * (size_t)total))
+                return -1;
         Q3_HIP(hipStreamSynchronize(v->s), -1);
     }
     for (int i = 0; i < n; i++) {
@@ -2779,8 +2804,8 @@
     if (!p.keys.empty()) {
         Q3_HIP(hipEventRecord(v->e1, v->s), -1);
         if (total > 0)
-            Q3_HIP(hipMemcpyAsync(out, want16 ? (void*)s->d_out16 : (void*)s->d_out, (want16 ? sizeof(int16_t) : sizeof(float)) * (size_t)total,
-                                  hipMemcpyDeviceToHost, v->s), -1);
+            if (voc_read_back(v, out, want16 ? (void*)s->d_out16 : (void*)s->d_out, (want16 ? sizeof(int16_t) : sizeof(float)) * (size_t)total))
+                return -1;
         Q3_HIP(hipStreamSynchronize(v->s), -1);
         hipEventElapsedTime(&s->last_ms, v->e0, v->e1);
     }
@@ -2865,7 +2890,7 @@
     s->out_cap = (size_t)max_streams * v->chunk * v->upsample;
     auto alloc = [&](void** p, size_t bytes, bool zero) {
         if (!ok) return;
-        ok = hipMalloc(p, bytes) == hipSuccess && (!zero || hipMemset(*p, 0, bytes) == hipSuccess);
+        ok = hipMalloc(p, bytes) == hipSuccess && (!zero || hipMemsetAsync(*p, 0, bytes, v->s) == hipSuccess);
         if (ok) s->device_bytes += bytes;
     };
     alloc((void**)&s->d_hist, sizeof(float) * std::max<size_t>(1, s->state_floats * max_streams), true);
@@ -2876,6 +2901,7 @@
     alloc((void**)&s->d_off, sizeof(long long) * mb, false);
     alloc((void**)&s->d_out, sizeof(float) * s->out_cap, false);
     alloc((void**)&s->d_out16, sizeof(int16_t) * s->out_cap, false);
+    ok = ok && hipStreamSynchronize(v->s) == hipSuccess;
     if (!ok) {
         Q3_LOG("voc_incr_create: device allocation failed");
         incr_destroy(s);
```

After: 10130 codec_frames/s, median of 6. 10.5% higher.
